# kolenyo2099/revers-o

Hardware: AMD Instinct MI355X
Metric: images/sec embed+top-k (PE-L14-336, 1M x 1024 gallery) (higher is better)
Workload: dtype bf16

## Files before the change

### include/revo.h

```cpp
#ifndef REVO_H
#define REVO_H
#include <stdint.h>

#ifdef __cplusplus
extern "C" {
#endif

typedef struct revo_vit revo_vit;
typedef struct revo_gallery revo_gallery;

typedef struct revo_vit_cfg {
    int32_t image_size, patch_size, width, layers, heads, mlp_dim, out_dim, pool_heads;
    int32_t use_cls;
    int32_t use_ls;
    float ln_eps, rope_theta;
    int32_t pool_mlp_dim;
} revo_vit_cfg;

typedef struct revo_tensor {
    const char* name;
    const float* data;
    int64_t numel;
} revo_tensor;

const char* revo_last_error(void);
int32_t revo_version(void);
int32_t revo_sync(void* stream);

int32_t revo_vit_create(const revo_vit_cfg* cfg, const revo_tensor* weights, int32_t n_weights, int32_t device,
                        int32_t max_batch, revo_vit** out);
int32_t revo_vit_destroy(revo_vit* vit);
int32_t revo_vit_forward(revo_vit* vit, const void* images, int32_t image_dtype, int32_t batch, float* out,
                         int32_t normalize, void* stream);
int32_t revo_vit_seq_len(const revo_vit* vit);
int32_t revo_vit_stats(revo_vit* vit, double* out4, int32_t reset, void* stream);

int32_t revo_gallery_create(int32_t dim, int64_t capacity, int32_t device, int32_t keep_f32, revo_gallery** out);
int32_t revo_gallery_destroy(revo_gallery* g);
int32_t revo_gallery_append(revo_gallery* g, const float* vecs, int64_t n, int32_t normalize, int32_t src_on_device,
                            void* stream);
int64_t revo_gallery_size(const revo_gallery* g);
int32_t revo_gallery_clear(revo_gallery* g);
int32_t revo_gallery_read(revo_gallery* g, int64_t start, int64_t n, float* dst, int32_t dst_on_device);

int32_t revo_gallery_remove(revo_gallery* g, const uint32_t* remove_bits, int64_t rows, int32_t src_on_device,
                            int64_t* n_removed, void* stream);
int32_t revo_gallery_update(revo_gallery* g, const int64_t* row_idx, const float* vecs, int64_t n, int32_t normalize,
                            int32_t src_on_device, void* stream);

int32_t revo_search_topk(revo_gallery* g, const float* queries, int32_t n_queries, int32_t k, int32_t has_threshold,
                         float threshold, int64_t index_offset, float* scores, int64_t* indices, int32_t* counts,
                         void* stream);
int32_t revo_search_topk_large(revo_gallery* g, const float* queries, int32_t n_queries, int32_t k, int32_t has_threshold,
                               float threshold, int64_t index_offset, float* scores, int64_t* indices, int32_t* counts,
                               void* stream);
int32_t revo_gallery_pairs(revo_gallery* g, float threshold, int64_t* n_pairs, void* stream);
int32_t revo_gallery_pairs_read(revo_gallery* g, int64_t start, int64_t n, int64_t* pairs, float* scores,
                                int32_t dst_on_device);
int32_t revo_gallery_clusters(revo_gallery* g, float threshold, int64_t* n_clusters, int64_t* n_members, void* stream);
int32_t revo_gallery_clusters_read(revo_gallery* g, int64_t* labels, int64_t* offsets, int64_t* members,
                                   int32_t dst_on_device);
int32_t revo_search_range(revo_gallery* g, const float* queries, int32_t n_queries, float threshold, int64_t index_offset,
                          int64_t* n_results, void* stream);
int32_t revo_search_range_read(revo_gallery* g, int64_t* offsets, int64_t start, int64_t n, int64_t* indices, float* scores,
                               int32_t dst_on_device);
int32_t revo_search_recommend(revo_gallery* g, const float* examples, int32_t n_positive, int32_t n_negative, int32_t k,
                              int32_t has_threshold, float threshold, int64_t index_offset, float* scores, int64_t* indices,
                              int32_t* counts, void* stream);
int32_t revo_search_discover(revo_gallery* g, const float* target, const float* positives, const float* negatives,
                             int32_t n_pairs, int32_t k, int32_t has_threshold, float threshold, int64_t index_offset,
                             float* scores, int64_t* indices, int32_t* counts, void* stream);
int32_t revo_search_maxsim(revo_gallery* g, const float* queries, int32_t n_vectors, int32_t k, int32_t has_threshold,
                           float threshold, int64_t index_offset, float* scores, int32_t* group_ids, int32_t* counts,
                           float* part_scores, int64_t* part_rows, void* stream);
int32_t revo_search_mmr(revo_gallery* g, const float* queries, int32_t n_queries, int32_t k, int32_t candidates,
                        float diversity, int32_t has_threshold, float threshold, int64_t index_offset, float* scores,
                        float* mmr_values, int64_t* indices, int32_t* counts, void* stream);
int32_t revo_search_ksel(int32_t k);
int32_t revo_search_set_total_rows(revo_gallery* g, int64_t total_rows);
int32_t revo_search_set_filter(revo_gallery* g, const uint32_t* allow_bits, int64_t rows, int32_t src_on_device,
                               void* stream);
int32_t revo_search_set_groups(revo_gallery* g, const int32_t* group_of_row, int64_t rows, int32_t src_on_device,
                               void* stream);
int32_t revo_search_groups(revo_gallery* g, const float* queries, int32_t n_queries, int32_t limit, int32_t group_size,
                           int32_t has_threshold, float threshold, int64_t index_offset, float* scores, int64_t* indices,
                           int32_t* hit_counts, int32_t* group_ids, int32_t* group_counts, void* stream);
int32_t revo_search_estimates(int32_t k);
int32_t revo_search_plan(const revo_gallery* g, int32_t n_queries, int32_t k, int64_t* out4);
int32_t revo_search_candidates(revo_gallery* g, const float* queries, int32_t n_queries, int32_t k, int32_t top_m,
                               uint32_t* bounds, void* stream);
int32_t revo_search_finish(revo_gallery* g, int32_t n_queries, int32_t k, int32_t has_threshold, float threshold,
                           int64_t index_offset, const uint32_t* all_bounds, int32_t parts, int32_t top_m, float* scores,
                           int64_t* indices, int32_t* counts, float* cert, void* stream);
int32_t revo_search_exact(revo_gallery* g, int32_t n, const int32_t* q_idx, const float* need, int32_t k,
                          int32_t has_threshold, float threshold, int64_t index_offset, float* scores, int64_t* indices,
                          int32_t* counts, void* stream);
int32_t revo_search_stats(revo_gallery* g, int32_t* out8, void* stream);
int32_t revo_topk_merge(const float* scores, const int64_t* indices, int32_t parts, int32_t n_queries, int32_t k,
                        int32_t has_threshold, float threshold, float* out_scores, int64_t* out_indices,
                        int32_t* out_counts, void* stream);

int64_t revo_topk_packed_bytes(int32_t n_queries, int32_t k);
int32_t revo_topk_merge_packed(const void* packed, int32_t parts, int32_t n_queries, int32_t k, int32_t has_threshold,
                               float threshold, float* out_scores, int64_t* out_indices, int32_t* out_counts,
                               int32_t* unc_count, int32_t* unc_q, float* unc_need, void* stream);

int32_t revo_op_gemm(int32_t epilogue, const void* a_bf16, int64_t lda, const void* b_bf16, int64_t ldb, int32_t m,
                     int32_t n, int32_t k, void* c, int64_t ldc, const float* bias, const float* gamma, void* stream);
int32_t revo_op_gemm_rope(const void* a_bf16, int64_t lda, const void* b_bf16, int64_t ldb, int32_t m, int32_t n, int32_t k,
                          void* c_bf16, int64_t ldc, const float* bias, const float* cos_sin, int32_t seq,
                          int32_t head_dim, int32_t rope_cols, void* stream);
int32_t revo_op_gemm_resid_ln(const void* a_bf16, int64_t lda, const void* b_bf16, int64_t ldb, int32_t m, int32_t n, int32_t k,
                              float* c, int64_t ldc, const float* bias, const float* gamma, void* xb_bf16, int64_t ldxb,
                              void* stats, int32_t* done, void* xlo_bf16, int32_t x_in_planes, int32_t planes_out, void* stream);
int32_t revo_op_gemm_ln_in(int32_t epilogue, const void* a_bf16, int64_t lda, const void* b_bf16, int64_t ldb, int32_t m, int32_t n,
                           int32_t k, void* c_bf16, int64_t ldc, const float* bias, const float* csum, const void* stats,
                           int32_t parts, float eps, void* tele, void* stream);
int32_t revo_op_gemm_ln_in_rope(const void* a_bf16, int64_t lda, const void* b_bf16, int64_t ldb, int32_t m, int32_t n, int32_t k,
                                void* c_bf16, int64_t ldc, const float* bias, const float* csum, const void* stats, int32_t parts,
                                float eps, const float* cos_sin, int32_t seq, int32_t head_dim, int32_t rope_cols, void* stream);
int32_t revo_op_gemm_resid_norm(const void* a_bf16, int64_t lda, const void* b_bf16, int64_t ldb, int32_t m, int32_t n, int32_t k,
                                float* c, int64_t ldc, const float* bias, const float* gamma, void* ln_out_bf16, int64_t ln_ldo,
                                float eps, int32_t* fused, void* stream);
int32_t revo_probe_mfma(const void* src_bf16, int64_t n_elems, float* sink, int32_t blocks, int32_t iters, void* stream);
int64_t revo_probe_mfma_flops(int32_t blocks, int32_t iters);
int32_t revo_probe_copy(void* dst, const void* src, int64_t bytes, void* stream);
#ifdef REVO_EXPERIMENTS
int32_t revo_vit_set_debug_layers(revo_vit* vit, int32_t n_layers);
int32_t revo_vit_read_residual(revo_vit* vit, int32_t batch, float* dst, void* stream);
int32_t revo_vit_read_tap(revo_vit* vit, int32_t which, int32_t batch, void* dst, void* stream);
int32_t revo_search_set_mode(revo_gallery* g, int32_t mode);
int32_t revo_debug_set_remove_chunk(int64_t rows);
int32_t revo_op_set_phase_groups(int32_t groups);
int32_t revo_op_set_qstores(int32_t on);
int32_t revo_debug_gemm_stamps(void* buf, int32_t items);
int32_t revo_debug_attention_clock(void* buf);
int32_t revo_debug_gemm_forms(int32_t reset);
int32_t revo_op_set_gemm_tile(int32_t tile);
int32_t revo_op_set_variant(int32_t flags);
int32_t revo_op_set_ln_fold(int32_t on);
int32_t revo_op_set_gemm_debug(int32_t flags);
int64_t revo_debug_scan_plan(int32_t Q, int64_t rows, int64_t* out, int32_t cap);
int32_t revo_debug_stream_in_planes(const revo_vit* vit, int32_t batch);
int64_t revo_debug_read_workspace(revo_gallery* g, int64_t offset, int64_t bytes, void* host_dst);
int32_t revo_debug_seed_bounds(revo_gallery* g, const uint32_t* bounds);
int32_t revo_probe_gridbar(int32_t mode, void* ctr_err, void* buf, int32_t n16, int32_t blocks, int32_t threads,
                           int32_t iters, float* sink, void* stamps, void* stream);
int32_t revo_debug_scan_stats(int64_t* out8);
#endif
int32_t revo_op_layernorm(const float* x, int64_t ldx, const float* w, const float* b, float eps, int32_t rows,
                          int32_t width, void* out, int64_t ldo, int32_t out_is_bf16, void* stream);
int32_t revo_op_layernorm_logits(const float* x, int64_t ldx, const float* w, const float* b, float eps, int32_t rows,
                                 int32_t width, float* out, int64_t ldo, const float* qk, const float* ck, int32_t heads,
                                 int32_t seq, float* logits, void* stream);
int32_t revo_op_linear_f32(int32_t epi, const float* A, int64_t lda, const float* Wt, int64_t ldw, const float* bias, int32_t M,
                           int32_t N, int32_t K, float* C, int64_t ldc, void* stream);
int32_t revo_op_pool_rows(const float* x, int64_t ldx, const float* logits, int32_t batch, int32_t seq, int32_t width,
                          int32_t heads, float* u, void* stream);
int32_t revo_op_rope(void* qkv_bf16, int64_t ld, const float* cos_sin, int32_t rows, int32_t seq, int32_t width,
                     int32_t heads, void* stream);
int32_t revo_op_attention(const void* qkv_bf16, int64_t ld, void* out_bf16, int64_t ldo, int32_t batch, int32_t seq,
                          int32_t heads, int32_t head_dim, void* stream);
int32_t revo_op_f32_to_bf16(const float* src, int64_t ld_src, void* dst_bf16, int64_t ld_dst, int64_t rows,
                            int32_t cols, void* stream);

int32_t revo_prof_enable(int32_t on);
int32_t revo_prof_reset(void);
int32_t revo_prof_report(char* buf, int32_t capacity);

typedef struct revo_crop_job {
    const uint8_t* src;
    int32_t height, width;
    int64_t row_stride;
    int32_t x0, y0, x1, y1;
} revo_crop_job;
int32_t revo_preprocess_crop_resize(const revo_crop_job* jobs, int32_t n, int32_t out_size, uint8_t* out, void* stream);

#ifdef __cplusplus
}
#endif
#endif
```

### revers-o_amd/_lib.py

```python
import ctypes as C
import os

_HERE = os.path.dirname(os.path.abspath(__file__))
LIB_PATH = os.path.join(_HERE, "librevo.so")


class RevoError(RuntimeError):
    pass


class VitCfg(C.Structure):
    _fields_ = [(n, C.c_int32) for n in (
        "image_size", "patch_size", "width", "layers", "heads", "mlp_dim", "out_dim", "pool_heads",
        "use_cls", "use_ls")] + [("ln_eps", C.c_float), ("rope_theta", C.c_float), ("pool_mlp_dim", C.c_int32)]


class Tensor(C.Structure):
    _fields_ = [("name", C.c_char_p), ("data", C.c_void_p), ("numel", C.c_int64)]


class CropJob(C.Structure):
    _fields_ = [("src", C.c_void_p), ("height", C.c_int32), ("width", C.c_int32), ("row_stride", C.c_int64),
                ("x0", C.c_int32), ("y0", C.c_int32), ("x1", C.c_int32), ("y1", C.c_int32)]


_p, _i32, _i64, _f32 = C.c_void_p, C.c_int32, C.c_int64, C.c_float

SIGNATURES = {
    "revo_last_error": (C.c_char_p, []),
    "revo_version": (_i32, []),
    "revo_sync": (_i32, [_p]),
    "revo_vit_create": (_i32, [C.POINTER(VitCfg), C.POINTER(Tensor), _i32, _i32, _i32, C.POINTER(_p)]),
    "revo_vit_destroy": (_i32, [_p]),
    "revo_vit_forward": (_i32, [_p, _p, _i32, _i32, _p, _i32, _p]),
    "revo_vit_seq_len": (_i32, [_p]),
    "revo_vit_stats": (_i32, [_p, C.POINTER(C.c_double), _i32, _p]),
    "revo_gallery_create": (_i32, [_i32, _i64, _i32, _i32, C.POINTER(_p)]),
    "revo_gallery_destroy": (_i32, [_p]),
    "revo_gallery_append": (_i32, [_p, _p, _i64, _i32, _i32, _p]),
    "revo_gallery_size": (_i64, [_p]),
    "revo_gallery_clear": (_i32, [_p]),
    "revo_gallery_read": (_i32, [_p, _i64, _i64, _p, _i32]),
    "revo_gallery_remove": (_i32, [_p, _p, _i64, _i32, C.POINTER(C.c_int64), _p]),
    "revo_gallery_update": (_i32, [_p, _p, _p, _i64, _i32, _i32, _p]),
    "revo_gallery_pairs": (_i32, [_p, _f32, C.POINTER(C.c_int64), _p]),
    "revo_gallery_pairs_read": (_i32, [_p, _i64, _i64, _p, _p, _i32]),
    "revo_gallery_clusters": (_i32, [_p, _f32, C.POINTER(C.c_int64), C.POINTER(C.c_int64), _p]),
    "revo_gallery_clusters_read": (_i32, [_p, _p, _p, _p, _i32]),
    "revo_search_range": (_i32, [_p, _p, _i32, _f32, _i64, C.POINTER(C.c_int64), _p]),
    "revo_search_range_read": (_i32, [_p, _p, _i64, _i64, _p, _p, _i32]),
    "revo_search_recommend": (_i32, [_p, _p, _i32, _i32, _i32, _i32, _f32, _i64, _p, _p, _p, _p]),
    "revo_search_discover": (_i32, [_p, _p, _p, _p, _i32, _i32, _i32, _f32, _i64, _p, _p, _p, _p]),
    "revo_search_maxsim": (_i32, [_p, _p, _i32, _i32, _i32, _f32, _i64, _p, _p, _p, _p, _p, _p]),
    "revo_search_mmr": (_i32, [_p, _p, _i32, _i32, _i32, _f32, _i32, _f32, _i64, _p, _p, _p, _p, _p]),
    "revo_search_topk": (_i32, [_p, _p, _i32, _i32, _i32, _f32, _i64, _p, _p, _p, _p]),
    "revo_search_topk_large": (_i32, [_p, _p, _i32, _i32, _i32, _f32, _i64, _p, _p, _p, _p]),
    "revo_search_ksel": (_i32, [_i32]),
    "revo_search_set_total_rows": (_i32, [_p, _i64]),
    "revo_search_set_filter": (_i32, [_p, _p, _i64, _i32, _p]),
    "revo_search_set_groups": (_i32, [_p, _p, _i64, _i32, _p]),
    "revo_search_groups": (_i32, [_p, _p, _i32, _i32, _i32, _i32, _f32, _i64, _p, _p, _p, _p, _p, _p]),
    "revo_search_estimates": (_i32, [_i32]),
    "revo_search_plan": (_i32, [_p, _i32, _i32, C.POINTER(C.c_int64)]),
    "revo_search_candidates": (_i32, [_p, _p, _i32, _i32, _i32, _p, _p]),
    "revo_search_finish": (_i32, [_p, _i32, _i32, _i32, _f32, _i64, _p, _i32, _i32, _p, _p, _p, _p, _p]),
    "revo_search_exact": (_i32, [_p, _i32, _p, _p, _i32, _i32, _f32, _i64, _p, _p, _p, _p]),
    "revo_search_stats": (_i32, [_p, C.POINTER(C.c_int32), _p]),
    "revo_topk_merge": (_i32, [_p, _p, _i32, _i32, _i32, _i32, _f32, _p, _p, _p, _p]),
    "revo_topk_packed_bytes": (_i64, [_i32, _i32]),
    "revo_topk_merge_packed": (_i32, [_p, _i32, _i32, _i32, _i32, _f32, _p, _p, _p, _p, _p, _p, _p]),
    "revo_op_gemm": (_i32, [_i32, _p, _i64, _p, _i64, _i32, _i32, _i32, _p, _i64, _p, _p, _p]),
    "revo_op_gemm_resid_ln": (_i32, [_p, _i64, _p, _i64, _i32, _i32, _i32, _p, _i64, _p, _p, _p, _i64, _p, C.POINTER(C.c_int32), _p, _i32,
                                     _i32, _p]),
    "revo_op_gemm_ln_in": (_i32, [_i32, _p, _i64, _p, _i64, _i32, _i32, _i32, _p, _i64, _p, _p, _p, _i32, _f32, _p, _p]),
    "revo_op_gemm_rope": (_i32, [_p, _i64, _p, _i64, _i32, _i32, _i32, _p, _i64, _p, _p, _i32, _i32, _i32, _p]),
    "revo_op_gemm_ln_in_rope": (_i32, [_p, _i64, _p, _i64, _i32, _i32, _i32, _p, _i64, _p, _p, _p, _i32, _f32, _p, _i32, _i32, _i32,
                                       _p]),
    "revo_op_gemm_resid_norm": (_i32, [_p, _i64, _p, _i64, _i32, _i32, _i32, _p, _i64, _p, _p, _p, _i64, _f32, C.POINTER(C.c_int32),
                                       _p]),
    "revo_op_layernorm": (_i32, [_p, _i64, _p, _p, _f32, _i32, _i32, _p, _i64, _i32, _p]),
    "revo_op_layernorm_logits": (_i32, [_p, _i64, _p, _p, _f32, _i32, _i32, _p, _i64, _p, _p, _i32, _i32, _p, _p]),
    "revo_op_linear_f32": (_i32, [_i32, _p, _i64, _p, _i64, _p, _i32, _i32, _i32, _p, _i64, _p]),
    "revo_op_pool_rows": (_i32, [_p, _i64, _p, _i32, _i32, _i32, _i32, _p, _p]),
    "revo_op_rope": (_i32, [_p, _i64, _p, _i32, _i32, _i32, _i32, _p]),
    "revo_op_attention": (_i32, [_p, _i64, _p, _i64, _i32, _i32, _i32, _i32, _p]),
    "revo_op_f32_to_bf16": (_i32, [_p, _i64, _p, _i64, _i64, _i32, _p]),
    "revo_prof_enable": (_i32, [_i32]),
    "revo_prof_reset": (_i32, []),
    "revo_prof_report": (_i32, [C.c_char_p, _i32]),
    "revo_preprocess_crop_resize": (_i32, [C.POINTER(CropJob), _i32, _i32, _p, _p]),
    "revo_probe_mfma": (_i32, [_p, _i64, _p, _i32, _i32, _p]),
    "revo_probe_mfma_flops": (_i64, [_i32, _i32]),
    "revo_probe_copy": (_i32, [_p, _p, _i64, _p]),
}

EXPERIMENT_SIGNATURES = {
    "revo_vit_set_debug_layers": (_i32, [_p, _i32]),
    "revo_vit_read_residual": (_i32, [_p, _i32, _p, _p]),
    "revo_vit_read_tap": (_i32, [_p, _i32, _i32, _p, _p]),
    "revo_search_set_mode": (_i32, [_p, _i32]),
    "revo_op_set_gemm_tile": (_i32, [_i32]),
    "revo_op_set_phase_groups": (_i32, [_i32]),
    "revo_op_set_qstores": (_i32, [_i32]),
    "revo_debug_gemm_forms": (_i32, [_i32]),
    "revo_debug_gemm_stamps": (_i32, [_p, _i32]),
    "revo_debug_attention_clock": (_i32, [_p]),
    "revo_op_set_variant": (_i32, [_i32]),
    "revo_op_set_ln_fold": (_i32, [_i32]),
    "revo_op_set_gemm_debug": (_i32, [_i32]),
    "revo_debug_scan_stats": (_i32, [C.POINTER(C.c_int64)]),
    "revo_debug_set_remove_chunk": (_i32, [_i64]),
    "revo_debug_seed_bounds": (_i32, [_p, _p]),
    "revo_debug_read_workspace": (_i64, [_p, _i64, _i64, _p]),
    "revo_debug_stream_in_planes": (_i32, [_p, _i32]),
    "revo_probe_gridbar": (_i32, [_i32, _p, _p, _i32, _i32, _i32, _i32, _p, _p, _p]),
    "revo_debug_scan_plan": (_i64, [_i32, _i64, C.POINTER(C.c_int64), _i32]),
}
BASE_SIGNATURES = dict(SIGNATURES)
if os.environ.get("REVO_LIBRARY_PATH"):
    LIB_PATH = os.environ["REVO_LIBRARY_PATH"]
elif os.environ.get("REVO_EXPERIMENTS") == "1":
    LIB_PATH = os.path.join(_HERE, "librevo_exp.so")
if os.environ.get("REVO_EXPERIMENTS") == "1":
    SIGNATURES = dict(SIGNATURES, **EXPERIMENT_SIGNATURES)

_lib = None
_lib_exp = None


def product_is_experiment_build():
    return os.environ.get("REVO_EXPERIMENTS") == "1"


def load_exp():
    global _lib_exp
    if _lib_exp is not None:
        return _lib_exp
    import torch
    path = os.path.join(_HERE, "librevo_exp.so")
    if not os.path.exists(path):
        raise RevoError(f"{path} not found: build it with `make -C revers-o_amd/csrc exp`")
    lib = C.CDLL(path)
    for name, (res, args) in dict(BASE_SIGNATURES, **EXPERIMENT_SIGNATURES).items():
        fn = getattr(lib, name)
        fn.restype = res
        fn.argtypes = args
    _lib_exp = lib
    return lib


def load():
    global _lib
    if _lib is not None:
        return _lib
    import torch
    if not os.path.exists(LIB_PATH):
        raise RevoError(
            f"{LIB_PATH} not found: build it with `python -c 'import __graft_entry__ as g; g.build()'` "
            "(or `make -C revers-o_amd/csrc`).  There is no CPU fallback for the hot path.")
    lib = C.CDLL(LIB_PATH)
    for name, (res, args) in SIGNATURES.items():
        try:
            fn = getattr(lib, name)
        except AttributeError:
            if os.environ.get("REVO_LIBRARY_PATH"):
                continue
            raise
        fn.restype = res
        fn.argtypes = args
    _lib = lib
    return lib


def check(rc, what=""):
    if rc != 0:
        msg = load().revo_last_error().decode("utf-8", "replace")
        if _lib_exp is not None:
            msg = (msg + " | " if msg else "") + _lib_exp.revo_last_error().decode("utf-8", "replace")
        raise RevoError(f"{what} failed (status {rc}): {msg}")


def ptr(t):
    return None if t is None else C.c_void_p(t.data_ptr())


def current_stream():
    import torch
    return C.c_void_p(torch.cuda.current_stream().cuda_stream)
```

### revers-o_amd/csrc/api.hip

```cpp
#include <algorithm>
#include <cmath>
#include <cstdlib>
#include <cstring>
#include <map>
#include <memory>
#include <mutex>
#include <string>
#include <vector>

#include "../../include/revo.h"
#include "api_internal.h"
#include "kernels.h"

static thread_local std::string g_err;
void revo_set_error(const std::string& msg) { g_err = msg; }
extern "C" const char* revo_last_error(void) { return g_err.c_str(); }
extern "C" int32_t revo_version(void) { return 100; }

extern "C" int32_t revo_sync(void* stream) {
    REVO_HIP_CHECK(hipStreamSynchronize((hipStream_t)stream));
    return 0;
}

namespace {
struct Profiler {
    int on = 0;
    unsigned sample[4] = {0, 0, 0, 0};
    std::mutex mu;
    std::vector<ProfRec> recs;
    std::vector<hipEvent_t> pool;
    std::map<std::string, std::pair<long, double>> acc;
    hipEvent_t get() {
        if (!pool.empty()) { hipEvent_t e = pool.back(); pool.pop_back(); return e; }
        hipEvent_t e; (void)hipEventCreate(&e); return e;
    }
    void drain() {
        for (auto& r : recs) {
            float ms = 0.f;
            if (hipEventSynchronize(r.b) == hipSuccess && hipEventElapsedTime(&ms, r.a, r.b) == hipSuccess) {
                auto& s = acc[r.cls];
                s.first += 1; s.second += ms;
            }
            pool.push_back(r.a); pool.push_back(r.b);
        }
        recs.clear();
    }
} g_prof;
}

ProfScope::ProfScope(const char* cls, hipStream_t s) : active(g_prof.on != 0), st(s) {
    if (active && g_prof.on >= 2) {
        const int which = !strcmp(cls, "gemm_qkv") ? 0 : !strcmp(cls, "gemm_out") ? 1 : !strcmp(cls, "gemm_fc1") ? 2 :
                          !strcmp(cls, "gemm_fc2") ? 3 : -1;
        active = which >= 0;
        if (active && g_prof.on == 3) active = (g_prof.sample[which]++ & 3) == 0;
    }
    if (!active) return;
    std::lock_guard<std::mutex> lk(g_prof.mu);
    rec.cls = cls; rec.a = g_prof.get(); rec.b = g_prof.get();
    (void)hipEventRecord(rec.a, st);
}
ProfScope::~ProfScope() {
    if (!active) return;
    (void)hipEventRecord(rec.b, st);
    std::lock_guard<std::mutex> lk(g_prof.mu);
    g_prof.recs.push_back(rec);
}

extern "C" int32_t revo_prof_enable(int32_t on) {
    g_prof.on = on < 0 ? 0 : (on > 3 ? 1 : on);
    for (auto& x : g_prof.sample) x = 0;
    return 0;
}
extern "C" int32_t revo_prof_reset(void) {
    std::lock_guard<std::mutex> lk(g_prof.mu);
    g_prof.drain();
    g_prof.acc.clear();
    return 0;
}
extern "C" int32_t revo_prof_report(char* buf, int32_t capacity) {
    std::lock_guard<std::mutex> lk(g_prof.mu);
    g_prof.drain();
    std::string s = "{";
    bool first = true;
    for (auto& kv : g_prof.acc) {
        if (!first) s += ", ";
        first = false;
        s += "\"" + kv.first + "\": {\"launches\": " + std::to_string(kv.second.first) +
             ", \"ms\": " + std::to_string(kv.second.second) + "}";
    }
    s += "}";
    if ((int)s.size() + 1 > capacity) { revo_set_error("prof_report: buffer too small"); return -2; }
    memcpy(buf, s.c_str(), s.size() + 1);
    return 0;
}

namespace revo {
__global__ __launch_bounds__(256) void probe_q_kernel(const float* __restrict__ w, const float* __restrict__ bias,
                                                      const float* __restrict__ probe, int W, float scale,
                                                      float* __restrict__ q) {
    const int lane = threadIdx.x & 63;
    const int o = blockIdx.x * 4 + (threadIdx.x >> 6);
    if (o >= W) return;
    float acc = 0.f;
    for (int i = lane; i < W; i += 64) acc = fmaf(w[(long)o * W + i], probe[i], acc);
    acc = wave_sum(acc);
    if (lane == 0) q[o] = (acc + bias[o]) * scale;
}
}

struct LayerW {
    bf16_t *w_qkv, *w_o, *w_fc1, *w_fc2;
    float *b_qkv, *b_o, *b_fc1, *b_fc2, *c_qkv, *c_fc1, *ls1, *ls2;
};

constexpr size_t SPLITK_WS_ELEMS = 16u << 20;
struct revo_vit {
    revo_vit_cfg cfg;
    int device = 0, max_batch = 0, S = 0, G2 = 0, Kp = 0, hd = 0, phd = 0, PM = 0, debug_layers = -1;
    std::vector<void*> owned;
    bf16_t* w_patch = nullptr; float *cls = nullptr, *pos = nullptr, *lnpre_w = nullptr, *lnpre_b = nullptr,
            *lnpost_w = nullptr, *lnpost_b = nullptr;
    std::vector<LayerW> layers;
    float *q_probe = nullptr, *qk = nullptr, *ck = nullptr, *w_v = nullptr, *b_v = nullptr, *w_po = nullptr, *b_po = nullptr;
    float *pln_w = nullptr, *pln_b = nullptr, *w_pfc1 = nullptr, *b_pfc1 = nullptr, *w_pfc2 = nullptr, *b_pfc2 = nullptr,
          *w_projT = nullptr;
    float2* rope_cs = nullptr;
    bf16_t *patches = nullptr, *h = nullptr, *qkv = nullptr, *att = nullptr, *mlp = nullptr;
    bf16_t* xlo = nullptr;
    float *x = nullptr, *pool_logits = nullptr, *pool_u = nullptr, *pool_att = nullptr, *pool_o = nullptr, *pool_h = nullptr,
          *pool_m = nullptr, *feat = nullptr;
    float* splitk_ws = nullptr;
    float2* ln_stats = nullptr;
    int ln_parts = 0;
    unsigned long long* ln_tele = nullptr;

    template <class T> int dalloc(T** out, size_t count) {
        void* p = nullptr;
        REVO_HIP_CHECK(hipMalloc(&p, count * sizeof(T) + 256));
        owned.push_back(p);
        *out = (T*)p;
        return 0;
    }
    ~revo_vit() {
        for (void* p : owned) (void)hipFree(p);
    }
};

namespace {
struct WeightMap {
    std::map<std::string, const revo_tensor*> m;
    const revo_tensor* get(const std::string& name, int64_t numel) {
        auto it = m.find(name);
        if (it == m.end()) { revo_set_error("missing weight tensor: " + name); return nullptr; }
        if (it->second->numel != numel) {
            revo_set_error("weight " + name + ": expected " + std::to_string(numel) + " elements, got " +
                           std::to_string(it->second->numel));
            return nullptr;
        }
        return it->second;
    }
};

int up_f32(revo_vit* v, WeightMap& wm, const std::string& name, int64_t numel, float** out) {
    const revo_tensor* t = wm.get(name, numel);
    if (!t) return -2;
    CHECK_RC(v->dalloc(out, (size_t)numel));
    REVO_HIP_CHECK(hipMemcpy(*out, t->data, (size_t)numel * 4, hipMemcpyDefault));
    return 0;
}
int up_folded(revo_vit* v, WeightMap& wm, float* stage, float* gb, const std::string& wname, const std::string& bname,
              const std::string& ln, int64_t rows, int64_t cols, bf16_t** w_out, float** c_out, float** b_out) {
    const revo_tensor *tw = wm.get(wname, rows * cols), *tb = wm.get(bname, rows), *tg = wm.get(ln + ".weight", cols),
                      *te = wm.get(ln + ".bias", cols);
    if (!tw || !tb || !tg || !te) return -2;
    CHECK_RC(v->dalloc(w_out, (size_t)(rows * cols)));
    CHECK_RC(v->dalloc(c_out, (size_t)rows));
    CHECK_RC(v->dalloc(b_out, (size_t)rows));
    REVO_HIP_CHECK(hipMemcpy(stage, tw->data, (size_t)(rows * cols) * 4, hipMemcpyDefault));
    REVO_HIP_CHECK(hipMemcpy(gb, tg->data, (size_t)cols * 4, hipMemcpyDefault));
    REVO_HIP_CHECK(hipMemcpy(gb + cols, te->data, (size_t)cols * 4, hipMemcpyDefault));
    REVO_HIP_CHECK(hipMemcpy(gb + 2 * cols, tb->data, (size_t)rows * 4, hipMemcpyDefault));
    CHECK_RC(revo::launch_fold_ln_linear(stage, gb, gb + cols, gb + 2 * cols, (int)rows, (int)cols, *w_out, cols, *c_out, *b_out, 0));
    REVO_HIP_CHECK(hipStreamSynchronize(0));
    return 0;
}
int up_bf16(revo_vit* v, float* stage, const float* src, int64_t rows, int64_t cols, int64_t ld, bf16_t** out) {
    CHECK_RC(v->dalloc(out, (size_t)(rows * ld)));
    REVO_HIP_CHECK(hipMemcpy(stage, src, (size_t)(rows * cols) * 4, hipMemcpyDefault));
    CHECK_RC(revo::launch_f32_to_bf16(stage, cols, *out, ld, rows, (int)cols, 0));
    REVO_HIP_CHECK(hipStreamSynchronize(0));
    return 0;
}
}

extern "C" int32_t revo_vit_create(const revo_vit_cfg* cfg, const revo_tensor* weights, int32_t n_weights,
                                   int32_t device, int32_t max_batch, revo_vit** out) {
    API_BEGIN
    REVO_REQUIRE(cfg && weights && out, "vit_create: null argument");
    REVO_REQUIRE(max_batch >= 1, "vit_create: max_batch must be >= 1");
    const revo_vit_cfg& c = *cfg;
    REVO_REQUIRE(c.image_size % c.patch_size == 0, "vit_create: image_size must be a multiple of patch_size");
    REVO_REQUIRE(c.width % c.heads == 0 && c.width % c.pool_heads == 0, "vit_create: width must divide into heads");
    REVO_REQUIRE(c.width % 64 == 0 && c.mlp_dim % 64 == 0, "vit_create: width and mlp_dim must be multiples of 64");
    REVO_REQUIRE(c.out_dim % 4 == 0, "vit_create: out_dim must be a multiple of 4");
    REVO_REQUIRE(c.width / c.heads == 64 || c.width / c.heads == 96,
                 "vit_create: body head_dim must be 64 (PE-Core B16 / L14) or 96 (G14)");
    REVO_REQUIRE(c.image_size > 0 && c.patch_size > 0 && c.layers >= 1 && c.heads >= 1 && c.pool_heads >= 1 && n_weights >= 0,
                 "vit_create: sizes must be positive");
    std::unique_ptr<revo_vit> v(new revo_vit());
    v->cfg = c; v->device = device; v->max_batch = max_batch;
#ifdef REVO_EXPERIMENTS
    if (const char* e = getenv("REVO_LN_FOLD")) revo::gemm_set_ln_fold(atoi(e));
#endif
    const int W = c.width, M = c.mlp_dim, D = c.out_dim, P = c.patch_size, G = c.image_size / P;
    v->G2 = G * G; v->S = v->G2 + (c.use_cls ? 1 : 0);
    v->hd = W / c.heads; v->phd = W / c.pool_heads;
    const int PM = c.pool_mlp_dim > 0 ? c.pool_mlp_dim : 4 * W;
    REVO_REQUIRE(PM % 64 == 0, "vit_create: pool_mlp_dim must be a multiple of 64");
    v->PM = PM;
    const int Kreal = 3 * P * P;
    v->Kp = (Kreal + 63) / 64 * 64;
    const int S = v->S;

    WeightMap wm;
    for (int i = 0; i < n_weights; ++i) {
        REVO_REQUIRE(weights[i].name && weights[i].data, "vit_create: weight entry with a null name or data pointer");
        wm.m[weights[i].name] = &weights[i];
    }
    {
        std::vector<std::pair<std::string, int64_t>> need = {
            {"visual.conv1.weight", (int64_t)W * Kreal}, {"visual.positional_embedding", (int64_t)S * W},
            {"visual.ln_pre.weight", W}, {"visual.ln_pre.bias", W}, {"visual.ln_post.weight", W}, {"visual.ln_post.bias", W},
            {"visual.attn_pool.probe", W}, {"visual.attn_pool.attn.in_proj_weight", (int64_t)3 * W * W},
            {"visual.attn_pool.attn.in_proj_bias", 3 * W}, {"visual.attn_pool.attn.out_proj.weight", (int64_t)W * W},
            {"visual.attn_pool.attn.out_proj.bias", W}, {"visual.attn_pool.layernorm.weight", W},
            {"visual.attn_pool.layernorm.bias", W}, {"visual.attn_pool.mlp.c_fc.weight", (int64_t)PM * W},
            {"visual.attn_pool.mlp.c_fc.bias", PM}, {"visual.attn_pool.mlp.c_proj.weight", (int64_t)W * PM},
            {"visual.attn_pool.mlp.c_proj.bias", W}, {"visual.proj", (int64_t)W * D}};
        if (c.use_cls) need.push_back({"visual.class_embedding", W});
        for (int i = 0; i < c.layers; ++i) {
            const std::string p = "visual.transformer.resblocks." + std::to_string(i) + ".";
            for (const char* n : {"ln_1.weight", "ln_1.bias", "ln_2.weight", "ln_2.bias", "attn.out_proj.bias", "mlp.c_proj.bias"})
                need.push_back({p + n, W});
            need.push_back({p + "attn.in_proj_weight", (int64_t)3 * W * W});
            need.push_back({p + "attn.in_proj_bias", 3 * W});
            need.push_back({p + "attn.out_proj.weight", (int64_t)W * W});
            need.push_back({p + "mlp.c_fc.weight", (int64_t)M * W});
            need.push_back({p + "mlp.c_fc.bias", M});
            need.push_back({p + "mlp.c_proj.weight", (int64_t)W * M});
            if (c.use_ls) { need.push_back({p + "ls_1.gamma", W}); need.push_back({p + "ls_2.gamma", W}); }
        }
        for (auto& kv : need)
            if (!wm.get(kv.first, kv.second)) return -2;
        if (wm.m.size() != need.size()) {
            std::map<std::string, int64_t> want(need.begin(), need.end());
            for (auto& kv : wm.m)
                if (!want.count(kv.first)) {
                    revo_set_error("unexpected weight tensor: " + kv.first + " (not read by this architecture" +
                                   (c.use_ls ? ")" : "; LayerScale needs cfg.use_ls = 1)"));
                    return -2;
                }
        }
    }
    REVO_ON_DEVICE(device);

    size_t stage_elems = (size_t)std::max({(long)3 * W * W, (long)M * W, (long)PM * W, (long)W * Kreal, (long)W * D});
    float* stage = nullptr;
    REVO_HIP_CHECK(hipMalloc((void**)&stage, stage_elems * 4));
    struct StageGuard { float* p; ~StageGuard() { (void)hipFree(p); } } sg{stage};
    float* gb = nullptr;
    REVO_HIP_CHECK(hipMalloc((void**)&gb, (size_t)(2 * W + std::max(3 * W, M)) * 4));
    StageGuard sg2{gb};

    const revo_tensor* t;
    if (!(t = wm.get("visual.conv1.weight", (int64_t)W * Kreal))) return -2;
    CHECK_RC(v->dalloc(&v->w_patch, (size_t)W * 3 * v->Kp));
    REVO_HIP_CHECK(hipMemcpy(stage, t->data, (size_t)W * Kreal * 4, hipMemcpyDefault));
    CHECK_RC(revo::launch_split_hi_lo_hi(stage, W, Kreal, 1.0f / 255.0f, v->w_patch, v->Kp, 0));
    REVO_HIP_CHECK(hipStreamSynchronize(0));
    if (c.use_cls) CHECK_RC(up_f32(v.get(), wm, "visual.class_embedding", W, &v->cls));
    CHECK_RC(up_f32(v.get(), wm, "visual.positional_embedding", (int64_t)S * W, &v->pos));
    CHECK_RC(up_f32(v.get(), wm, "visual.ln_pre.weight", W, &v->lnpre_w));
    CHECK_RC(up_f32(v.get(), wm, "visual.ln_pre.bias", W, &v->lnpre_b));
    CHECK_RC(up_f32(v.get(), wm, "visual.ln_post.weight", W, &v->lnpost_w));
    CHECK_RC(up_f32(v.get(), wm, "visual.ln_post.bias", W, &v->lnpost_b));
    v->layers.resize(c.layers);
    for (int i = 0; i < c.layers; ++i) {
        const std::string p = "visual.transformer.resblocks." + std::to_string(i) + ".";
        LayerW& L = v->layers[i];
        memset(&L, 0, sizeof(L));
        CHECK_RC(up_folded(v.get(), wm, stage, gb, p + "attn.in_proj_weight", p + "attn.in_proj_bias", p + "ln_1", 3 * W, W,
                           &L.w_qkv, &L.c_qkv, &L.b_qkv));
        if (!(t = wm.get(p + "attn.out_proj.weight", (int64_t)W * W))) return -2;
        CHECK_RC(up_bf16(v.get(), stage, t->data, W, W, W, &L.w_o));
        CHECK_RC(up_f32(v.get(), wm, p + "attn.out_proj.bias", W, &L.b_o));
        CHECK_RC(up_folded(v.get(), wm, stage, gb, p + "mlp.c_fc.weight", p + "mlp.c_fc.bias", p + "ln_2", M, W,
                           &L.w_fc1, &L.c_fc1, &L.b_fc1));
        if (!(t = wm.get(p + "mlp.c_proj.weight", (int64_t)W * M))) return -2;
        CHECK_RC(up_bf16(v.get(), stage, t->data, W, M, M, &L.w_fc2));
        CHECK_RC(up_f32(v.get(), wm, p + "mlp.c_proj.bias", W, &L.b_fc2));
        if (c.use_ls) {
            CHECK_RC(up_f32(v.get(), wm, p + "ls_1.gamma", W, &L.ls1));
            CHECK_RC(up_f32(v.get(), wm, p + "ls_2.gamma", W, &L.ls2));
        }
    }
    {
        const std::string p = "visual.attn_pool.";
        float *probe = nullptr, *wi = nullptr, *bi = nullptr;
        CHECK_RC(up_f32(v.get(), wm, p + "probe", W, &probe));
        CHECK_RC(up_f32(v.get(), wm, p + "attn.in_proj_weight", (int64_t)3 * W * W, &wi));
        CHECK_RC(up_f32(v.get(), wm, p + "attn.in_proj_bias", 3 * W, &bi));
        CHECK_RC(v->dalloc(&v->q_probe, (size_t)W));
        hipLaunchKernelGGL(revo::probe_q_kernel, dim3((W + 3) / 4), dim3(256), 0, 0, wi, bi, probe, W,
                           1.0f / sqrtf((float)v->phd), v->q_probe);
        REVO_HIP_CHECK(hipGetLastError());
        CHECK_RC(v->dalloc(&v->qk, (size_t)c.pool_heads * W));
        CHECK_RC(v->dalloc(&v->ck, (size_t)c.pool_heads));
        CHECK_RC(revo::launch_probe_qk(v->q_probe, wi + (size_t)W * W, bi + W, W, c.pool_heads, v->qk, v->ck, 0));
        v->w_v = wi + (size_t)2 * W * W;
        v->b_v = bi + 2 * W;
        REVO_HIP_CHECK(hipStreamSynchronize(0));
        CHECK_RC(up_f32(v.get(), wm, p + "attn.out_proj.weight", (int64_t)W * W, &v->w_po));
        CHECK_RC(up_f32(v.get(), wm, p + "attn.out_proj.bias", W, &v->b_po));
        CHECK_RC(up_f32(v.get(), wm, p + "layernorm.weight", W, &v->pln_w));
        CHECK_RC(up_f32(v.get(), wm, p + "layernorm.bias", W, &v->pln_b));
        CHECK_RC(up_f32(v.get(), wm, p + "mlp.c_fc.weight", (int64_t)PM * W, &v->w_pfc1));
        CHECK_RC(up_f32(v.get(), wm, p + "mlp.c_fc.bias", PM, &v->b_pfc1));
        CHECK_RC(up_f32(v.get(), wm, p + "mlp.c_proj.weight", (int64_t)W * PM, &v->w_pfc2));
        CHECK_RC(up_f32(v.get(), wm, p + "mlp.c_proj.bias", W, &v->b_pfc2));
    }
    if (!(t = wm.get("visual.proj", (int64_t)W * D))) return -2;
    CHECK_RC(v->dalloc(&v->w_projT, (size_t)D * W));
    REVO_HIP_CHECK(hipMemcpy(stage, t->data, (size_t)W * D * 4, hipMemcpyDefault));
    CHECK_RC(revo::launch_transpose_f32(stage, W, D, v->w_projT, 0));
    REVO_HIP_CHECK(hipStreamSynchronize(0));

    {
        const int hd = v->hd, d = hd / 2, nf = d / 2;
        std::vector<float2> cs((size_t)S * (hd / 2));
        const int start = c.use_cls ? 1 : 0;
        for (int s = 0; s < S; ++s) {
            for (int pi = 0; pi < hd / 2; ++pi) {
                double ang = 0.0;
                if (!(c.use_cls && s == 0)) {
                    const int g = s - (c.use_cls ? 1 : 0);
                    const int gy = g / G, gx = g % G;
                    const bool xaxis = pi < nf;
                    const int f = xaxis ? pi : pi - nf;
                    const double freq = 1.0 / pow((double)c.rope_theta, (double)(2 * f) / (double)d);
                    ang = (double)((xaxis ? gx : gy) + start) * freq;
                }
                cs[(size_t)s * (hd / 2) + pi] = make_float2((float)cos(ang), (float)sin(ang));
            }
        }
        CHECK_RC(v->dalloc(&v->rope_cs, cs.size()));
        REVO_HIP_CHECK(hipMemcpy(v->rope_cs, cs.data(), cs.size() * sizeof(float2), hipMemcpyHostToDevice));
    }

    const size_t rows = (size_t)max_batch * S, B = (size_t)max_batch;
    CHECK_RC(v->dalloc(&v->patches, (size_t)max_batch * v->G2 * 3 * v->Kp));
    CHECK_RC(v->dalloc(&v->x, rows * W));
    CHECK_RC(v->dalloc(&v->h, rows * W));
    CHECK_RC(v->dalloc(&v->qkv, rows * 3 * W));
    CHECK_RC(v->dalloc(&v->att, rows * W));
    CHECK_RC(v->dalloc(&v->mlp, rows * M));
    CHECK_RC(v->dalloc(&v->pool_logits, B * c.pool_heads * S));
    CHECK_RC(v->dalloc(&v->pool_u, B * c.pool_heads * W));
    CHECK_RC(v->dalloc(&v->pool_att, B * W));
    CHECK_RC(v->dalloc(&v->pool_o, B * W));
    CHECK_RC(v->dalloc(&v->pool_h, B * W));
    CHECK_RC(v->dalloc(&v->pool_m, B * PM));
    CHECK_RC(v->dalloc(&v->feat, B * D));
    CHECK_RC(v->dalloc(&v->splitk_ws, SPLITK_WS_ELEMS));
    v->ln_parts = (W % 256 == 0 && W / 256 <= 6) ? W / 256 : 0;
    if (v->ln_parts) CHECK_RC(v->dalloc(&v->ln_stats, rows * (size_t)v->ln_parts));
    if (v->ln_parts) CHECK_RC(v->dalloc(&v->xlo, rows * W));
    CHECK_RC(v->dalloc(&v->ln_tele, 4));
    REVO_HIP_CHECK(hipMemset(v->ln_tele, 0, 4 * sizeof(unsigned long long)));
    REVO_HIP_CHECK(hipDeviceSynchronize());
    *out = v.release();
    return 0;
    API_END
}

extern "C" int32_t revo_vit_destroy(revo_vit* vit) {
    API_BEGIN
    if (vit) { DeviceGuard dg(vit->device); delete vit; }
    return 0;
    API_END
}
extern "C" int32_t revo_vit_seq_len(const revo_vit* vit) { return vit ? vit->S : -1; }
extern "C" int32_t revo_vit_stats(revo_vit* vit, double* out4, int32_t reset, void* stream) {
    API_BEGIN
    REVO_REQUIRE(vit && out4, "vit_stats: null argument");
    REVO_ON_DEVICE(vit->device);
    unsigned long long c[4] = {0, 0, 0, 0};
    REVO_HIP_CHECK(hipStreamSynchronize((hipStream_t)stream));
    REVO_HIP_CHECK(hipMemcpy(c, vit->ln_tele, sizeof(c), hipMemcpyDeviceToHost));
    if (reset) REVO_HIP_CHECK(hipMemset(vit->ln_tele, 0, sizeof(c)));
    out4[0] = (double)c[0]; out4[1] = (double)c[1]; out4[2] = (double)c[2]; out4[3] = (double)revo::LNC_TELE_RATIO;
    return 0;
    API_END
}
#ifdef REVO_EXPERIMENTS
extern "C" int32_t revo_vit_set_debug_layers(revo_vit* vit, int32_t n) {
    REVO_REQUIRE(vit, "null handle");
    vit->debug_layers = n;
    return 0;
}
extern "C" int32_t revo_vit_read_residual(revo_vit* vit, int32_t batch, float* dst, void* stream) {
    REVO_REQUIRE(vit && dst && batch >= 1 && batch <= vit->max_batch, "read_residual: bad arguments");
    REVO_ON_DEVICE(vit->device);
    REVO_HIP_CHECK(hipMemcpyAsync(dst, vit->x, (size_t)batch * vit->S * vit->cfg.width * 4, hipMemcpyDeviceToDevice,
                                  (hipStream_t)stream));
    return 0;
}

extern "C" int32_t revo_vit_read_tap(revo_vit* vit, int32_t which, int32_t batch, void* dst, void* stream) {
    REVO_REQUIRE(vit && dst && batch >= 1 && batch <= vit->max_batch, "read_tap: bad arguments");
    REVO_ON_DEVICE(vit->device);
    const size_t rows = (size_t)batch * vit->S, W = vit->cfg.width;
    const void* src = nullptr;
    size_t bytes = 0;
    switch (which) {
        case 0: src = vit->x; bytes = rows * W * 4; break;
        case 1: src = vit->x; bytes = rows * W * 4; break;
        case 2: src = vit->pool_o; bytes = (size_t)batch * W * 4; break;
        default: REVO_REQUIRE(false, "read_tap: which must be 0 (residual), 1 (ln_post output) or 2 (pooled)");
    }
    REVO_HIP_CHECK(hipMemcpyAsync(dst, src, bytes, hipMemcpyDeviceToDevice, (hipStream_t)stream));
    return 0;
}
#endif

namespace {
struct LnAfter { float eps; bf16_t* out; long ldo; int* fused; float2* stats; int* folded; bf16_t* lo; int x_in_planes, planes_out; };
struct LnBefore { const float2* stats; int parts; const float* c; float eps; };
int gemm(const char* cls, int epi, const bf16_t* A, long lda, const bf16_t* B, long ldb, int M, int N, int K, void* C,
         long ldc, const float* bias, const float* gamma, hipStream_t st, float* ws = nullptr, long ws_elems = 0,
         const LnAfter* ln = nullptr) {
    revo::GemmArgs a{};
    a.A = A; a.lda = lda; a.B = B; a.ldb = ldb; a.M = M; a.N = N; a.K = K; a.C = C; a.ldc = ldc;
    a.bias = bias; a.gamma = gamma; a.ws = ws; a.ws_elems = ws_elems;
    if (ln) {
        a.ln_eps = ln->eps; a.ln_ldo = ln->ldo; a.ln_fused = ln->fused;
        if (ln->fused) a.ln_out = ln->out;
        if (ln->stats) { a.lnf_xb = ln->out; a.lnf_ldxb = ln->ldo; a.lnf_stats = ln->stats; a.lnf_done = ln->folded; }
        if (ln->lo) { a.xp_hi = ln->out; a.xp_lo = ln->lo; a.xp_ld = ln->ldo; a.xp_in = ln->x_in_planes; a.xp_out = ln->planes_out; }
    }
    ProfScope ps(cls, st);
    return revo::launch_gemm(epi, a, st);
}
}

static int vit_forward_range(revo_vit* vv, const void* images_all, int32_t image_dtype, int b0, int B, float* out_all,
                             int32_t normalize, hipStream_t st) {
    const revo_vit_cfg& c = vv->cfg;
    const int W = c.width, Md = c.mlp_dim, D = c.out_dim, S = vv->S, PM = vv->PM;
    const int rows = B * S;
    using namespace revo;
    struct View {
        bf16_t *patches, *h, *qkv, *att, *mlp;
        float *x, *pool_logits, *pool_u, *pool_att, *pool_o, *pool_h, *pool_m, *feat;
    } w;
    const size_t r0 = (size_t)b0 * S;
    const int PH = c.pool_heads;
    w.patches = vv->patches + (size_t)b0 * vv->G2 * 3 * vv->Kp;
    w.x = vv->x + r0 * W; w.h = vv->h + r0 * W; w.qkv = vv->qkv + r0 * 3 * W; w.att = vv->att + r0 * W;
    w.mlp = vv->mlp + r0 * Md;
    w.pool_logits = vv->pool_logits + (size_t)b0 * PH * S; w.pool_u = vv->pool_u + (size_t)b0 * PH * W;
    w.pool_att = vv->pool_att + (size_t)b0 * W; w.pool_o = vv->pool_o + (size_t)b0 * W;
    w.pool_h = vv->pool_h + (size_t)b0 * W; w.pool_m = vv->pool_m + (size_t)b0 * PM;
    w.feat = vv->feat + (size_t)b0 * D;
    const size_t img_elems = (size_t)3 * c.image_size * c.image_size;
    const void* images = (const char*)images_all + (size_t)b0 * img_elems * (image_dtype == 1 ? 1 : 4);
    float* out = out_all + (size_t)b0 * D;
    struct FW {
        bf16_t *patches, *h, *qkv, *att, *mlp;
        float *x, *pool_logits, *pool_u, *pool_att, *pool_o, *pool_h, *pool_m, *feat;
        int Kp, G2, hd, phd, debug_layers;
        bf16_t* w_patch; float *pos, *cls, *lnpre_w, *lnpre_b, *lnpost_w, *lnpost_b;
        const std::vector<LayerW>& layers;
        float *qk, *ck, *w_v, *b_v, *w_po, *b_po, *pln_w, *pln_b, *w_pfc1, *b_pfc1, *w_pfc2, *b_pfc2, *w_projT;
        float2* rope_cs;
    } fw{w.patches, w.h, w.qkv, w.att, w.mlp, w.x, w.pool_logits, w.pool_u, w.pool_att, w.pool_o, w.pool_h, w.pool_m, w.feat,
         vv->Kp, vv->G2, vv->hd, vv->phd, vv->debug_layers, vv->w_patch, vv->pos, vv->cls, vv->lnpre_w, vv->lnpre_b,
         vv->lnpost_w, vv->lnpost_b, vv->layers, vv->qk, vv->ck, vv->w_v, vv->b_v, vv->w_po, vv->b_po, vv->pln_w,
         vv->pln_b, vv->w_pfc1, vv->b_pfc1, vv->w_pfc2, vv->b_pfc2, vv->w_projT, vv->rope_cs};
    const FW* v = &fw;

    {
        const int parts = image_dtype == 1 ? 2 : 3;
        { ProfScope ps("patchify", st);
          CHECK_RC(launch_patchify(images, image_dtype == 1, B, c.image_size, c.patch_size, v->patches, v->Kp, st)); }
        GemmArgs a{};
        a.A = v->patches; a.lda = (long)parts * v->Kp; a.B = v->w_patch; a.ldb = 3l * v->Kp; a.M = B * v->G2; a.N = W;
        a.K = parts * v->Kp;
        a.C = v->x; a.ldc = W; a.pos = v->pos; a.S = S; a.G2 = v->G2; a.cls = c.use_cls ? 1 : 0;
        { ProfScope ps("gemm_patch", st); CHECK_RC(launch_gemm(EPI_PATCH, a, st)); }
        if (c.use_cls) { ProfScope ps("elementwise", st); CHECK_RC(launch_cls_rows(v->x, W, v->cls, v->pos, B, S, W, st)); }
    }
    if (v->debug_layers == -2) return 0;
    { ProfScope ps("layernorm", st);
      CHECK_RC(launch_layernorm(v->x, W, v->lnpre_w, v->lnpre_b, c.ln_eps, rows, W, v->x, W, 0, st)); }

    const int nl = v->debug_layers < 0 ? c.layers : std::min(v->debug_layers, c.layers);
    enum { H_NONE = 0, H_NORM = 1, H_XB = 2 };
    int h_state = H_NONE;
    float2* stats = vv->ln_parts ? vv->ln_stats + r0 * vv->ln_parts : nullptr;
    bf16_t* xlo = (vv->xlo && gemm_ln_planes_enabled() && gemm_resid_folds(rows, W, W, W, W, W) && gemm_resid_folds(rows, W, Md, Md, Md, W))
                      ? vv->xlo + r0 * W : nullptr;
    bool x_planes = false;
    auto ln_before = [&](const float* csum, GemmArgs& a) {
        if (h_state == H_XB) { a.lnc_stats = stats; a.lnc_parts = vv->ln_parts; a.lnc_c = csum; a.lnc_eps = c.ln_eps; a.lnc_tele = vv->ln_tele; }
    };
    auto normalise_if_needed = [&]() -> int {
        if (h_state != H_NONE) return 0;
        if (x_planes) { revo_set_error("vit_forward: internal: a LayerNorm kernel was asked for while the stream is in planes"); return -3; }
        ProfScope ps("layernorm", st);
        CHECK_RC(launch_layernorm(v->x, W, nullptr, nullptr, c.ln_eps, rows, W, v->h, W, 1, st));
        h_state = H_NORM;
        return 0;
    };
    for (int i = 0; i < nl; ++i) {
        const LayerW& L = v->layers[i];
        CHECK_RC(normalise_if_needed());
        {
            GemmArgs a{};
            a.A = v->h; a.lda = W; a.B = L.w_qkv; a.ldb = W; a.M = rows; a.N = 3 * W; a.K = W; a.C = v->qkv;
            a.ldc = 3 * W; a.bias = L.b_qkv; a.rope_cs = v->rope_cs; a.rope_S = S; a.rope_hd = v->hd;
            a.rope_cols = 2 * W;
            ln_before(L.c_qkv, a);
            ProfScope ps("gemm_qkv", st);
            CHECK_RC(launch_gemm(EPI_BF16_ROPE, a, st));
        }
        { ProfScope ps("attention", st);
          CHECK_RC(launch_attention_ex(v->qkv, 3 * W, v->att, W, B, S, c.heads, v->hd, c.use_cls, st)); }
        int fused = 0, folded = 0;
        const LnAfter ln2{c.ln_eps, v->h, W, &fused, stats, &folded, xlo, x_planes ? 1 : 0, xlo ? 1 : 0};
        CHECK_RC(gemm("gemm_out", EPI_RESID_F32, v->att, W, L.w_o, W, rows, W, W, v->x, W, L.b_o, L.ls1, st, vv->splitk_ws,
                      (long)SPLITK_WS_ELEMS, &ln2));
        h_state = folded ? H_XB : (fused ? H_NORM : H_NONE);
        x_planes = xlo && folded;
#ifdef REVO_EXPERIMENTS
        if (folded && getenv("REVO_LNFOLD_TOUCH")) {
            ProfScope ps("touch", st);
            REVO_HIP_CHECK(hipMemcpyAsync(v->qkv, v->h, (size_t)rows * W * 2, hipMemcpyDeviceToDevice, st));
        }
#endif
        CHECK_RC(normalise_if_needed());
        {
            GemmArgs a{};
            a.A = v->h; a.lda = W; a.B = L.w_fc1; a.ldb = W; a.M = rows; a.N = Md; a.K = W; a.C = v->mlp; a.ldc = Md;
            a.bias = L.b_fc1;
            ln_before(L.c_fc1, a);
            ProfScope ps("gemm_fc1", st);
            CHECK_RC(launch_gemm(EPI_BF16_GELU, a, st));
        }
        fused = 0; folded = 0;
        const bool last = i + 1 >= nl;
        const LnAfter ln1n{c.ln_eps, v->h, W, last ? nullptr : &fused, last ? nullptr : stats, last ? nullptr : &folded, xlo,
                           x_planes ? 1 : 0, (xlo && !last) ? 1 : 0};
        CHECK_RC(gemm("gemm_fc2", EPI_RESID_F32, v->mlp, Md, L.w_fc2, Md, rows, W, Md, v->x, W, L.b_fc2, L.ls2, st,
                      vv->splitk_ws, (long)SPLITK_WS_ELEMS, (!last || x_planes) ? &ln1n : nullptr));
        h_state = last ? H_NONE : (folded ? H_XB : (fused ? H_NORM : H_NONE));
        x_planes = !last && xlo && folded;
#ifdef REVO_EXPERIMENTS
        if (folded && !last && getenv("REVO_LNFOLD_TOUCH")) {
            ProfScope ps("touch", st);
            REVO_HIP_CHECK(hipMemcpyAsync(v->qkv, v->h, (size_t)rows * W * 2, hipMemcpyDeviceToDevice, st));
        }
#endif
    }
    if (v->debug_layers >= 0) return 0;

    { ProfScope ps("layernorm", st);
      const LnLogits lg{v->qk, v->ck, v->pool_logits, PH, S};
      CHECK_RC(launch_layernorm(v->x, W, v->lnpost_w, v->lnpost_b, c.ln_eps, rows, W, v->x, W, 0, st, &lg)); }
    { ProfScope ps("pool_attention", st);
      CHECK_RC(launch_pool_head_rows(v->x, W, B, S, W, PH, v->pool_logits, v->pool_u, st)); }
    { ProfScope ps("gemm_pool", st);
      CHECK_RC(launch_gemm_f32_skinny(0, v->pool_u, (long)PH * W, W, v->phd, v->w_v, W, v->b_v, B, W, W, v->pool_att, W, st));
      CHECK_RC(launch_gemm_f32_skinny(0, v->pool_att, W, 0, 0, v->w_po, W, v->b_po, B, W, W, v->pool_o, W, st)); }
    { ProfScope ps("layernorm", st);
      CHECK_RC(launch_layernorm(v->pool_o, W, v->pln_w, v->pln_b, c.ln_eps, B, W, v->pool_h, W, 0, st)); }
    float* feat = normalize ? v->feat : out;
    { ProfScope ps("gemm_pool", st);
      CHECK_RC(launch_gemm_f32_skinny(1, v->pool_h, W, 0, 0, v->w_pfc1, W, v->b_pfc1, B, PM, W, v->pool_m, PM, st));
      CHECK_RC(launch_gemm_f32_skinny(2, v->pool_m, PM, 0, 0, v->w_pfc2, PM, v->b_pfc2, B, W, PM, v->pool_o, W, st));
      CHECK_RC(launch_gemm_f32_skinny(0, v->pool_o, W, 0, 0, v->w_projT, W, nullptr, B, D, W, feat, D, st)); }
    if (normalize) {
        ProfScope ps("l2norm", st);
        CHECK_RC(launch_l2norm_rows(v->feat, D, out, D, nullptr, 0, B, D, st));
    }
    return 0;
}

extern "C" int32_t revo_vit_forward(revo_vit* v, const void* images, int32_t image_dtype, int32_t batch, float* out,
                                    int32_t normalize, void* stream) {
    API_BEGIN
    REVO_REQUIRE(v && images && out, "vit_forward: null argument");
    REVO_REQUIRE(batch >= 1 && batch <= v->max_batch, "vit_forward: batch exceeds max_batch of the handle");
    REVO_REQUIRE(image_dtype == 0 || image_dtype == 1, "vit_forward: image_dtype must be 0 (f32) or 1 (u8)");
    REVO_ON_DEVICE(v->device);
    hipStream_t st = (hipStream_t)stream;
    return vit_forward_range(v, images, image_dtype, 0, batch, out, normalize, st);
    API_END
}

extern "C" int32_t revo_op_gemm(int32_t epi, const void* a, int64_t lda, const void* b, int64_t ldb, int32_t m,
                                int32_t n, int32_t k, void* c, int64_t ldc, const float* bias, const float* gamma,
                                void* stream) {
    API_BEGIN
    REVO_REQUIRE(epi >= 0 && epi <= 3, "op_gemm: epilogue must be 0..3");
    constexpr long OP_WS_ELEMS = 16l << 20;
    hipStream_t st = (hipStream_t)stream;
    float* ws = nullptr;
    if (epi == revo::EPI_RESID_F32) REVO_HIP_CHECK(hipMallocAsync((void**)&ws, OP_WS_ELEMS * 4, st));
    const int rc = gemm("gemm_op", epi, (const bf16_t*)a, lda, (const bf16_t*)b, ldb, m, n, k, c, ldc, bias, gamma, st, ws,
                        ws ? OP_WS_ELEMS : 0);
    if (ws) REVO_HIP_CHECK(hipFreeAsync(ws, st));
    return rc;
    API_END
}
extern "C" int32_t revo_op_gemm_resid_ln(const void* a, int64_t lda, const void* b, int64_t ldb, int32_t m, int32_t n, int32_t k,
                                         float* c, int64_t ldc, const float* bias, const float* gamma, void* xb, int64_t ldxb,
                                         void* stats, int32_t* done, void* xlo, int32_t x_in_planes, int32_t planes_out,
                                         void* stream) {
    API_BEGIN
    REVO_REQUIRE(a && b && c && xb && done, "op_gemm_resid_ln: null argument");
    REVO_REQUIRE(stats || (xlo && x_in_planes && !planes_out), "op_gemm_resid_ln: stats may be NULL only for planes in, fp32 out");
    REVO_REQUIRE(xlo || (!x_in_planes && !planes_out), "op_gemm_resid_ln: planes need the low plane");
    constexpr long OP_WS_ELEMS = 16l << 20;
    hipStream_t st = (hipStream_t)stream;
    float* ws = nullptr;
    REVO_HIP_CHECK(hipMallocAsync((void**)&ws, OP_WS_ELEMS * 4, st));
    revo::GemmArgs g{};
    g.A = (const bf16_t*)a; g.lda = lda; g.B = (const bf16_t*)b; g.ldb = ldb; g.M = m; g.N = n; g.K = k; g.C = c; g.ldc = ldc;
    g.bias = bias; g.gamma = gamma; g.ws = ws; g.ws_elems = OP_WS_ELEMS;
    int flag = 0;
    if (stats) { g.lnf_xb = (bf16_t*)xb; g.lnf_ldxb = ldxb; g.lnf_stats = (float2*)stats; g.lnf_done = &flag; }
    if (xlo) { g.xp_hi = (bf16_t*)xb; g.xp_lo = (bf16_t*)xlo; g.xp_ld = ldxb; g.xp_in = x_in_planes != 0; g.xp_out = planes_out != 0; }
    const int rc = revo::launch_gemm(revo::EPI_RESID_F32, g, st);
    REVO_HIP_CHECK(hipFreeAsync(ws, st));
    *done = flag;
    return rc;
    API_END
}
extern "C" int32_t revo_op_gemm_ln_in(int32_t epi, const void* a, int64_t lda, const void* b, int64_t ldb, int32_t m, int32_t n,
                                      int32_t k, void* c, int64_t ldc, const float* bias, const float* csum, const void* stats,
                                      int32_t parts, float eps, void* tele, void* stream) {
    API_BEGIN
    REVO_REQUIRE(epi == revo::EPI_BF16 || epi == revo::EPI_BF16_GELU, "op_gemm_ln_in: epilogue must be 0 (bf16) or 1 (bf16 + GELU)");
    REVO_REQUIRE(a && b && c && csum && stats, "op_gemm_ln_in: null argument");
    revo::GemmArgs g{};
    g.A = (const bf16_t*)a; g.lda = lda; g.B = (const bf16_t*)b; g.ldb = ldb; g.M = m; g.N = n; g.K = k; g.C = c; g.ldc = ldc;
    g.bias = bias; g.lnc_stats = (const float2*)stats; g.lnc_parts = parts; g.lnc_c = csum; g.lnc_eps = eps;
    g.lnc_tele = (unsigned long long*)tele;
    return revo::launch_gemm(epi, g, (hipStream_t)stream);
    API_END
}
extern "C" int32_t revo_op_gemm_rope(const void* a, int64_t lda, const void* b, int64_t ldb, int32_t m, int32_t n,
                                     int32_t k, void* c, int64_t ldc, const float* bias, const float* cos_sin,
                                     int32_t seq, int32_t head_dim, int32_t rope_cols, void* stream) {
    API_BEGIN
    revo::GemmArgs g{};
    g.A = (const bf16_t*)a; g.lda = lda; g.B = (const bf16_t*)b; g.ldb = ldb; g.M = m; g.N = n; g.K = k; g.C = c; g.ldc = ldc;
    g.bias = bias; g.rope_cs = (const float2*)cos_sin; g.rope_S = seq; g.rope_hd = head_dim; g.rope_cols = rope_cols;
    return revo::launch_gemm(revo::EPI_BF16_ROPE, g, (hipStream_t)stream);
    API_END
}
extern "C" int32_t revo_op_gemm_ln_in_rope(const void* a, int64_t lda, const void* b, int64_t ldb, int32_t m, int32_t n, int32_t k,
                                           void* c, int64_t ldc, const float* bias, const float* csum, const void* stats,
                                           int32_t parts, float eps, const float* cos_sin, int32_t seq, int32_t head_dim,
                                           int32_t rope_cols, void* stream) {
    API_BEGIN
    REVO_REQUIRE(a && b && c && csum && stats && cos_sin, "op_gemm_ln_in_rope: null argument");
    revo::GemmArgs g{};
    g.A = (const bf16_t*)a; g.lda = lda; g.B = (const bf16_t*)b; g.ldb = ldb; g.M = m; g.N = n; g.K = k; g.C = c; g.ldc = ldc;
    g.bias = bias; g.rope_cs = (const float2*)cos_sin; g.rope_S = seq; g.rope_hd = head_dim; g.rope_cols = rope_cols;
    g.lnc_stats = (const float2*)stats; g.lnc_parts = parts; g.lnc_c = csum; g.lnc_eps = eps;
    return revo::launch_gemm(revo::EPI_BF16_ROPE, g, (hipStream_t)stream);
    API_END
}
extern "C" int32_t revo_op_gemm_resid_norm(const void* a, int64_t lda, const void* b, int64_t ldb, int32_t m, int32_t n, int32_t k,
                                           float* c, int64_t ldc, const float* bias, const float* gamma, void* ln_out,
                                           int64_t ln_ldo, float eps, int32_t* fused, void* stream) {
    API_BEGIN
    REVO_REQUIRE(a && b && c && ln_out && fused, "op_gemm_resid_norm: null argument");
    constexpr long OP_WS_ELEMS = 16l << 20;
    hipStream_t st = (hipStream_t)stream;
    float* ws = nullptr;
    REVO_HIP_CHECK(hipMallocAsync((void**)&ws, OP_WS_ELEMS * 4, st));
    int flag = 0;
    const LnAfter ln{eps, (bf16_t*)ln_out, ln_ldo, &flag, nullptr, nullptr, nullptr, 0, 0};
    const int rc = gemm("gemm_op", revo::EPI_RESID_F32, (const bf16_t*)a, lda, (const bf16_t*)b, ldb, m, n, k, c, ldc, bias, gamma,
                        st, ws, OP_WS_ELEMS, &ln);
    REVO_HIP_CHECK(hipFreeAsync(ws, st));
    *fused = flag;
    return rc;
    API_END
}
#ifdef REVO_EXPERIMENTS
extern "C" int32_t revo_op_set_variant(int32_t flags) {
    revo::gemm_force_gy((flags >> 4) & 15);
    revo::attention_force_nw((flags >> 8) & 15);
    revo::gemm_set_tail_split(((flags >> 12) & 1) ? 0 : 1);
    revo::gemm_set_persistent(((flags >> 16) & 1) ? 0 : 1);
    revo::gemm_set_splitk(((flags >> 17) & 1) ? 0 : 1);
    revo::gemm_set_min_tiles256(((flags >> 18) & 1) ? 0 : 100);
    revo::gemm_set_ring(((flags >> 19) & 1) ? 0 : 1, 0);
    revo::gemm_set_rows192(((flags >> 3) & 1) ? 0 : 1);
    revo::attention_set_shape16((flags >> 20) & 1);
    return 0;
}
extern "C" int32_t revo_op_set_ln_fold(int32_t on) {
    REVO_REQUIRE(on >= 0 && on <= 2, "set_ln_fold: 0 (LayerNorm kernels), 1 (folded, stream in planes: default) or 2 (folded, fp32 stream + bf16 copy)");
    revo::gemm_set_ln_fold(on);
    return 0;
}
extern "C" int32_t revo_op_set_qstores(int32_t on) {
    revo::gemm_set_qstores(on);
    return 0;
}
extern "C" int32_t revo_op_set_phase_groups(int32_t groups) {
    REVO_REQUIRE(groups >= 0 && groups <= 4, "set_phase_groups: 0 (heuristic), 1 (off) or 2..4");
    revo::gemm_set_phase_groups(groups);
    return 0;
}
extern "C" int32_t revo_debug_attention_clock(void* buf) {
    revo::attention_set_clock_buffer((unsigned long long*)buf);
    return 0;
}
extern "C" int32_t revo_debug_gemm_stamps(void* buf, int32_t items) {
    revo::gemm_set_stamps((unsigned long long*)buf, buf ? items : 0);
    return 0;
}
extern "C" int32_t revo_debug_gemm_forms(int32_t reset) { return (int32_t)revo::gemm_debug_forms(reset); }
extern "C" int32_t revo_op_set_gemm_tile(int32_t tile) {
    REVO_REQUIRE(tile == 0 || tile == 128 || tile == 256, "set_gemm_tile: 0, 128 or 256");
    revo::gemm_force_tile(tile);
    return 0;
}
extern "C" int32_t revo_op_set_gemm_debug(int32_t flags) {
    revo::gemm_set_debug(flags & 3);
    revo::gemm_set_stagger(((flags >> 28) & 15) * 200, 2 + ((flags >> 2) & 3));
    revo::topk_scan256_set_debug(((flags >> 13) & 7) | (((flags >> 20) & 255) << 3));
    return revo_op_set_variant(flags);
}
extern "C" int64_t revo_debug_scan_plan(int32_t Q, int64_t rows, int64_t* out, int32_t cap) {
    if (Q < 1 || rows < 1 || !out || cap < 2) return -1;
    return (int64_t)revo::topk_scan256_plan_dump(Q, (long)rows, (long*)out, cap);
}
extern "C" int32_t revo_debug_stream_in_planes(const revo_vit* v, int32_t batch) {
    if (!v || !v->xlo) return 0;
    const int W = v->cfg.width, Md = v->cfg.mlp_dim, rows = batch * v->S;
    return revo::gemm_ln_planes_enabled() && revo::gemm_resid_folds(rows, W, W, W, W, W) && revo::gemm_resid_folds(rows, W, Md, Md, Md, W);
}
#endif
extern "C" int32_t revo_op_layernorm(const float* x, int64_t ldx, const float* w, const float* b, float eps,
                                     int32_t rows, int32_t width, void* out, int64_t ldo, int32_t out_is_bf16,
                                     void* stream) {
    API_BEGIN
    return revo::launch_layernorm(x, ldx, w, b, eps, rows, width, out, ldo, out_is_bf16, (hipStream_t)stream);
    API_END
}
extern "C" int32_t revo_op_layernorm_logits(const float* x, int64_t ldx, const float* w, const float* b, float eps, int32_t rows,
                                            int32_t width, float* out, int64_t ldo, const float* qk, const float* ck,
                                            int32_t heads, int32_t seq, float* logits, void* stream) {
    API_BEGIN
    REVO_REQUIRE(x && out && qk && ck && logits && rows >= 1 && seq >= 1 && rows % seq == 0, "op_layernorm_logits: bad arguments");
    const revo::LnLogits lg{qk, ck, logits, heads, seq};
    return revo::launch_layernorm(x, ldx, w, b, eps, rows, width, out, ldo, 0, (hipStream_t)stream, &lg);
    API_END
}
extern "C" int32_t revo_op_linear_f32(int32_t epi, const float* A, int64_t lda, const float* Wt, int64_t ldw, const float* bias,
                                      int32_t M, int32_t N, int32_t K, float* C, int64_t ldc, void* stream) {
    API_BEGIN
    REVO_REQUIRE(A && Wt && C && M >= 1 && N >= 1 && K >= 16 && lda >= K && ldw >= K && ldc >= N, "op_linear_f32: bad arguments");
    return revo::launch_gemm_f32_skinny(epi, A, lda, 0, 0, Wt, ldw, bias, M, N, K, C, ldc, (hipStream_t)stream);
    API_END
}
extern "C" int32_t revo_op_pool_rows(const float* x, int64_t ldx, const float* logits, int32_t batch, int32_t seq, int32_t width,
                                     int32_t heads, float* u, void* stream) {
    API_BEGIN
    REVO_REQUIRE(x && logits && u && batch >= 1 && seq >= 1 && width >= 4 && ldx >= width, "op_pool_rows: bad arguments");
    return revo::launch_pool_head_rows(x, ldx, batch, seq, width, heads, logits, u, (hipStream_t)stream);
    API_END
}
extern "C" int32_t revo_op_rope(void* qkv, int64_t ld, const float* cs, int32_t rows, int32_t seq, int32_t width,
                                int32_t heads, void* stream) {
    API_BEGIN
    return revo::launch_rope((bf16_t*)qkv, ld, (const float2*)cs, rows, seq, width, heads, (hipStream_t)stream);
    API_END
}
extern "C" int32_t revo_op_attention(const void* qkv, int64_t ld, void* out, int64_t ldo, int32_t batch, int32_t seq,
                                     int32_t heads, int32_t head_dim, void* stream) {
    API_BEGIN
    ProfScope ps("attention", (hipStream_t)stream);
    return revo::launch_attention((const bf16_t*)qkv, ld, (bf16_t*)out, ldo, batch, seq, heads, head_dim,
                                  (hipStream_t)stream);
    API_END
}
extern "C" int32_t revo_op_f32_to_bf16(const float* src, int64_t ld_src, void* dst, int64_t ld_dst, int64_t rows,
                                       int32_t cols, void* stream) {
    API_BEGIN
    return revo::launch_f32_to_bf16(src, ld_src, (bf16_t*)dst, ld_dst, rows, cols, (hipStream_t)stream);
    API_END
}
```

### revers-o_amd/csrc/gemm.hip

```cpp
#include <type_traits>
#include "gemm_core.h"
#include "gemm256_core.h"
#include "kernels.h"

namespace revo {

__device__ __forceinline__ f32x2 gelu_erf2(f32x2 x) {
    const f32x2 ax = {__builtin_fabsf(x.x), __builtin_fabsf(x.y)};
    const f32x2 z = ax * 0.70710678118654752f;
    f32x2 p = z * 0.0000430638f + 0.0002765672f;
    p = p * z + 0.0001520143f;
    p = p * z + 0.0092705272f;
    p = p * z + 0.0422820123f;
    p = p * z + 0.0705230784f;
    p = p * z + 1.0f;
    p = p * p;
    p = p * p;
    p = p * p;
    p = p * p;
    const f32x2 r = {__builtin_amdgcn_rcpf(p.x), __builtin_amdgcn_rcpf(p.y)};
    return (x + ax * (1.0f - r)) * 0.5f;
}
__device__ __forceinline__ f32x4 gelu_erf4(f32x4 v) {
    const f32x2 lo = gelu_erf2((f32x2){v[0], v[1]}), hi = gelu_erf2((f32x2){v[2], v[3]});
    return (f32x4){lo.x, lo.y, hi.x, hi.y};
}
#ifndef REVO_LNC_ABLATE
#define REVO_LNC_ABLATE 0
#endif
#ifndef REVO_GELU_WIDTH
#define REVO_GELU_WIDTH 2
#endif
template <int NV>
__device__ __forceinline__ void gelu_erf4xn(f32x4 (&v)[NV]) {
    constexpr int NP = 2 * NV;
    f32x2 x[NP], ax[NP], z[NP], q[NP];
#pragma unroll
    for (int i = 0; i < NP; ++i) {
        x[i] = (f32x2){v[i >> 1][(i & 1) * 2], v[i >> 1][(i & 1) * 2 + 1]};
        ax[i] = (f32x2){__builtin_fabsf(x[i].x), __builtin_fabsf(x[i].y)};
    }
#pragma unroll
    for (int i = 0; i < NP; ++i) z[i] = ax[i] * 0.70710678118654752f;
#pragma unroll
    for (int i = 0; i < NP; ++i) q[i] = z[i] * 0.0000430638f + 0.0002765672f;
#pragma unroll
    for (int i = 0; i < NP; ++i) q[i] = q[i] * z[i] + 0.0001520143f;
#pragma unroll
    for (int i = 0; i < NP; ++i) q[i] = q[i] * z[i] + 0.0092705272f;
#pragma unroll
    for (int i = 0; i < NP; ++i) q[i] = q[i] * z[i] + 0.0422820123f;
#pragma unroll
    for (int i = 0; i < NP; ++i) q[i] = q[i] * z[i] + 0.0705230784f;
#pragma unroll
    for (int i = 0; i < NP; ++i) q[i] = q[i] * z[i] + 1.0f;
#pragma unroll
    for (int r = 0; r < 4; ++r)
#pragma unroll
        for (int i = 0; i < NP; ++i) q[i] = q[i] * q[i];
#pragma unroll
    for (int i = 0; i < NP; ++i) q[i] = (f32x2){__builtin_amdgcn_rcpf(q[i].x), __builtin_amdgcn_rcpf(q[i].y)};
#pragma unroll
    for (int i = 0; i < NP; ++i) q[i] = 1.0f - q[i];
#pragma unroll
    for (int i = 0; i < NP; ++i) x[i] = x[i] + ax[i] * q[i];
#pragma unroll
    for (int i = 0; i < NP; ++i) x[i] = x[i] * 0.5f;
#pragma unroll
    for (int i = 0; i < NV; ++i) v[i] = (f32x4){x[2 * i].x, x[2 * i].y, x[2 * i + 1].x, x[2 * i + 1].y};
}

__device__ __forceinline__ float row16_sum(float v) {
    v += __builtin_bit_cast(float, __builtin_amdgcn_update_dpp(0, __builtin_bit_cast(int, v), 0xB1, 0xf, 0xf, true));
    v += __builtin_bit_cast(float, __builtin_amdgcn_update_dpp(0, __builtin_bit_cast(int, v), 0x4E, 0xf, 0xf, true));
    v += __builtin_bit_cast(float, __builtin_amdgcn_update_dpp(0, __builtin_bit_cast(int, v), 0x141, 0xf, 0xf, true));
    v += __builtin_bit_cast(float, __builtin_amdgcn_update_dpp(0, __builtin_bit_cast(int, v), 0x140, 0xf, 0xf, true));
    return v;
}
constexpr int LNF_SLICE = 256;
__device__ __forceinline__ void lnf_merge(const float2* part, int P, float eps, float& rstd, float& mr) {
    float sm = 0.f, sq = 0.f;
    for (int i = 0; i < P; ++i) { const float2 t = part[i]; sm += t.x; sq += t.y; }
    const float mean = sm / (float)P;
    float dd = 0.f;
    for (int i = 0; i < P; ++i) { const float d = part[i].x - mean; dd = fmaf(d, d, dd); }
    const float var = fmaf((float)LNF_SLICE, dd, sq) / (float)(LNF_SLICE * P);
    rstd = rsqrtf(var + eps);
    mr = -mean * rstd;
}

template <int EPI, int MF, int NF>
__device__ __forceinline__ void gemm_epilogue(const GemmArgs& p, int m_base, int n_base, int lane,
                                              f32x4 (&acc)[MF][NF]) {
    const int lr = lane & 15, lq = lane >> 4;
    const bool lnc = (EPI == EPI_BF16 || EPI == EPI_BF16_GELU || EPI == EPI_BF16_ROPE) && p.lnc_stats != nullptr;
#pragma unroll
    for (int m = 0; m < MF; ++m) {
        const int row = m_base + m * 16 + lr;
        if (row >= p.M) continue;
        float ln_rstd = 1.f, ln_mr = 0.f;
        if (lnc)
            lnf_merge(p.lnc_stats + (long)row * p.lnc_parts, p.lnc_parts, p.lnc_eps, ln_rstd, ln_mr);
        long orow = row;
        int prow = 0;
        if (EPI == EPI_PATCH) {
            const int b = row / p.G2, g = row - b * p.G2;
            orow = (long)b * p.S + p.cls + g;
            prow = p.cls + g;
        }
#pragma unroll
        for (int n = 0; n < NF; ++n) {
            const int col = n_base + n * 16 + lq * 4;
            if (col >= p.N) continue;
            f32x4 v = acc[m][n];
            if (lnc) {
                const f32x4 c = *(const f32x4*)(p.lnc_c + col);
                const f32x4 b = p.bias ? *(const f32x4*)(p.bias + col) : (f32x4){0.f, 0.f, 0.f, 0.f};
                v = v * ln_rstd + (c * ln_mr + b);
            } else
            if (p.bias) {
                const f32x4 b = *(const f32x4*)(p.bias + col);
                v += b;
            }
            if (EPI == EPI_BF16_ROPE) {
                {
                    const bool rot = col < p.rope_cols;
                    const float2* t = p.rope_cs + (long)(row % p.rope_S) * (p.rope_hd >> 1) + ((col % p.rope_hd) >> 1);
                    const f32x4 tc = *(const f32x4*)t;
#pragma unroll
                    for (int h2 = 0; h2 < 2; ++h2) {
                        const float x0 = bf16_to_f32(f32_to_bf16(v[2 * h2])), x1 = bf16_to_f32(f32_to_bf16(v[2 * h2 + 1]));
                        const float cx = rot ? tc[2 * h2] : 1.0f, cy = rot ? tc[2 * h2 + 1] : 0.0f;
                        v[2 * h2] = x0 * cx - x1 * cy;
                        v[2 * h2 + 1] = x1 * cx + x0 * cy;
                    }
                }
            }
            if (EPI == EPI_BF16 || EPI == EPI_BF16_GELU || EPI == EPI_BF16_ROPE) {
                if (EPI == EPI_BF16_GELU) v = gelu_erf4(v);
                uint2 o;
                o.x = pack_bf16x2(v[0], v[1]);
                o.y = pack_bf16x2(v[2], v[3]);
                *(uint2*)((bf16_t*)p.C + orow * p.ldc + col) = o;
            } else if (EPI == EPI_RESID_F32) {
                float* dst = (float*)p.C + orow * p.ldc + col;
                f32x4 x = *(const f32x4*)dst;
                if (p.gamma) {
                    const f32x4 g = *(const f32x4*)(p.gamma + col);
                    v *= g;
                }
                x += v;
                *(f32x4*)dst = x;
            } else if (EPI == EPI_F32) {
                *(f32x4*)((float*)p.C + orow * p.ldc + col) = v;
            } else if (EPI == EPI_PATCH) {
                const f32x4 pe = *(const f32x4*)(p.pos + (long)prow * p.N + col);
                v += pe;
                *(f32x4*)((float*)p.C + orow * p.ldc + col) = v;
            }
        }
    }
}

template <int QT>
__device__ __forceinline__ void gemm256_load_resid(const GemmArgs& p, int m_base, int n_base, int lane, f32x4 (&res)[8],
                                                   bool nt = false) {
    int gcol = n_base + (lane & 15) * 4;
    gcol = gcol < p.N ? gcol : p.N - 4;
#pragma unroll
    for (int it = 0; it < 8; ++it) {
        int grow = m_base + QT * 32 + it * 4 + (lane >> 4);
        grow = grow < p.M ? grow : p.M - 1;
        const f32x4* src = (const f32x4*)((const float*)p.C + (long)grow * p.ldc + gcol);
        res[it] = nt ? __builtin_nontemporal_load(src) : *src;
    }
}
template <int EPI, int QT>
__device__ __forceinline__ void gemm256_epilogue_f32_quarter(const GemmArgs& p, char* slab, int m_base, int n_base,
                                                             int lane, f32x4 (&acc)[8][4], const f32x4 (&bias4)[4],
                                                             const f32x4 (&gamma4)[4], const f32x4 (&res)[8],
                                                             float2* lnst = nullptr) {
    constexpr int RS = 272;
    asm volatile("" : "+v"(lane) :: "memory");
    const int lr = lane & 15, lq = lane >> 4;
#pragma unroll
    for (int m = 0; m < 2; ++m)
#pragma unroll
        for (int n = 0; n < 4; ++n) {
            f32x4 v = acc[QT * 2 + m][n] + bias4[n];
            if (EPI == EPI_RESID_F32) v *= gamma4[n];
            *(f32x4*)(slab + (m * 16 + lr) * RS + (n * 16 + lq * 4) * 4) = v;
        }
    const int gcol = n_base + (lane & 15) * 4;
    float keep_m = 0.f, keep_q = 0.f;
#pragma unroll
    for (int it = 0; it < 8; ++it) {
        const int rl = it * 4 + (lane >> 4);
        f32x4 v = *(const f32x4*)(slab + rl * RS + (lane & 15) * 16);
        const int grow = m_base + QT * 32 + rl;
        if (EPI == EPI_RESID_F32) v += res[it];
        if (grow < p.M && gcol < p.N) {
            float* dst = (float*)p.C + (long)grow * p.ldc + gcol;
            if (EPI == EPI_RESID_F32 && lnst) __builtin_nontemporal_store(v, (f32x4*)dst);
            else *(f32x4*)dst = v;
            if (EPI == EPI_RESID_F32 && lnst) {
                uint2 o;
                o.x = pack_bf16x2(v[0], v[1]);
                o.y = pack_bf16x2(v[2], v[3]);
                *(uint2*)(p.lnf_xb + (long)grow * p.lnf_ldxb + gcol) = o;
            }
        }
        if (EPI == EPI_RESID_F32 && lnst) {
            const float mean = row16_sum((v[0] + v[1]) + (v[2] + v[3])) * (1.0f / 64.0f);
            const float d0 = v[0] - mean, d1 = v[1] - mean, d2 = v[2] - mean, d3 = v[3] - mean;
            const float q = row16_sum(fmaf(d0, d0, d1 * d1) + fmaf(d2, d2, d3 * d3));
            if ((lane & 15) == it) { keep_m = mean; keep_q = q; }
        }
    }
    if (EPI == EPI_RESID_F32 && lnst && (lane & 15) < 8)
        lnst[(QT * 32 + (lane & 15) * 4 + (lane >> 4)) * 4] = make_float2(keep_m, keep_q);
    asm volatile("" ::: "memory");
}

template <int QT, bool PIN>
__device__ __forceinline__ void gemm256_resid8_load(const GemmArgs& p, int m_base, int n_base, int lane, uint4 (&res)[4][2]) {
    typedef uint32_t nt_u32x4 __attribute__((ext_vector_type(4)));
    asm volatile("" : "+v"(lane));
    int gcol = n_base + (lane & 7) * 8;
    gcol = gcol < p.N ? gcol : p.N - 8;
#pragma unroll
    for (int it = 0; it < 4; ++it) {
        int grow = m_base + QT * 32 + it * 8 + (lane >> 3);
        grow = grow < p.M ? grow : p.M - 1;
        const nt_u32x4 *s0, *s1;
        if (PIN) {
            s0 = (const nt_u32x4*)(p.xp_hi + (long)grow * p.xp_ld + gcol);
            s1 = (const nt_u32x4*)(p.xp_lo + (long)grow * p.xp_ld + gcol);
        } else {
            s0 = (const nt_u32x4*)((const float*)p.C + (long)grow * p.ldc + gcol);
            s1 = s0 + 1;
        }
        res[it][0] = __builtin_bit_cast(uint4, __builtin_nontemporal_load(s0));
        res[it][1] = __builtin_bit_cast(uint4, __builtin_nontemporal_load(s1));
    }
}
__device__ __forceinline__ float row8_sum(float v) {
    v += __builtin_bit_cast(float, __builtin_amdgcn_update_dpp(0, __builtin_bit_cast(int, v), 0xB1, 0xf, 0xf, true));
    v += __builtin_bit_cast(float, __builtin_amdgcn_update_dpp(0, __builtin_bit_cast(int, v), 0x4E, 0xf, 0xf, true));
    v += __builtin_bit_cast(float, __builtin_amdgcn_update_dpp(0, __builtin_bit_cast(int, v), 0x141, 0xf, 0xf, true));
    return v;
}
template <int QT, bool PIN, bool POUT, bool ST>
__device__ __forceinline__ void gemm256_resid8_quarter(const GemmArgs& p, char* slab, int m_base, int n_base, int lane,
                                                       f32x4 (&acc)[8][4], const uint4 (&res)[4][2], float2* lnst) {
    constexpr int RS = 272;
    typedef uint32_t nt_u32x4 __attribute__((ext_vector_type(4)));
    asm volatile("" : "+v"(lane) :: "memory");
    const int lr = lane & 15, lq = lane >> 4;
#pragma unroll
    for (int m = 0; m < 2; ++m)
#pragma unroll
        for (int n = 0; n < 4; ++n) *(f32x4*)(slab + (m * 16 + lr) * RS + (n * 16 + lq * 4) * 4) = acc[QT * 2 + m][n];
    const int gcol = n_base + (lane & 7) * 8;
    float keep_m = 0.f, keep_q = 0.f;
#pragma unroll
    for (int it = 0; it < 4; ++it) {
        const int rl = it * 8 + (lane >> 3);
        const f32x4 v0 = *(const f32x4*)(slab + rl * RS + (lane & 7) * 32), v1 = *(const f32x4*)(slab + rl * RS + (lane & 7) * 32 + 16);
        float x[8] = {v0[0], v0[1], v0[2], v0[3], v1[0], v1[1], v1[2], v1[3]};
        const uint32_t a[4] = {res[it][0].x, res[it][0].y, res[it][0].z, res[it][0].w};
        const uint32_t b[4] = {res[it][1].x, res[it][1].y, res[it][1].z, res[it][1].w};
        if (PIN) {
#pragma unroll
            for (int j = 0; j < 4; ++j) {
                x[2 * j] += __uint_as_float(a[j] << 16) + __uint_as_float(b[j] << 16);
                x[2 * j + 1] += __uint_as_float(a[j] & 0xffff0000u) + __uint_as_float(b[j] & 0xffff0000u);
            }
        } else {
#pragma unroll
            for (int j = 0; j < 4; ++j) { x[j] += __uint_as_float(a[j]); x[4 + j] += __uint_as_float(b[j]); }
        }
        const int grow = m_base + QT * 32 + rl;
        if (grow < p.M && gcol < p.N) {
            uint32_t hi[4];
#pragma unroll
            for (int j = 0; j < 4; ++j) hi[j] = pack_bf16x2(x[2 * j], x[2 * j + 1]);
            if (POUT) {
                uint32_t lo[4];
#pragma unroll
                for (int j = 0; j < 4; ++j)
                    lo[j] = pack_bf16x2(x[2 * j] - __uint_as_float(hi[j] << 16), x[2 * j + 1] - __uint_as_float(hi[j] & 0xffff0000u));
                *(uint4*)(p.xp_hi + (long)grow * p.xp_ld + gcol) = make_uint4(hi[0], hi[1], hi[2], hi[3]);
                __builtin_nontemporal_store((nt_u32x4){lo[0], lo[1], lo[2], lo[3]}, (nt_u32x4*)(p.xp_lo + (long)grow * p.xp_ld + gcol));
            } else {
                float* dst = (float*)p.C + (long)grow * p.ldc + gcol;
                __builtin_nontemporal_store((f32x4){x[0], x[1], x[2], x[3]}, (f32x4*)dst);
                __builtin_nontemporal_store((f32x4){x[4], x[5], x[6], x[7]}, (f32x4*)(dst + 4));
                if (ST) *(uint4*)(p.lnf_xb + (long)grow * p.lnf_ldxb + gcol) = make_uint4(hi[0], hi[1], hi[2], hi[3]);
            }
        }
        if (ST) {
            const float mean = row8_sum(((x[0] + x[1]) + (x[2] + x[3])) + ((x[4] + x[5]) + (x[6] + x[7]))) * (1.0f / 64.0f);
            float q = 0.f;
#pragma unroll
            for (int j = 0; j < 8; ++j) { const float d = x[j] - mean; q = fmaf(d, d, q); }
            q = row8_sum(q);
            if ((lane & 7) == it) { keep_m = mean; keep_q = q; }
        }
    }
    if (ST && (lane & 7) < 4) lnst[(QT * 32 + (lane & 7) * 8 + (lane >> 3)) * 4] = make_float2(keep_m, keep_q);
    asm volatile("" ::: "memory");
}

template <int EPI, bool SKIP_DEAD = false, int XP = 0>
__device__ __forceinline__ void gemm256_epilogue(const GemmArgs& p, char* slab, int m_base, int n_base, int lane,
                                                 f32x4 (&acc)[8][4], float2* lnst = nullptr, const float2* lnmr = nullptr) {
    static_assert(EPI == EPI_BF16 || EPI == EPI_BF16_GELU || EPI == EPI_F32 || EPI == EPI_RESID_F32 ||
                  EPI == EPI_BF16_ROPE, "");
    asm volatile("" : "+v"(lane) :: "memory");
    const int lq = lane >> 4;
    f32x4 bias4[4], gamma4[4];
#pragma unroll
    for (int n = 0; n < 4; ++n) {
        const int col = n_base + n * 16 + lq * 4;
        bias4[n] = (p.bias && col < p.N) ? *(const f32x4*)(p.bias + col) : (f32x4){0.f, 0.f, 0.f, 0.f};
        if (EPI == EPI_RESID_F32)
            gamma4[n] = (p.gamma && col < p.N) ? *(const f32x4*)(p.gamma + col) : (f32x4){1.f, 1.f, 1.f, 1.f};
    }
    if (EPI == EPI_BF16 || EPI == EPI_BF16_GELU || EPI == EPI_BF16_ROPE) {
        constexpr int RS = 144;
        f32x4 c4[4];
        if (lnmr) {
#pragma unroll
            for (int n = 0; n < 4; ++n) {
                const int col = n_base + n * 16 + lq * 4;
                c4[n] = col < p.N ? *(const f32x4*)(p.lnc_c + col) : (f32x4){0.f, 0.f, 0.f, 0.f};
            }
        }
        f32x4 rtab_next[8][2];
#pragma unroll
        for (int half = 0; half < 2; ++half) {
            if (SKIP_DEAD && m_base + half * 64 >= p.M) break;
            asm volatile("" : "+v"(lane) :: "memory");
            const int lr = lane & 15, lq = lane >> 4;
            auto rope_load = [&](int hf, f32x4 (&rt)[8][2]) {
                const int gcol_ = n_base + (lane & 7) * 8;
                int tok_ = (m_base + hf * 64 + (lane >> 3)) % p.rope_S;
                const float2* cs_ = p.rope_cs + ((gcol_ % p.rope_hd) >> 1);
#pragma unroll
                for (int it = 0; it < 8; ++it) {
                    const float2* t = cs_ + (long)tok_ * (p.rope_hd >> 1);
                    rt[it][0] = *(const f32x4*)t;
                    rt[it][1] = *(const f32x4*)(t + 2);
                    tok_ += 8;
                    if (tok_ >= p.rope_S) tok_ -= p.rope_S;
                }
            };
            f32x4 rtab[8][2];
            if (EPI == EPI_BF16_ROPE) {
                if (half == 0) rope_load(0, rtab);
                else {
#pragma unroll
                    for (int it = 0; it < 8; ++it) { rtab[it][0] = rtab_next[it][0]; rtab[it][1] = rtab_next[it][1]; }
                }
            }
            auto frag_phase = [&](auto lnc_tag) {
                constexpr bool LNC = decltype(lnc_tag)::value;
#pragma unroll
                for (int m = 0; m < 4; ++m) {
                    float2 st = make_float2(1.f, 0.f);
                    if (LNC) st = lnmr[half * 64 + m * 16 + lr];
                    if (EPI == EPI_BF16_GELU) {
                        constexpr int GV = REVO_GELU_WIDTH;
#pragma unroll
                        for (int n0 = 0; n0 < 4; n0 += GV) {
                            f32x4 v[GV];
#pragma unroll
                            for (int n = 0; n < GV; ++n) {
                                if (LNC && !(REVO_LNC_ABLATE & 2)) v[n] = acc[half * 4 + m][n0 + n] * st.x + (c4[n0 + n] * st.y + bias4[n0 + n]);
                                else v[n] = acc[half * 4 + m][n0 + n] + bias4[n0 + n];
                            }
                            gelu_erf4xn<GV>(v);
#pragma unroll
                            for (int n = 0; n < GV; ++n) {
                                uint2 o;
                                o.x = pack_bf16x2(v[n][0], v[n][1]);
                                o.y = pack_bf16x2(v[n][2], v[n][3]);
                                *(uint2*)(slab + (m * 16 + lr) * RS + ((n0 + n) * 16 + lq * 4) * 2) = o;
                            }
                        }
                    } else {
#pragma unroll
                        for (int n = 0; n < 4; ++n) {
                            f32x4 v;
                            if (LNC && !(REVO_LNC_ABLATE & 2)) v = acc[half * 4 + m][n] * st.x + (c4[n] * st.y + bias4[n]);
                            else v = acc[half * 4 + m][n] + bias4[n];
                            uint2 o;
                            o.x = pack_bf16x2(v[0], v[1]);
                            o.y = pack_bf16x2(v[2], v[3]);
                            *(uint2*)(slab + (m * 16 + lr) * RS + (n * 16 + lq * 4) * 2) = o;
                        }
                    }
                }
            };
            if (lnmr) frag_phase(std::true_type{});
            else frag_phase(std::false_type{});
            if (EPI == EPI_BF16_ROPE && half == 0 && !(SKIP_DEAD && m_base + 64 >= p.M)) rope_load(1, rtab_next);
            const int gcol = n_base + (lane & 7) * 8;
#pragma unroll
            for (int it = 0; it < 8; ++it) {
                const int rl = it * 8 + (lane >> 3);
                uint4 v = *(const uint4*)(slab + rl * RS + (lane & 7) * 16);
                const int grow = m_base + half * 64 + rl;
                if (EPI == EPI_BF16_ROPE) {
                    if (gcol < p.rope_cols) {
                        uint32_t w[4] = {v.x, v.y, v.z, v.w};
#pragma unroll
                        for (int j = 0; j < 4; ++j) {
                            const float x0 = bf16_to_f32((bf16_t)(w[j] & 0xffff)), x1 = bf16_to_f32((bf16_t)(w[j] >> 16));
                            const float cx = rtab[it][j >> 1][(j & 1) * 2], cy = rtab[it][j >> 1][(j & 1) * 2 + 1];
                            w[j] = pack_bf16x2(x0 * cx - x1 * cy, x1 * cx + x0 * cy);
                        }
                        v = make_uint4(w[0], w[1], w[2], w[3]);
                    }
                }
                typedef uint32_t nt_u32x4 __attribute__((ext_vector_type(4)));
                if (EPI == EPI_BF16_ROPE || EPI == EPI_BF16_GELU) {
                    if (grow < p.M && gcol < p.N)
                        __builtin_nontemporal_store(__builtin_bit_cast(nt_u32x4, v), (nt_u32x4*)((bf16_t*)p.C + (long)grow * p.ldc + gcol));
                } else
                if (grow < p.M && gcol < p.N) *(uint4*)((bf16_t*)p.C + (long)grow * p.ldc + gcol) = v;
            }
            asm volatile("" ::: "memory");
        }
    } else {
        if (SKIP_DEAD && m_base >= p.M) return;
        if constexpr (EPI == EPI_RESID_F32 && XP != 0) {
            constexpr bool PIN = XP >= 2, POUT = XP <= 2, ST = XP <= 2;
#pragma unroll
            for (int m = 0; m < 8; ++m)
#pragma unroll
                for (int n = 0; n < 4; ++n) acc[m][n] = (acc[m][n] + bias4[n]) * gamma4[n];
            asm volatile("" ::: "memory");
            uint4 pa[4][2], pb[4][2];
            gemm256_resid8_load<0, PIN>(p, m_base, n_base, lane, pa);
            gemm256_resid8_quarter<0, PIN, POUT, ST>(p, slab, m_base, n_base, lane, acc, pa, lnst);
            gemm256_resid8_load<1, PIN>(p, m_base, n_base, lane, pa);
            gemm256_resid8_load<2, PIN>(p, m_base, n_base, lane, pb);
            gemm256_resid8_quarter<1, PIN, POUT, ST>(p, slab, m_base, n_base, lane, acc, pa, lnst);
            if (SKIP_DEAD && m_base + 64 >= p.M) return;
            gemm256_resid8_quarter<2, PIN, POUT, ST>(p, slab, m_base, n_base, lane, acc, pb, lnst);
            gemm256_resid8_load<3, PIN>(p, m_base, n_base, lane, pa);
            gemm256_resid8_quarter<3, PIN, POUT, ST>(p, slab, m_base, n_base, lane, acc, pa, lnst);
            return;
        }
        f32x4 ra[8], rb[8];
        const bool nt = lnst != nullptr;
        if (EPI == EPI_RESID_F32) gemm256_load_resid<0>(p, m_base, n_base, lane, ra, nt);
        if (EPI == EPI_RESID_F32) gemm256_load_resid<1>(p, m_base, n_base, lane, rb, nt);
        gemm256_epilogue_f32_quarter<EPI, 0>(p, slab, m_base, n_base, lane, acc, bias4, gamma4, ra, lnst);
        gemm256_epilogue_f32_quarter<EPI, 1>(p, slab, m_base, n_base, lane, acc, bias4, gamma4, rb, lnst);
        if (SKIP_DEAD && m_base + 64 >= p.M) return;
        if (EPI == EPI_RESID_F32) gemm256_load_resid<2>(p, m_base, n_base, lane, ra, nt);
        if (EPI == EPI_RESID_F32) gemm256_load_resid<3>(p, m_base, n_base, lane, rb, nt);
        gemm256_epilogue_f32_quarter<EPI, 2>(p, slab, m_base, n_base, lane, acc, bias4, gamma4, ra, lnst);
        gemm256_epilogue_f32_quarter<EPI, 3>(p, slab, m_base, n_base, lane, acc, bias4, gamma4, rb, lnst);
    }
}

constexpr int LNC_RAW_BYTES = 256 * 6 * 8 + 1024, LNC_MR_BYTES = 256 * 8;
constexpr int G256P_LN_OFF = 98304 + 5 * 9216;
static_assert(G256P_LN_OFF + LNC_RAW_BYTES + LNC_MR_BYTES <= 163840, "");
constexpr int G256_LDS_LN = G256_LDS + LNC_RAW_BYTES + LNC_MR_BYTES;
constexpr int G256Q_BC_OFF = G256_LDS_LN + LNC_MR_BYTES;
constexpr int G256Q_LDS = G256Q_BC_OFF + 2 * 2048;
static_assert(G256Q_LDS <= 163840, "");
template <class ARGS>
__device__ __forceinline__ void lnc_issue_stats(const ARGS& p, int m0, char* lds_raw, int wave, int ) {
    if (wave >= 4) return;
    int lane;
    asm volatile("v_mbcnt_lo_u32_b32 %0, -1, 0\n\tv_mbcnt_hi_u32_b32 %0, -1, %0" : "=v"(lane) :: "memory");
    const int P = p.lnc_parts;
    long left = ((long)p.M - m0) * P * 8;
    const long full = 256l * P * 8;
    left = left < 0 ? 0 : (left > full ? full : left);
    const __amdgpu_buffer_rsrc_t rs = __builtin_amdgcn_make_buffer_rsrc((void*)(p.lnc_stats + (long)m0 * P), 0, (int)left, 0x00020000);
    const int share = 512 * P, pieces = (share + 1023) >> 10;
    for (int j = 0; j < pieces; ++j) {
        const int off = wave * share + j * 1024;
        if (off + 1024 <= LNC_RAW_BYTES)
            __builtin_amdgcn_raw_ptr_buffer_load_lds(rs, (__attribute__((address_space(3))) void*)(lds_raw + off), 16,
                                                     (uint32_t)(off + lane * 16), 0, 0, 0);
    }
}
template <int VM = 4, class ARGS = GemmArgs>
__device__ __forceinline__ void lnc_merge_rows(const ARGS& p, const char* lds_raw, float2* lds_mr, int wave, int , bool one_ktile,
                                               bool tele = false, int rows_left = 0) {
    if (wave >= 4) return;
    int lane;
    asm volatile("v_mbcnt_lo_u32_b32 %0, -1, 0\n\tv_mbcnt_hi_u32_b32 %0, -1, %0" : "=v"(lane) :: "memory");
    if (one_ktile) asm volatile("s_waitcnt vmcnt(0)" ::: "memory");
    else asm volatile("s_waitcnt vmcnt(%0)" :: "n"(VM) : "memory");
    const int t = wave * 64 + lane;
    if (t < 256) {
        float r, m;
        auto merge_n = [&](auto np) {
            constexpr int NP = decltype(np)::value;
            f32x4 v[NP / 2];
#pragma unroll
            for (int i = 0; i < NP / 2; ++i) v[i] = *(const f32x4*)(lds_raw + t * (NP * 8) + i * 16);
            float sm = 0.f, sq = 0.f;
#pragma unroll
            for (int i = 0; i < NP; ++i) { sm += v[i >> 1][(i & 1) * 2]; sq += v[i >> 1][(i & 1) * 2 + 1]; }
            const float mean = sm / (float)NP;
            float dd = 0.f;
#pragma unroll
            for (int i = 0; i < NP; ++i) { const float d = v[i >> 1][(i & 1) * 2] - mean; dd = fmaf(d, d, dd); }
            const float var = fmaf((float)LNF_SLICE, dd, sq) / (float)(LNF_SLICE * NP);
            r = rsqrtf(var + p.lnc_eps);
            m = -mean * r;
        };
        if (p.lnc_parts == 4) merge_n(std::integral_constant<int, 4>{});
        else if (p.lnc_parts == 6) merge_n(std::integral_constant<int, 6>{});
        else lnf_merge((const float2*)lds_raw + t * p.lnc_parts, p.lnc_parts, p.lnc_eps, r, m);
        lds_mr[t] = make_float2(r, m);
        if (tele) {
            const int live = rows_left - wave * 64 < 0 ? 0 : (rows_left - wave * 64 > 64 ? 64 : rows_left - wave * 64);
            const float am = lane < live ? __builtin_fabsf(m) : 0.f;
            const unsigned long long big = __builtin_amdgcn_ballot_w64(am > LNC_TELE_RATIO);
            const unsigned long long huge = __builtin_amdgcn_ballot_w64(am > 4.0f * LNC_TELE_RATIO);
            if (lane == 0 && live > 0) {
                unsigned long long* tp = p.lnc_tele;
                asm volatile("" : "+v"(tp));
                atomicAdd(tp, (unsigned long long)live);
                if (big) atomicAdd(tp + 1, (unsigned long long)__builtin_popcountll(big));
                if (huge) atomicAdd(tp + 2, (unsigned long long)__builtin_popcountll(huge));
            }
        }
    }
    asm volatile("s_waitcnt lgkmcnt(0)" ::: "memory");
}
__device__ __forceinline__ void lnf_store_tile_stats(const GemmArgs& p, const float2* lds_st, int m0, int mend, int tn, int wave,
                                                     int lane) {
    asm volatile("" : "+v"(lane) :: "memory");
    const int t = wave * 64 + lane;
    if (t < 256 && m0 + t < mend) {
        const float2 a = lds_st[t * 4], b = lds_st[t * 4 + 1], c = lds_st[t * 4 + 2], d = lds_st[t * 4 + 3];
        const float mean = ((a.x + b.x) + (c.x + d.x)) * 0.25f;
        const float da = a.x - mean, db = b.x - mean, dc = c.x - mean, dd = d.x - mean;
        const float m2 = ((a.y + b.y) + (c.y + d.y)) + 64.0f * (fmaf(da, da, db * db) + fmaf(dc, dc, dd * dd));
        p.lnf_stats[(long)(m0 + t) * (p.N / LNF_SLICE) + tn] = make_float2(mean, m2);
    }
}

template <int EPI, int BN = 128>
__global__ __launch_bounds__(GEMM_THREADS) void gemm128_kernel(GemmArgs p) {
    extern __shared__ __attribute__((aligned(16))) char smem[];
    constexpr int BM = 128, MF = 4, NF = BN / 32;
    const int tiles_n = (p.N + BN - 1) / BN;
    const int tiles_m = (p.M + BM - 1) / BM;
    const int s = xcd_remap(blockIdx.x, tiles_m * tiles_n);
    const int tm = s / tiles_n, tn = s - tm * tiles_n;
    const int m0 = tm * BM, n0 = tn * BN;
    const int wave = __builtin_amdgcn_readfirstlane(threadIdx.x >> 6);
    const int lane = threadIdx.x & 63;
    const int wr = wave >> 1, wc = wave & 1;

    TileLoader<BM> la;
    TileLoader<BN> lb;
    la.init(p.A, p.lda, m0, p.M, wave, lane);
    lb.init(p.B, p.ldb, n0, p.N, wave, lane);

    f32x4 acc[MF][NF];
#pragma unroll
    for (int m = 0; m < MF; ++m)
#pragma unroll
        for (int n = 0; n < NF; ++n) acc[m][n] = (f32x4){0.f, 0.f, 0.f, 0.f};

    gemm_mainloop<BM, BN, MF, NF>(la, lb, smem, p.K, wave, lane, wr * 64, wc * (BN / 2), acc);
    gemm_epilogue<EPI, MF, NF>(p, m0 + wr * 64, n0 + wc * (BN / 2), lane, acc);
}

constexpr int G128R_NST = 6;
template <int EPI>
__global__ __launch_bounds__(GEMM_THREADS) void gemm128r_kernel(GemmArgs p) {
    extern __shared__ __attribute__((aligned(16))) char smem[];
    constexpr int BM = 128, BN = 64, MF = 4, NF = BN / 32;
    const int tiles_n = (p.N + BN - 1) / BN;
    const int tiles_m = (p.M + BM - 1) / BM;
    const int s = xcd_remap(blockIdx.x, tiles_m * tiles_n);
    const int tm = s / tiles_n, tn = s - tm * tiles_n;
    const int m0 = tm * BM, n0 = tn * BN;
    const int wave = __builtin_amdgcn_readfirstlane(threadIdx.x >> 6);
    const int lane = threadIdx.x & 63;
    const int wr = wave >> 1, wc = wave & 1;
    if (EPI == EPI_F32 && p.ksplit > 1) {
        const int nt = p.K >> 6, t0 = (int)blockIdx.y * nt / p.ksplit, t1 = ((int)blockIdx.y + 1) * nt / p.ksplit;
        p.A += t0 * 64;
        p.B += t0 * 64;
        p.K = (t1 - t0) * 64;
        p.C = (float*)p.C + (long)blockIdx.y * p.c_split_stride;
    }
    TileLoader<BM> la;
    TileLoader<BN> lb;
    la.init(p.A, p.lda, m0, p.M, wave, lane);
    lb.init(p.B, p.ldb, n0, p.N, wave, lane);
    f32x4 acc[MF][NF];
#pragma unroll
    for (int m = 0; m < MF; ++m)
#pragma unroll
        for (int n = 0; n < NF; ++n) acc[m][n] = (f32x4){0.f, 0.f, 0.f, 0.f};
    gemm_mainloop_ring<BM, BN, MF, NF, G128R_NST>(la, lb, smem, p.K, wave, lane, wr * 64, wc * (BN / 2), acc);
    gemm_epilogue<EPI, MF, NF>(p, m0 + wr * 64, n0 + wc * (BN / 2), lane, acc);
}

template <int EPI, int DBG>
__global__ __launch_bounds__(G256_THREADS, 2) void gemm256_kernel(GemmArgs p) {
    extern __shared__ __attribute__((aligned(16))) char smem[];
    const int tiles_n = (p.N + 255) / 256;
    const int tiles_m = (p.M + 255) / 256;
    const int gy = p.gy, gx = 8 / gy;
    const int xcd = blockIdx.x & 7, slot = blockIdx.x >> 3;
    const int xi = xcd / gy, xj = xcd - xi * gy;
    const int pm = (tiles_m + gx - 1) / gx, pn = (tiles_n + gy - 1) / gy;
    const int m_lo = xi * pm, n_lo = xj * pn;
    const int m_cnt = (tiles_m - m_lo) < pm ? (tiles_m - m_lo) : pm;
    const int n_cnt = (tiles_n - n_lo) < pn ? (tiles_n - n_lo) : pn;
    if (m_cnt <= 0 || n_cnt <= 0 || slot >= m_cnt * n_cnt) return;
    const int tm = m_lo + slot / n_cnt, tn = n_lo + slot % n_cnt;
    const int m0 = tm * 256, n0 = tn * 256;
    const int wave = __builtin_amdgcn_readfirstlane(threadIdx.x >> 6);
    const int lane = threadIdx.x & 63;

    if (DBG & 4) {
        const int nt = p.K >> 6, t0 = (int)blockIdx.y * nt / p.ksplit, t1 = ((int)blockIdx.y + 1) * nt / p.ksplit;
        p.A += t0 * 64;
        p.B += t0 * 64;
        p.K = (t1 - t0) * 64;
        p.C = (float*)p.C + (long)blockIdx.y * p.c_split_stride;
    }
    G256Operand A, B;
    g256_operand_init(A, p.A, p.lda, p.M, m0, wave, lane);
    g256_operand_init(B, p.B, p.ldb, p.N, n0, wave, lane);

    f32x4 acc[8][4];
#pragma unroll
    for (int m = 0; m < 8; ++m)
#pragma unroll
        for (int n = 0; n < 4; ++n) acc[m][n] = (f32x4){0.f, 0.f, 0.f, 0.f};

    const bool lnc = (EPI == EPI_BF16 || EPI == EPI_BF16_GELU || EPI == EPI_BF16_ROPE) && p.lnc_stats != nullptr;
    float2* lds_mr = (float2*)(smem + G256_LDS + LNC_RAW_BYTES);
    if (!(DBG & 2)) {
        if (lnc) lnc_issue_stats(p, m0, smem + G256_LDS, wave, lane);
        g256_issue_prologue(A, B, smem, p.K, wave);
        if (lnc) lnc_merge_rows(p, smem + G256_LDS, lds_mr, wave, lane, p.K <= 64, p.lnc_tele != nullptr && n0 == 0, p.M - m0);
        gemm256_mainloop(A, B, smem, p.K, wave, lane, acc);
    }
    if (DBG & 1) {
        if (acc[0][0][0] != 12345.678f) return;
    }
    if constexpr (EPI == EPI_PATCH) {
        gemm_epilogue<EPI, 8, 4>(p, m0 + (wave >> 2) * 128, n0 + (wave & 3) * 64, lane, acc);
    } else {
        const bool wide = (p.N & 7) == 0 && (p.ldc & 7) == 0;
        if (wide) gemm256_epilogue<EPI>(p, smem + wave * 16384, m0 + (wave >> 2) * 128, n0 + (wave & 3) * 64, lane, acc, nullptr,
                                        lnc ? lds_mr + (wave >> 2) * 128 : nullptr);
        else gemm_epilogue<EPI, 8, 4>(p, m0 + (wave >> 2) * 128, n0 + (wave & 3) * 64, lane, acc);
    }
}


constexpr int G256P_LDS = 163840;
template <int EPI, int BMR = 256, int XP = 0>
__global__ __launch_bounds__(G256_THREADS, 2) void gemm256p_kernel(GemmArgs p, int nslot) {
    static_assert(BMR == 256 || BMR == 192, "");
    extern __shared__ __attribute__((aligned(16))) char smem[];
    const int tiles_n = (p.N + 255) / 256;
    const int tiles_m = BMR == 256 ? (p.M + 255) / 256 : p.t192_tiles;
    const int tall0 = tiles_m - p.t192_tall;
    const int gy = p.gy, gx = 8 / gy;
    const int xcd = blockIdx.x & 7;
    const int xi = __builtin_amdgcn_readfirstlane(xcd / gy), xj = xcd - xi * gy;
    const int pm = __builtin_amdgcn_readfirstlane((tiles_m + gx - 1) / gx), pn = __builtin_amdgcn_readfirstlane((tiles_n + gy - 1) / gy);
    const int m_lo = xi * pm, n_lo = xj * pn;
    const int m_cnt = (tiles_m - m_lo) < pm ? (tiles_m - m_lo) : pm;
    const int n_cnt = (tiles_n - n_lo) < pn ? (tiles_n - n_lo) : pn;
    const int total = (m_cnt > 0 && n_cnt > 0) ? m_cnt * n_cnt : 0;
    int slot = blockIdx.x >> 3;
    if (slot >= total) return;
    const int wave = __builtin_amdgcn_readfirstlane(threadIdx.x >> 6);
    const int lane = threadIdx.x & 63;
    char* slab = smem + (wave < 3 ? 32768 + wave * 9216 : 98304 + (wave - 3) * 9216);
#ifdef REVO_EXPERIMENTS
    if (p.stagger_cycles > 0) {
        const int grp = (blockIdx.x >> 3) % p.stagger_groups;
        const long t0 = (long)__builtin_amdgcn_s_memrealtime();
        const long wait = (long)p.stagger_cycles * grp / p.stagger_groups;
        while ((long)__builtin_amdgcn_s_memrealtime() - t0 < wait) __builtin_amdgcn_s_sleep(8);
    }
#endif

    auto tile_row0 = [&](int mi) { return BMR == 256 ? mi * 256 : mi * 192 + (mi > tall0 ? (mi - tall0) * 16 : 0); };
    int sq = __builtin_amdgcn_readfirstlane(slot / n_cnt);
    int mi = m_lo + sq;
    int m0 = tile_row0(mi), n0 = (n_lo + (slot - sq * n_cnt)) * 256;
    bool tall = BMR != 256 && mi >= tall0;
    const bool lnc = (EPI == EPI_BF16 || EPI == EPI_BF16_GELU || EPI == EPI_BF16_ROPE) && p.lnc_stats != nullptr;
    const bool lnf = EPI == EPI_RESID_F32 && p.lnf_stats != nullptr;
    char* lds_raw = smem + G256P_LN_OFF;
    float2* lds_mr = (float2*)(smem + G256P_LN_OFF + LNC_RAW_BYTES);
    float2* lds_st = (float2*)(smem + G256P_LN_OFF);
    if (lnc) lnc_issue_stats(p, m0, lds_raw, wave, lane);
    G256Operand A, B;
    g256_operand_init(A, p.A, p.lda, p.M, m0, wave, lane, BMR == 256 ? 256 : (tall ? 208 : 192));
    g256_operand_init(B, p.B, p.ldb, p.N, n0, wave, lane);
    g256_issue_half(A, 0, 0, G256_A(smem, 0), wave);
    g256_issue_half(A, 1, 0, G256_A(smem, 0), wave);
    g256_issue_half(B, 0, 0, G256_B(smem, 0), wave);
    g256_issue_half(B, 1, 0, G256_B(smem, 0), wave);
    for (;;) {
        if (p.K > 64) {
            g256_issue_half(A, 0, 128, G256_A(smem, 1), wave);
            g256_issue_half(A, 1, 128, G256_A(smem, 1), wave);
        }
        if (lnc && !(REVO_LNC_ABLATE & 1)) lnc_merge_rows(p, lds_raw, lds_mr, wave, lane, p.K <= 64, p.lnc_tele != nullptr && n0 == 0, p.M - m0);
        f32x4 acc[8][4];
#pragma unroll
        for (int m = 0; m < 8; ++m)
#pragma unroll
            for (int n = 0; n < 4; ++n) acc[m][n] = (f32x4){0.f, 0.f, 0.f, 0.f};
        if constexpr (BMR == 256) gemm256_mainloop(A, B, smem, p.K, wave, lane, acc);
        else gemm256_mainloop<192>(A, B, smem, p.K, wave, lane, acc, tall);

        int lane_e = lane;
        if constexpr (EPI != EPI_BF16 && EPI != EPI_BF16_ROPE)
            asm volatile("v_mbcnt_lo_u32_b32 %0, -1, 0\n\tv_mbcnt_hi_u32_b32 %0, -1, %0" : "=v"(lane_e));
        const int mb = m0 + (wave >> 2) * 128, nb = n0 + (wave & 3) * 64;
        GemmArgs pe = p;
        if (BMR != 256) {
            const int mend = m0 + (tall ? 208 : 192);
            pe.M = mend < p.M ? mend : p.M;
        }
        const int m0_done = m0, tn_done = n0 >> 8;
        slot += nslot;
        const bool more = slot < total;
        if (more) {
            sq = __builtin_amdgcn_readfirstlane(slot / n_cnt);
            mi = m_lo + sq;
            m0 = tile_row0(mi);
            n0 = (n_lo + (slot - sq * n_cnt)) * 256;
            tall = BMR != 256 && mi >= tall0;
            if (lnc && !(REVO_LNC_ABLATE & 4)) lnc_issue_stats(p, m0, lds_raw, wave, lane);
            g256_operand_init(A, p.A, p.lda, p.M, m0, wave, lane, BMR == 256 ? 256 : (tall ? 208 : 192));
            g256_operand_init(B, p.B, p.ldb, p.N, n0, wave, lane);
            g256_issue_half(A, 0, 0, G256_A(smem, 0), wave);
            g256_issue_half(A, 1, 0, G256_A(smem, 0), wave);
            g256_issue_half(B, 0, 0, G256_B(smem, 0), wave);
            g256_issue_half(B, 1, 0, G256_B(smem, 0), wave);
        }
        if constexpr (EPI == EPI_PATCH) {
            gemm_epilogue<EPI, 8, 4>(pe, mb, nb, lane_e, acc);
        } else {
            const bool wide = (p.N & 7) == 0 && (p.ldc & 7) == 0;
            if (wide) gemm256_epilogue<EPI, BMR != 256, XP>(pe, slab, mb, nb, lane_e, acc,
                                                            lnf ? lds_st + (wave >> 2) * 128 * 4 + (wave & 3) : nullptr,
                                                            lnc ? lds_mr + (wave >> 2) * 128 : nullptr);
            else gemm_epilogue<EPI, 8, 4>(pe, mb, nb, lane_e, acc);
        }
        if (lnf) {
            asm volatile("s_waitcnt lgkmcnt(0)" ::: "memory");
            __builtin_amdgcn_s_barrier();
            lnf_store_tile_stats(pe, lds_st, m0_done, pe.M, tn_done, wave, lane_e);
            if (!more) break;
            continue;
        }
        if (!more) break;
        __builtin_amdgcn_s_barrier();
    }
}


template <int EPI>
__device__ __forceinline__ void gemm256q_tail(char* smem, int wave) {
    const __attribute__((address_space(4))) GemmArgs* pk0 = (const __attribute__((address_space(4))) GemmArgs*)__builtin_amdgcn_kernarg_segment_ptr();
    if (pk0->qtail_rows <= 0) return;
    const bool lnc = pk0->lnc_stats != nullptr;
    {
        const __attribute__((address_space(4))) GemmArgs& q = *pk0;
        int lane_t;
        asm volatile("v_mbcnt_lo_u32_b32 %0, -1, 0\n\tv_mbcnt_hi_u32_b32 %0, -1, %0" : "=v"(lane_t));
        const int li = lane_t & 15, lq = lane_t >> 4;
        const int tail = q.qtail_rows, Kw = q.K >> 3;
        const __amdgpu_buffer_rsrc_t ars = __builtin_amdgcn_make_buffer_rsrc((void*)(q.A + (long)q.M * q.lda), 0, (int)(tail * q.lda * 2), 0x00020000);
        float* part = (float*)smem;
        for (int strip = blockIdx.x; strip * 16 < q.N; strip += gridDim.x) {
            __builtin_amdgcn_s_barrier();
            f32x4 acc4[4];
#pragma unroll
            for (int m = 0; m < 4; ++m) acc4[m] = (f32x4){0.f, 0.f, 0.f, 0.f};
            const bf16_t* wrow = q.B + (long)(strip * 16 + li) * q.ldb + wave * Kw + lq * 8;
            const int aoff = (li * (int)q.lda + wave * Kw + lq * 8) * 2;
            for (int k0 = 0; k0 < Kw; k0 += 128) {
                bf16x8 wf[4], af[4][4];
#pragma unroll
                for (int s4 = 0; s4 < 4; ++s4) {
                    if (k0 + s4 * 32 < Kw) {
                        wf[s4] = *(const bf16x8*)(wrow + k0 + s4 * 32);
#pragma unroll
                        for (int m = 0; m < 4; ++m)
                            af[s4][m] = __builtin_bit_cast(bf16x8, __builtin_amdgcn_raw_buffer_load_b128(ars, aoff + (m * 16 * (int)q.lda + k0 + s4 * 32) * 2, 0, 0));
                    }
                }
#pragma unroll
                for (int s4 = 0; s4 < 4; ++s4)
                    if (k0 + s4 * 32 < Kw) {
#pragma unroll
                        for (int m = 0; m < 4; ++m) acc4[m] = __builtin_amdgcn_mfma_f32_16x16x32_bf16(wf[s4], af[s4][m], acc4[m], 0, 0, 0);
                    }
            }
#pragma unroll
            for (int m = 0; m < 4; ++m) *(f32x4*)(part + (wave * 64 + m * 16 + li) * 16 + lq * 4) = acc4[m];
            __builtin_amdgcn_s_barrier();
            if (wave < 4) {
                const int tt = wave * 64 + lane_t;
                const int row = tt >> 2, cq = tt & 3;
                f32x4 v = *(const f32x4*)(part + row * 16 + cq * 4);
#pragma unroll
                for (int w = 1; w < 8; ++w) v += *(const f32x4*)(part + (w * 64 + row) * 16 + cq * 4);
                if (row < tail) {
                    const int col = strip * 16 + cq * 4;
                    const long grow = (long)q.M + row;
                    const f32x4 b4 = q.bias ? *(const f32x4*)(q.bias + col) : (f32x4){0.f, 0.f, 0.f, 0.f};
                    if (lnc) {
                        float rstd, mr;
                        lnf_merge(q.lnc_stats + grow * q.lnc_parts, q.lnc_parts, q.lnc_eps, rstd, mr);
                        if (q.lnc_tele && strip == 0 && cq == 0) {
                            unsigned long long* tp = q.lnc_tele;
                            asm volatile("" : "+v"(tp));
                            const float am = __builtin_fabsf(mr);
                            atomicAdd(tp, 1ull);
                            if (am > LNC_TELE_RATIO) atomicAdd(tp + 1, 1ull);
                            if (am > 4.0f * LNC_TELE_RATIO) atomicAdd(tp + 2, 1ull);
                        }
                        const f32x4 c = *(const f32x4*)(q.lnc_c + col);
                        v = v * rstd + (c * mr + b4);
                    } else {
                        v += b4;
                    }
                    if (EPI == EPI_BF16_GELU) v = gelu_erf4(v);
                    uint2 o;
                    o.x = pack_bf16x2(v[0], v[1]);
                    o.y = pack_bf16x2(v[2], v[3]);
                    *(uint2*)((bf16_t*)q.C + grow * q.ldc + col) = o;
                }
            }
        }
    }
}

constexpr int G256Q_STORES = 16;
template <int EPI>
__global__ __launch_bounds__(G256_THREADS, 2) void gemm256q_kernel(GemmArgs p, int nslot) {
    static_assert(EPI == EPI_BF16 || EPI == EPI_BF16_GELU || EPI == EPI_BF16_ROPE, "");
    extern __shared__ __attribute__((aligned(16))) char smem[];
    const int tiles_n = p.N >> 8;
    const int tiles_m = (p.M + 255) >> 8;
    const int gy = p.gy, gx = 8 / gy;
    const int xcd = blockIdx.x & 7;
    const int xi = __builtin_amdgcn_readfirstlane(xcd / gy), xj = xcd - xi * gy;
    const int pm = __builtin_amdgcn_readfirstlane((tiles_m + gx - 1) / gx), pn = __builtin_amdgcn_readfirstlane((tiles_n + gy - 1) / gy);
    const int m_lo = xi * pm, n_lo = xj * pn;
    const int m_cnt = (tiles_m - m_lo) < pm ? (tiles_m - m_lo) : pm;
    const int n_cnt = (tiles_n - n_lo) < pn ? (tiles_n - n_lo) : pn;
    const int total = (m_cnt > 0 && n_cnt > 0) ? m_cnt * n_cnt : 0;
    int slot = blockIdx.x >> 3;
    const int wave = __builtin_amdgcn_readfirstlane(threadIdx.x >> 6);
    if (slot >= total) {
        gemm256q_tail<EPI>(smem, wave);
        return;
    }
    const int lane = threadIdx.x & 63;

    int sq = __builtin_amdgcn_readfirstlane(slot / n_cnt);
    int m0 = (m_lo + sq) * 256, n0 = (n_lo + (slot - sq * n_cnt)) * 256;
    const bool lnc = p.lnc_stats != nullptr;
    char* lds_raw = smem + G256_LDS;
    float2* lds_mr = (float2*)(smem + G256_LDS + LNC_RAW_BYTES);
    float2* lds_mr_next = lds_mr + 256;
    char* lds_bc = smem + G256Q_BC_OFF;
    char* lds_bc_next = lds_bc + 2048;
    auto issue_bias_csum = [&](const float* bias, const float* csum, int N, int n0_, char* dst, int lane_) {
        if (wave == 4 || wave == 5) {
            const float* src = wave == 4 ? bias : csum;
            const __amdgpu_buffer_rsrc_t rs = __builtin_amdgcn_make_buffer_rsrc((void*)(src + n0_), 0, src ? (N - n0_ < 256 ? N - n0_ : 256) * 4 : 0, 0x00020000);
            __builtin_amdgcn_raw_ptr_buffer_load_lds(rs, (__attribute__((address_space(3))) void*)(dst + (wave - 4) * 1024), 16,
                                                     (uint32_t)(lane_ * 16), 0, 0, 0);
        }
    };
    if (lnc) lnc_issue_stats(p, m0, lds_raw, wave, lane);
    issue_bias_csum(p.bias, lnc ? p.lnc_c : nullptr, p.N, n0, lds_bc, lane);
    G256Operand A, B;
    g256_operand_init(A, p.A, p.lda, p.M, m0, wave, lane);
    g256_operand_init(B, p.B, p.ldb, p.N, n0, wave, lane);
    g256_issue_prologue(A, B, smem, p.K, wave);
    G256_FENCE();
    {
        const __amdgpu_buffer_rsrc_t none = __builtin_amdgcn_make_buffer_rsrc(p.C, 0, 0, 0x00020000);
        typedef uint32_t u32x4 __attribute__((ext_vector_type(4)));
#pragma unroll
        for (int i = 0; i < G256Q_STORES; ++i)
            __builtin_amdgcn_raw_buffer_store_b128((u32x4){0u, 0u, 0u, 0u}, none, i * 16, 0, 0);
    }
    G256_FENCE();
#ifdef REVO_EXPERIMENTS
    int tiles_done = 0;
#endif
    if (lnc) lnc_merge_rows<G256Q_STORES>(p, lds_raw, lds_mr, wave, lane, false, p.lnc_tele != nullptr && n0 == 0, p.M - m0);
    else if (threadIdx.x < 512) lds_mr[threadIdx.x] = make_float2(1.f, 0.f);
    for (;;) {
        f32x4 acc[8][4];
#pragma unroll
        for (int m = 0; m < 8; ++m)
#pragma unroll
            for (int n = 0; n < 4; ++n) acc[m][n] = (f32x4){0.f, 0.f, 0.f, 0.f};
#ifdef REVO_EXPERIMENTS
        unsigned long long t_a = 0, t_b = 0, t_c = 0, c_a = 0;
        if (p.stamps) { t_a = __builtin_amdgcn_s_memrealtime(); c_a = __builtin_amdgcn_s_memtime(); }
#endif
        gemm256_mainloop<0, false, false, G256Q_STORES>(A, B, smem, p.K, wave, lane, acc);
#ifdef REVO_EXPERIMENTS
        if (p.stamps) { t_b = __builtin_amdgcn_s_memrealtime(); c_a = __builtin_amdgcn_s_memtime() - c_a; }
#endif

        const __attribute__((address_space(4))) GemmArgs* pk = (const __attribute__((address_space(4))) GemmArgs*)__builtin_amdgcn_kernarg_segment_ptr();
        asm volatile("" : "+s"(pk));
        const __attribute__((address_space(4))) GemmArgs& q = *pk;
        int lane_e;
        asm volatile("v_mbcnt_lo_u32_b32 %0, -1, 0\n\tv_mbcnt_hi_u32_b32 %0, -1, %0" : "=v"(lane_e));
        const int lr = lane_e & 15, lq = lane_e >> 4;
        const int wr = wave >> 2, wc = wave & 3;
        const int m0_done = m0, n0_done = n0;
        const int nb = n0_done + wc * 64;
        slot += nslot;
        const bool more = slot < total;
        float2 st8[8];
#pragma unroll
        for (int m = 0; m < 8; ++m) st8[m] = lds_mr[wr * 128 + m * 16 + lr];
        f32x4 bias4[4], c4[4];
#pragma unroll
        for (int n = 0; n < 4; ++n) {
            bias4[n] = *(const f32x4*)(lds_bc + (wc * 64 + n * 16 + lq * 4) * 4);
            c4[n] = *(const f32x4*)(lds_bc + 1024 + (wc * 64 + n * 16 + lq * 4) * 4);
        }
        asm volatile("s_waitcnt lgkmcnt(0)" ::: "memory");
        G256_FENCE();
        const bool rot = EPI == EPI_BF16_ROPE && nb < q.rope_cols;
        __amdgpu_buffer_rsrc_t rtab = __builtin_amdgcn_make_buffer_rsrc((void*)q.rope_cs, 0, EPI == EPI_BF16_ROPE ? q.rope_S * (q.rope_hd >> 1) * 8 : 0, 0x00020000);
        int tok = 0, cpair[4] = {0, 0, 0, 0};
        if (EPI == EPI_BF16_ROPE) {
            tok = (m0_done + wr * 128 + lr) % q.rope_S;
            int c0 = (nb + lq * 4) % q.rope_hd;
#pragma unroll
            for (int n = 0; n < 4; ++n) {
                cpair[n] = (c0 >> 1) * 8;
                c0 += 16;
                if (c0 >= q.rope_hd) c0 -= q.rope_hd;
            }
        }
        const int tok_row_bytes = (q.rope_hd >> 1) * 8;
        f32x4 rt[2][2][4];
        auto rope_load = [&](auto bufc) {
            constexpr int buf = decltype(bufc)::value;
#pragma unroll
            for (int mm = 0; mm < 2; ++mm) {
#pragma unroll
                for (int n = 0; n < 4; ++n)
                    rt[buf][mm][n] = __builtin_bit_cast(f32x4, __builtin_amdgcn_raw_buffer_load_b128(rtab, tok * tok_row_bytes + cpair[n], 0, 0));
                tok += 16;
                if (tok >= q.rope_S) tok -= q.rope_S;
            }
        };
        using I0 = std::integral_constant<int, 0>; using I1 = std::integral_constant<int, 1>;
        using I2 = std::integral_constant<int, 2>; using I3 = std::integral_constant<int, 3>;
        if (rot) { rope_load(I0{}); rope_load(I1{}); }
        if (rot) {
#pragma unroll
            for (int i = 0; i < 2; ++i)
#pragma unroll
                for (int mm = 0; mm < 2; ++mm)
#pragma unroll
                    for (int n = 0; n < 4; ++n) asm volatile("" : "+v"(rt[i][mm][n]));
        }
        G256_FENCE();
        if (more) {
            sq = __builtin_amdgcn_readfirstlane(slot / n_cnt);
            m0 = (m_lo + sq) * 256;
            n0 = (n_lo + (slot - sq * n_cnt)) * 256;
            if (lnc) lnc_issue_stats(q, m0, lds_raw, wave, lane_e);
            issue_bias_csum(q.bias, lnc ? q.lnc_c : nullptr, q.N, n0, lds_bc_next, lane_e);
            g256_operand_init(A, q.A, q.lda, q.M, m0, wave, lane_e);
            g256_operand_init(B, q.B, q.ldb, q.N, n0, wave, lane_e);
            g256_issue_prologue(A, B, smem, q.K, wave);
        }
        G256_FENCE();
        typedef uint32_t u32x2 __attribute__((ext_vector_type(2)));
        typedef uint32_t u32x4 __attribute__((ext_vector_type(4)));
        const long rows_here = (long)q.M - m0_done < 256 ? (long)q.M - m0_done : 256;
#ifdef REVO_EXPERIMENTS
        const bool drop_stores = (q.stagger_groups & 0x100) != 0;
#else
        constexpr bool drop_stores = false;
#endif
        const __amdgpu_buffer_rsrc_t crs = __builtin_amdgcn_make_buffer_rsrc(
            (void*)((bf16_t*)q.C + (long)m0_done * q.ldc + n0_done), 0, drop_stores ? 0 : (int)((rows_here - 1) * q.ldc * 2 + 512), 0x00020000);
        const int rstep = (int)(q.ldc * 32);
        int voff = (wr * 128 + lr) * (int)(q.ldc * 2) + (wc * 64 + (lq & 1) * 16 + (lq >> 1) * 8) * 2;
        auto quarter = [&](auto qc, auto bufc) {
            u32x4 out[2][2];
            constexpr int q = decltype(qc)::value, buf = decltype(bufc)::value;
#pragma unroll
            for (int mm = 0; mm < 2; ++mm) {
                constexpr int dummy_ = 0; (void)dummy_;
                const int m = q * 2 + mm;
                const float2 st = st8[m];
                uint32_t d[4][2];
#pragma unroll
                for (int n0f = 0; n0f < 4; n0f += 2) {
                    f32x4 v[2];
#pragma unroll
                    for (int n = 0; n < 2; ++n) v[n] = acc[m][n0f + n] * st.x + (c4[n0f + n] * st.y + bias4[n0f + n]);
                    if (EPI == EPI_BF16_GELU) gelu_erf4xn<2>(v);
#pragma unroll
                    for (int n = 0; n < 2; ++n) {
                        uint32_t w0 = pack_bf16x2(v[n][0], v[n][1]), w1 = pack_bf16x2(v[n][2], v[n][3]);
                        if (EPI == EPI_BF16_ROPE) {
                            if (rot) {
                                const f32x4 tc = rt[buf][mm][n0f + n];
                                const float a0 = __uint_as_float(w0 << 16), a1 = __uint_as_float(w0 & 0xffff0000u);
                                const float b0 = __uint_as_float(w1 << 16), b1 = __uint_as_float(w1 & 0xffff0000u);
                                w0 = pack_bf16x2(a0 * tc[0] - a1 * tc[1], a1 * tc[0] + a0 * tc[1]);
                                w1 = pack_bf16x2(b0 * tc[2] - b1 * tc[3], b1 * tc[2] + b0 * tc[3]);
                            }
                        }
                        d[n0f + n][0] = w0;
                        d[n0f + n][1] = w1;
                    }
                }
#pragma unroll
                for (int P = 0; P < 2; ++P) {
                    const u32x2 s0 = __builtin_amdgcn_permlane16_swap(d[2 * P][0], d[2 * P + 1][0], false, false);
                    const u32x2 s1 = __builtin_amdgcn_permlane16_swap(d[2 * P][1], d[2 * P + 1][1], false, false);
                    out[mm][P] = (u32x4){s0[0], s1[0], s0[1], s1[1]};
                }
            }
            G256_FENCE();
#pragma unroll
            for (int mm = 0; mm < 2; ++mm) {
                constexpr int aux = (EPI == EPI_BF16_ROPE || EPI == EPI_BF16_GELU) ? 2 : 0;
                __builtin_amdgcn_raw_buffer_store_b128(out[mm][0], crs, voff, 0, aux);
                __builtin_amdgcn_raw_buffer_store_b128(out[mm][1], crs, voff + 64, 0, aux);
                voff += rstep;
            }
            G256_FENCE();
        };
#ifdef REVO_EXPERIMENTS
        if (q.stamps) t_c = __builtin_amdgcn_s_memrealtime();
#endif
        quarter(I0{}, I0{});
        if (rot) rope_load(I0{});
        quarter(I1{}, I1{});
        if (rot) rope_load(I1{});
        quarter(I2{}, I0{});
        quarter(I3{}, I1{});
        G256_FENCE();
#ifdef REVO_EXPERIMENTS
        if (q.stamps && wave == 0 && lane_e == 0 && tiles_done < q.stamp_items) {
            unsigned long long* dst = q.stamps + ((size_t)blockIdx.x * q.stamp_items + tiles_done) * 4;
            dst[0] = t_a; dst[1] = t_b; dst[2] = (q.stagger_groups & 0x200) ? c_a : t_c; dst[3] = __builtin_amdgcn_s_memrealtime();
        }
        ++tiles_done;
#endif
        if (!more) break;
        if (lnc) {
            lnc_merge_rows<G256Q_STORES>(q, lds_raw, lds_mr_next, wave, lane_e, false, q.lnc_tele != nullptr && n0 == 0, q.M - m0);
        }
        { float2* t = lds_mr; lds_mr = lds_mr_next; lds_mr_next = t; }
        { char* t = lds_bc; lds_bc = lds_bc_next; lds_bc_next = t; }
    }
    gemm256q_tail<EPI>(smem, wave);
}

#ifdef REVO_EXPERIMENTS
template <int EPI, int BMR = 256>
__global__ __launch_bounds__(G256_THREADS, 2) void gemm256pp_kernel(GemmArgs p, int nslot, int groups) {
    static_assert(BMR == 256 || BMR == 192, "");
    extern __shared__ __attribute__((aligned(16))) char smem[];
    const int tiles_n = (p.N + 255) / 256;
    const int tiles_m = BMR == 256 ? (p.M + 255) / 256 : p.t192_tiles;
    const int tall0 = tiles_m - (BMR == 256 ? 0 : p.t192_tall);
    const int gy = p.gy, gx = 8 / gy;
    const int xcd = blockIdx.x & 7;
    const int xi = xcd / gy, xj = xcd - xi * gy;
    const int pm = (tiles_m + gx - 1) / gx, pn = (tiles_n + gy - 1) / gy;
    const int m_lo = xi * pm, n_lo = xj * pn;
    const int m_cnt = (tiles_m - m_lo) < pm ? (tiles_m - m_lo) : pm;
    const int n_cnt = (tiles_n - n_lo) < pn ? (tiles_n - n_lo) : pn;
    const int total = (m_cnt > 0 && n_cnt > 0) ? m_cnt * n_cnt : 0;
    const int slot0 = blockIdx.x >> 3;
    if (slot0 >= total) return;
    const int wave = __builtin_amdgcn_readfirstlane(threadIdx.x >> 6);
    const int lane = threadIdx.x & 63;
    const int wr = wave >> 2;
    char* slab = smem + (wave < 3 ? 32768 + wave * 9216 : 98304 + (wave - 3) * 9216);

    auto tile_row0 = [&](int mi) { return BMR == 256 ? mi * 256 : mi * 192 + (mi > tall0 ? (mi - tall0) * 16 : 0); };
    const int ntiles = (total - slot0 + nslot - 1) / nslot;
    const int grp = (slot0 / n_cnt) % groups;
    const int h = 64 * (((grp + 1) * (BMR / 64) + groups - 1) / groups);
    const bool first_tall = BMR != 256 && (m_lo + slot0 / n_cnt) >= tall0;
    const bool split = h < BMR && ntiles >= 2 && !first_tall;
    const int nitems = ntiles + (split ? 1 : 0);

    int m0, n0, rows;
    auto item = [&](int it) {
        const bool last_piece = split && it == nitems - 1;
        const int s = last_piece ? slot0 : slot0 + it * nslot;
        const int mi = m_lo + s / n_cnt;
        n0 = (n_lo + s % n_cnt) * 256;
        m0 = tile_row0(mi);
        rows = BMR == 256 ? 256 : (mi >= tall0 ? 208 : 192);
        if (split && it == 0) rows = h;
        if (last_piece) { m0 += h; rows = BMR - h; }
    };
    item(0);
    G256Operand A, B;
    g256_operand_init(A, p.A, p.lda, p.M, m0, wave, lane, rows);
    g256_operand_init(B, p.B, p.ldb, p.N, n0, wave, lane);
    g256_issue_half(A, 0, 0, G256_A(smem, 0), wave);
    g256_issue_half(A, 1, 0, G256_A(smem, 0), wave);
    g256_issue_half(B, 0, 0, G256_B(smem, 0), wave);
    g256_issue_half(B, 1, 0, G256_B(smem, 0), wave);
    for (int it = 0;;) {
        if (p.K > 64) {
            g256_issue_half(A, 0, 128, G256_A(smem, 1), wave);
            g256_issue_half(A, 1, 128, G256_A(smem, 1), wave);
        }
        f32x4 acc[8][4];
#pragma unroll
        for (int m = 0; m < 8; ++m)
#pragma unroll
            for (int n = 0; n < 4; ++n) acc[m][n] = (f32x4){0.f, 0.f, 0.f, 0.f};
        const bool do_lo = wr == 0 ? true : rows > 128;
        const bool do_hi = wr == 0 ? rows > 64 : rows >= 256;
        const bool do_ht = wr == 1 && rows == 208;
#ifdef REVO_EXPERIMENTS
        unsigned long long t_a = 0, t_b = 0;
        if (p.stamps) t_a = __builtin_amdgcn_s_memrealtime();
#endif
        gemm256_mainloop<0, true>(A, B, smem, p.K, wave, lane, acc, do_ht, do_lo, do_hi);
#ifdef REVO_EXPERIMENTS
        if (p.stamps) t_b = __builtin_amdgcn_s_memrealtime();
#endif

        const int mb = m0 + wr * 128, nb = n0 + (wave & 3) * 64;
        GemmArgs pe = p;
        {
            const int mend = m0 + rows;
            pe.M = mend < p.M ? mend : p.M;
        }
#ifdef REVO_EXPERIMENTS
        const int it_done = it, rows_done = rows;
#endif
        ++it;
        const bool more = it < nitems;
        if (more) {
            item(it);
            g256_operand_init(A, p.A, p.lda, p.M, m0, wave, lane, rows);
            g256_operand_init(B, p.B, p.ldb, p.N, n0, wave, lane);
            g256_issue_half(A, 0, 0, G256_A(smem, 0), wave);
            g256_issue_half(A, 1, 0, G256_A(smem, 0), wave);
            g256_issue_half(B, 0, 0, G256_B(smem, 0), wave);
            g256_issue_half(B, 1, 0, G256_B(smem, 0), wave);
        }
        if constexpr (EPI == EPI_PATCH) {
            gemm_epilogue<EPI, 8, 4>(pe, mb, nb, lane, acc);
        } else {
            const bool wide = (p.N & 7) == 0 && (p.ldc & 7) == 0;
            if (wide) gemm256_epilogue<EPI, true>(pe, slab, mb, nb, lane, acc);
            else gemm_epilogue<EPI, 8, 4>(pe, mb, nb, lane, acc);
        }
#ifdef REVO_EXPERIMENTS
        if (p.stamps && wave == 0 && lane == 0 && it_done < p.stamp_items) {
            unsigned long long* dst = p.stamps + ((size_t)blockIdx.x * p.stamp_items + it_done) * 4;
            dst[0] = t_a; dst[1] = t_b; dst[2] = __builtin_amdgcn_s_memrealtime(); dst[3] = (unsigned long long)rows_done;
        }
#endif
        if (!more) break;
        __builtin_amdgcn_s_barrier();
    }
}
#endif

template <int EPI, int NW, int DEPTH, int MY>
__global__ __launch_bounds__(NW * 64) void gemm_skinny_kernel(GemmArgs p) {
    constexpr int MFR = MY == 1 ? 4 : 1;
    __shared__ f32x4 red[NW - 1][MFR][64];
    const int wave = threadIdx.x >> 6, lane = threadIdx.x & 63;
    const int lr = lane & 15, lq = lane >> 4;
    const int n0 = blockIdx.x * 16;
    const int m0 = MY == 1 ? 0 : (int)blockIdx.y * 16;
    const int kw = p.K / NW;
    const int nrow = n0 + lr < p.N ? n0 + lr : p.N - 1;
    const bf16_t* bp = p.B + (long)nrow * p.ldb + wave * kw + lq * 8;
    const bf16_t* ap[MFR];
#pragma unroll
    for (int m = 0; m < MFR; ++m) {
        const int row = m0 + m * 16 + lr < p.M ? m0 + m * 16 + lr : p.M - 1;
        ap[m] = p.A + (long)row * p.lda + wave * kw + lq * 8;
    }
    f32x4 acc[MFR][1];
#pragma unroll
    for (int m = 0; m < MFR; ++m) acc[m][0] = (f32x4){0.f, 0.f, 0.f, 0.f};
    for (int k = 0; k < kw; k += 64 * DEPTH) {
        bf16x8 b[2 * DEPTH], a[2 * DEPTH][MFR];
#pragma unroll
        for (int u = 0; u < 2 * DEPTH; ++u) {
            b[u] = *(const bf16x8*)(bp + k + u * 32);
#pragma unroll
            for (int m = 0; m < MFR; ++m) a[u][m] = *(const bf16x8*)(ap[m] + k + u * 32);
        }
#pragma unroll
        for (int u = 0; u < 2 * DEPTH; ++u)
#pragma unroll
            for (int m = 0; m < MFR; ++m)
                acc[m][0] = __builtin_amdgcn_mfma_f32_16x16x32_bf16(b[u], a[u][m], acc[m][0], 0, 0, 0);
    }
    if (wave > 0) {
#pragma unroll
        for (int m = 0; m < MFR; ++m) red[wave - 1][m][lane] = acc[m][0];
    }
    __syncthreads();
    if (wave == 0) {
#pragma unroll
        for (int w = 0; w < NW - 1; ++w)
#pragma unroll
            for (int m = 0; m < MFR; ++m) acc[m][0] += red[w][m][lane];
        gemm_epilogue<EPI, MFR, 1>(p, m0, n0, lane, acc);
    }
}

static const char* check_args(const GemmArgs& a) {
    if (a.K <= 0 || a.K % GEMM_BK) return "gemm: K must be a positive multiple of 64";
    if (a.N % 4) return "gemm: N must be a multiple of 4";
    if (a.M <= 0 || a.N <= 0) return "gemm: empty problem";
    if (a.lda % 8 || a.ldb % 8) return "gemm: lda/ldb must be multiples of 8 (16-byte rows)";
    if (a.ldc % 4) return "gemm: ldc must be a multiple of 4";
    if (((uintptr_t)a.A | (uintptr_t)a.B | (uintptr_t)a.C) & 15) return "gemm: operands must be 16-byte aligned";
    return nullptr;
}

#ifdef REVO_EXPERIMENTS
static unsigned g_forms = 0;
#define REVO_FORM(bit) (g_forms |= (bit))
unsigned gemm_debug_forms(int reset) { const unsigned f = g_forms; if (reset) g_forms = 0; return f; }
#else
#define REVO_FORM(bit) ((void)0)
#endif
static int xcd_stripes(int tiles_n) { return tiles_n >= 24 ? 4 : (tiles_n >= 8 ? 2 : 1); }
static int g_force_gy = 0;
void gemm_force_gy(int gy) { g_force_gy = gy; }
template <int EPI, int DBG>
static int launch_256d(const GemmArgs& a, hipStream_t st) {
    REVO_FUNC_LDS((gemm256_kernel<EPI, DBG>), G256_LDS_LN);
    GemmArgs b = a;
    const int tiles_m = (a.M + 255) / 256, tiles_n = (a.N + 255) / 256;
    int gy = xcd_stripes(tiles_n);
    if (g_force_gy) gy = g_force_gy;
    b.gy = gy;
    const int gx = 8 / gy;
    const int region = ((tiles_m + gx - 1) / gx) * ((tiles_n + gy - 1) / gy);
    hipLaunchKernelGGL((gemm256_kernel<EPI, DBG>), dim3(8 * region), dim3(G256_THREADS), G256_LDS_LN, st, b);
    REVO_FORM(GF_256_TILE);
    REVO_HIP_CHECK(hipGetLastError());
    return 0;
}

#ifdef REVO_EXPERIMENTS
static int g_stagger_cycles = 0, g_stagger_groups = 2;
void gemm_set_stagger(int cycles, int groups) { g_stagger_cycles = cycles; g_stagger_groups = groups < 1 ? 1 : groups; }
#endif
static int g_persistent = 1;
void gemm_set_persistent(int on) { g_persistent = on; }
#ifdef REVO_EXPERIMENTS
static int g_phase_groups = 0;
void gemm_set_phase_groups(int g) { g_phase_groups = g < 0 ? 0 : (g > 4 ? 4 : g); }
static unsigned long long* g_stamps = nullptr; static int g_stamp_items = 0;
void gemm_set_stamps(unsigned long long* buf, int items) { g_stamps = buf; g_stamp_items = items; }
#endif
template <int EPI, int BMR = 256>
static int launch_256p(const GemmArgs& a, hipStream_t st) {
    GemmArgs b = a;
#ifdef REVO_EXPERIMENTS
    b.stagger_cycles = g_stagger_cycles; b.stagger_groups = g_stagger_groups;
    b.stamps = g_stamps; b.stamp_items = g_stamp_items;
#endif
    const int tiles_m = BMR == 256 ? (a.M + 255) / 256 : a.t192_tiles, tiles_n = (a.N + 255) / 256;
    REVO_FORM(BMR == 256 ? GF_256P : GF_256P_192);
    if (EPI == EPI_RESID_F32 && b.xp_in) REVO_FORM(GF_PLANES_IN);
    if (EPI == EPI_RESID_F32 && b.xp_out) REVO_FORM(GF_PLANES_OUT);
    int gy = xcd_stripes(tiles_n);
    if (g_force_gy) gy = g_force_gy;
    b.gy = gy;
    const int gx = 8 / gy;
    const int region = ((tiles_m + gx - 1) / gx) * ((tiles_n + gy - 1) / gy);
    int nslot = region < 32 ? region : 32;
#ifdef REVO_EXPERIMENTS
    if (const char* e = getenv("REVO_GEMM_NSLOT")) { const int v = atoi(e); if (v >= 1 && v < nslot) nslot = v; }
    {
        int groups = g_phase_groups > 1 ? g_phase_groups : 1;
        if (BMR != 256 && groups > 3) groups = 3;
        if (groups > 1 || b.stamps != nullptr) {
            REVO_FUNC_LDS((gemm256pp_kernel<EPI, BMR>), G256P_LDS);
            hipLaunchKernelGGL((gemm256pp_kernel<EPI, BMR>), dim3(8 * nslot), dim3(G256_THREADS), G256P_LDS, st, b, nslot, groups);
            REVO_HIP_CHECK(hipGetLastError());
            return 0;
        }
    }
#endif
    if constexpr (EPI == EPI_RESID_F32) {
        const int xp = (b.xp_in || b.xp_out) ? (b.xp_in ? (b.xp_out ? 2 : 3) : 1) : 0;
        if (xp && ((b.N & 7) || (b.ldc & 7))) { revo_set_error("gemm: planes need the row-coalesced epilogue"); return -2; }
#define REVO_LAUNCH_XP(X)                                                                                              \
    case X:                                                                                                             \
        REVO_FUNC_LDS((gemm256p_kernel<EPI, BMR, X>), G256P_LDS);                                                       \
        hipLaunchKernelGGL((gemm256p_kernel<EPI, BMR, X>), dim3(8 * nslot), dim3(G256_THREADS), G256P_LDS, st, b, nslot); \
        break;
        switch (xp) { REVO_LAUNCH_XP(1) REVO_LAUNCH_XP(2) REVO_LAUNCH_XP(3) default: break; }
#undef REVO_LAUNCH_XP
        if (xp) { REVO_HIP_CHECK(hipGetLastError()); return 0; }
    }
    REVO_FUNC_LDS((gemm256p_kernel<EPI, BMR>), G256P_LDS);
    hipLaunchKernelGGL((gemm256p_kernel<EPI, BMR>), dim3(8 * nslot), dim3(G256_THREADS), G256P_LDS, st, b, nslot);
    REVO_HIP_CHECK(hipGetLastError());
    return 0;
}
#ifdef REVO_EXPERIMENTS
static int g_dbg = 0;
void gemm_set_debug(int d) { g_dbg = d; }
#endif
static int g_qtail = 1;
static int g_qstores = 1;
void gemm_set_qstores(int on) { g_qstores = on & 31; g_qtail = !(on & 32); }
#ifdef REVO_EXPERIMENTS
constexpr bool G256Q_ROPE_BUILT = true;
#else
constexpr bool G256Q_ROPE_BUILT = false;
#endif
template <int EPI>
static bool use_256q(const GemmArgs& a) {
    if (!(EPI == EPI_BF16 || EPI == EPI_BF16_GELU || (EPI == EPI_BF16_ROPE && G256Q_ROPE_BUILT)) || !g_qstores) return false;
    if (a.N % 256 || a.K < 128 || (a.ldc & 7) || 256l * a.ldc * 2 >= (1l << 31)) return false;
    if (EPI == EPI_BF16_ROPE && (a.rope_cols % 64 || (long)a.rope_S * (a.rope_hd >> 1) * 8 >= (1l << 31))) return false;
    if (EPI == EPI_BF16_ROPE && (g_qstores & 7) != 3) return false;
    return true;
}
template <int EPI>
static int launch_256q(const GemmArgs& a, hipStream_t st) {
    if constexpr (EPI == EPI_BF16 || EPI == EPI_BF16_GELU || (EPI == EPI_BF16_ROPE && G256Q_ROPE_BUILT)) {
        GemmArgs b = a;
#ifdef REVO_EXPERIMENTS
        b.stamps = g_stamps; b.stamp_items = g_stamp_items;
        b.stagger_cycles = 0;
        b.stagger_groups = ((g_qstores & 7) == 2 ? 0x100 : 0)
                           | ((g_qstores & 8) ? 0x200 : 0);
#endif
        const int tiles_m = (a.M + 255) / 256, tiles_n = a.N / 256;
        int gy = xcd_stripes(tiles_n);
        if (g_force_gy) gy = g_force_gy;
        b.gy = gy;
        const int gx = 8 / gy;
        const int region = ((tiles_m + gx - 1) / gx) * ((tiles_n + gy - 1) / gy);
        const int nslot = region < 32 ? region : 32;
        REVO_FUNC_LDS((gemm256q_kernel<EPI>), G256Q_LDS);
        hipLaunchKernelGGL((gemm256q_kernel<EPI>), dim3(8 * nslot), dim3(G256_THREADS), G256Q_LDS, st, b, nslot);
        REVO_FORM(b.qtail_rows > 0 ? GF_256Q_QTAIL : GF_256Q);
        REVO_HIP_CHECK(hipGetLastError());
        return 0;
    } else {
        revo_set_error("gemm: internal: queued stores with a non-bf16 epilogue");
        return -3;
    }
}
template <int EPI>
static int launch_256(const GemmArgs& a, hipStream_t st) {
#ifdef REVO_EXPERIMENTS
    if (EPI == EPI_BF16 && g_dbg) {
        switch (g_dbg) {
            case 1: return launch_256d<EPI_BF16, 1>(a, st);
            case 2: return launch_256d<EPI_BF16, 2>(a, st);
            default: return launch_256d<EPI_BF16, 3>(a, st);
        }
    }
#endif
    if (g_persistent && a.K >= 128 && (long)((a.M + 255) / 256) * ((a.N + 255) / 256) > 256) {
#ifdef REVO_EXPERIMENTS
        if (use_256q<EPI>(a) && (a.qtail_rows > 0 || (g_phase_groups <= 1 && g_stagger_cycles == 0))) return launch_256q<EPI>(a, st);
#else
        if (use_256q<EPI>(a)) return launch_256q<EPI>(a, st);
#endif
        return launch_256p<EPI>(a, st);
    }
    return launch_256d<EPI, 0>(a, st);
}

static int g_force_tile = 0;
void gemm_force_tile(int t) { g_force_tile = t; }

static int g_min_tiles256 = 100;
void gemm_set_min_tiles256(int n) { g_min_tiles256 = n; }
static bool use_256(const GemmArgs& a) {
    if (256l * a.lda * 2 >= (1l << 31) || 256l * a.ldb * 2 >= (1l << 31)) return false;
    if (g_force_tile == 256) return true;
    if (g_force_tile == 128) return false;
    return a.M >= 1024 && a.N >= 256 && (long)((a.M + 255) / 256) * ((a.N + 255) / 256) >= g_min_tiles256;
}

bool gemm_uses_wide_epilogue(int M, int N, long lda, long ldb, long ldc) {
    GemmArgs a{};
    a.M = M; a.N = N; a.lda = lda; a.ldb = ldb;
    return use_256(a) && (N & 7) == 0 && (ldc & 7) == 0;
}

template <int EPI>
static int launch_128(const GemmArgs& a, hipStream_t st);

static int g_ring = 1, g_ring_max_tiles = 256;
void gemm_set_ring(int on, int max_tiles) { g_ring = on; if (max_tiles > 0) g_ring_max_tiles = max_tiles; }
static int g_tail_split = 1;
void gemm_set_tail_split(int on) { g_tail_split = on; }

__global__ __launch_bounds__(256) void splitk_reduce_resid_kernel(const float* __restrict__ ws, int S, long plane,
                                                                  int rows, int N, const float* __restrict__ bias,
                                                                  const float* __restrict__ gamma,
                                                                  float* __restrict__ x, long ldc) {
    const long i = ((long)blockIdx.x * 256 + threadIdx.x) * 4;
    if (i >= (long)rows * N) return;
    const int r = (int)(i / N), c = (int)(i - (long)r * N);
    f32x4 v = *(const f32x4*)(ws + i);
    for (int s = 1; s < S; ++s) v += *(const f32x4*)(ws + (long)s * plane + i);
    if (bias) v += *(const f32x4*)(bias + c);
    if (gamma) v *= *(const f32x4*)(gamma + c);
    float* dst = x + (long)r * ldc + c;
    *(f32x4*)dst = *(const f32x4*)dst + v;
}
template <int MAXG>
__global__ __launch_bounds__(256) void splitk_reduce_resid_ln_kernel(const float* __restrict__ ws, int S, long plane, int rows, int N,
                                                                     const float* __restrict__ bias, const float* __restrict__ gamma,
                                                                     float* __restrict__ x, long ldc, const float* __restrict__ lw,
                                                                     const float* __restrict__ lb, float eps,
                                                                     bf16_t* __restrict__ h, long ldo) {
    const int lane = threadIdx.x & 63;
    const int row = blockIdx.x * 4 + (threadIdx.x >> 6);
    if (row >= rows) return;
    const int ngroup = N >> 3;
    f32x4 v[MAXG][2];
    float s = 0.f;
#pragma unroll
    for (int i = 0; i < MAXG; ++i) {
        const int g = lane + 64 * i;
        if (g < ngroup) {
#pragma unroll
            for (int hh = 0; hh < 2; ++hh) {
                const long e = (long)row * N + g * 8 + hh * 4;
                f32x4 t = *(const f32x4*)(ws + e);
                for (int p2 = 1; p2 < S; ++p2) t += *(const f32x4*)(ws + (long)p2 * plane + e);
                if (bias) t += *(const f32x4*)(bias + g * 8 + hh * 4);
                if (gamma) t *= *(const f32x4*)(gamma + g * 8 + hh * 4);
                float* dst = x + (long)row * ldc + g * 8 + hh * 4;
                t = *(const f32x4*)dst + t;
                *(f32x4*)dst = t;
                v[i][hh] = t;
            }
            s += ((v[i][0][0] + v[i][0][1]) + (v[i][0][2] + v[i][0][3])) + ((v[i][1][0] + v[i][1][1]) + (v[i][1][2] + v[i][1][3]));
        } else {
            v[i][0] = v[i][1] = (f32x4){0.f, 0.f, 0.f, 0.f};
        }
    }
    const float mean = wave_sum(s) / (float)N;
    float q = 0.f;
#pragma unroll
    for (int i = 0; i < MAXG; ++i) {
        const int g = lane + 64 * i;
        if (g < ngroup) {
#pragma unroll
            for (int hh = 0; hh < 2; ++hh)
#pragma unroll
                for (int j = 0; j < 4; ++j) {
                    const float d = v[i][hh][j] - mean;
                    q = fmaf(d, d, q);
                }
        }
    }
    const float rstd = rsqrtf(wave_sum(q) / (float)N + eps);
#pragma unroll
    for (int i = 0; i < MAXG; ++i) {
        const int g = lane + 64 * i;
        if (g < ngroup) {
            float y[8];
#pragma unroll
            for (int hh = 0; hh < 2; ++hh) {
                const f32x4 gm = lw ? *(const f32x4*)(lw + g * 8 + hh * 4) : (f32x4){1.f, 1.f, 1.f, 1.f};
                const f32x4 be = lb ? *(const f32x4*)(lb + g * 8 + hh * 4) : (f32x4){0.f, 0.f, 0.f, 0.f};
#pragma unroll
                for (int j = 0; j < 4; ++j) y[hh * 4 + j] = fmaf((v[i][hh][j] - mean) * rstd, gm[j], be[j]);
            }
            uint4 o;
            o.x = pack_bf16x2(y[0], y[1]);
            o.y = pack_bf16x2(y[2], y[3]);
            o.z = pack_bf16x2(y[4], y[5]);
            o.w = pack_bf16x2(y[6], y[7]);
            *(uint4*)(h + (long)row * ldo + g * 8) = o;
        }
    }
}
static int g_splitk = 1;
void gemm_set_splitk(int on) { g_splitk = on; }
static int try_splitk_tail(const GemmArgs& a, hipStream_t st) {
    if (!g_splitk || !a.ws || a.N % 4 || a.K < 1024) return 0;
    const int tiles_m = (a.M + 255) / 256, tiles_n = (a.N + 255) / 256, nt = a.K / 64;
    {
        const int tiles64 = ((a.M + 127) / 128) * ((a.N + 63) / 64);
        const bool with_ln = a.ln_out && a.ln_fused && a.N % 8 == 0 && a.N <= 2048 && a.ln_ldo % 8 == 0;
        int S = g_ring && a.N % 64 == 0 ? 256 / tiles64 : 0;
        S = S > 8 ? 8 : S;
        while (S > 1 && nt / S < (with_ln ? 4 : 8)) --S;
        if (a.K < 2048 && !with_ln) S = 0;
        const long plane = (long)a.M * a.N;
        if (S >= 2 && plane * S <= a.ws_elems) {
            constexpr int LDS = G128R_NST * (128 + 64) * 128;
            REVO_FUNC_LDS((gemm128r_kernel<EPI_F32>), LDS);
            GemmArgs b = a;
            b.C = a.ws; b.ldc = a.N; b.bias = nullptr; b.gamma = nullptr;
            b.ksplit = S; b.c_split_stride = plane;
            hipLaunchKernelGGL((gemm128r_kernel<EPI_F32>), dim3(tiles64, S), dim3(GEMM_THREADS), LDS, st, b);
            REVO_HIP_CHECK(hipGetLastError());
            if (with_ln) {
                const dim3 grid((unsigned)((a.M + 3) / 4));
                const int groups = (a.N / 8 + 63) / 64;
#define RLN_LAUNCH(G) hipLaunchKernelGGL((splitk_reduce_resid_ln_kernel<G>), grid, dim3(256), 0, st, a.ws, S, plane, a.M, a.N, a.bias, \
                                         a.gamma, (float*)a.C, a.ldc, a.ln_w, a.ln_b, a.ln_eps, a.ln_out, a.ln_ldo)
                if (groups <= 1) RLN_LAUNCH(1);
                else if (groups <= 2) RLN_LAUNCH(2);
                else if (groups <= 3) RLN_LAUNCH(3);
                else RLN_LAUNCH(4);
#undef RLN_LAUNCH
                REVO_FORM(GF_SPLITK_RING_LN);
                REVO_HIP_CHECK(hipGetLastError());
                *a.ln_fused = 1;
                return 1;
            }
            const long quads = plane / 4;
            hipLaunchKernelGGL(splitk_reduce_resid_kernel, dim3((unsigned)((quads + 255) / 256)), dim3(256), 0, st, a.ws, S, plane,
                               a.M, a.N, a.bias, a.gamma, (float*)a.C, a.ldc);
            REVO_FORM(GF_SPLITK_RING);
            REVO_HIP_CHECK(hipGetLastError());
            return 1;
        }
    }
    if (a.K < 2048) return 0;
    int gy = 1, per = 1 << 30;
    for (int g : {1, 2, 4, 8}) {
        const int pm = (tiles_m + 8 / g - 1) / (8 / g), pn = (tiles_n + g - 1) / g;
        if (pm * pn < per) { per = pm * pn; gy = g; }
    }
    int S = 32 / per;
    S = S > 8 ? 8 : S;
    while (S > 1 && nt / S < 8) --S;
    if (S < 2) return 0;
    const long plane = (long)a.M * a.N;
    if (plane * S > a.ws_elems) return 0;
    REVO_FUNC_LDS((gemm256_kernel<EPI_F32, 4>), G256_LDS);
    GemmArgs b = a;
    b.C = a.ws; b.ldc = a.N; b.bias = nullptr; b.gamma = nullptr;
    b.ksplit = S; b.c_split_stride = plane;
    b.gy = gy;
    hipLaunchKernelGGL((gemm256_kernel<EPI_F32, 4>), dim3(8 * per, S), dim3(G256_THREADS), G256_LDS, st, b);
    REVO_HIP_CHECK(hipGetLastError());
    const long quads = plane / 4;
    hipLaunchKernelGGL(splitk_reduce_resid_kernel, dim3((unsigned)((quads + 255) / 256)), dim3(256), 0, st, a.ws, S, plane,
                       a.M, a.N, a.bias, a.gamma, (float*)a.C, a.ldc);
    REVO_FORM(GF_SPLITK_256);
    REVO_HIP_CHECK(hipGetLastError());
    return 1;
}

static bool use_skinny(const GemmArgs& a) { return g_force_tile == 0 && a.M <= 64 && a.K % 256 == 0 && a.N >= 256; }

static int g_rows192 = 1;
void gemm_set_rows192(int on) { g_rows192 = on; }
static int plan_rows192(const GemmArgs& a, bool can_split_tail, int* tall) {
    if (!g_rows192 || g_force_tile || a.K < 128 || a.M % 16) return 0;
    const long tn = (a.N + 255) / 256, T = a.M / 192, e = (a.M - T * 192) / 16;
    if (e > T || e > 8) return 0;
    const long tiles192 = T * tn, rounds192 = (tiles192 + 255) / 256;
    if (tiles192 <= 256 || rounds192 * 256 - tiles192 > tiles192 / 32) return 0;
    const long tiles = ((a.M + 255) / 256) * tn, full = tiles / 256, rem = tiles % 256;
    double cost256 = (double)full;
    if (rem) cost256 += (can_split_tail && g_tail_split && full > 0 && rem <= 160) ? (rem > 77 ? rem / 128.0 : 0.6) : 1.0;
    const double cost192 = rounds192 * 0.75 * 1.06 + (e ? 0.0625 : 0.0);
    if (cost192 >= cost256) return 0;
    *tall = (int)e;
    return (int)T;
}
template <int EPI>
static int launch_skinny(const GemmArgs& a, hipStream_t st) {
    if (a.K % 1024 == 0 && a.N <= 2048) {
        hipLaunchKernelGGL((gemm_skinny_kernel<EPI, 4, 4, 4>), dim3((a.N + 15) / 16, (a.M + 15) / 16), dim3(256), 0, st, a);
        REVO_FORM(GF_SKINNY_444);
    } else {
        hipLaunchKernelGGL((gemm_skinny_kernel<EPI, 4, 1, 1>), dim3((a.N + 15) / 16), dim3(256), 0, st, a);
        REVO_FORM(GF_SKINNY_411);
    }
    REVO_HIP_CHECK(hipGetLastError());
    return 0;
}

static int g_lnf = 1;
static int g_ln_planes = 1;
void gemm_set_ln_fold(int on) { g_lnf = on != 0; g_ln_planes = on != 2; }
bool gemm_ln_planes_enabled() { return g_lnf && g_ln_planes; }
static int resid_fold_form(const GemmArgs& a, int* t192 = nullptr, int* tall = nullptr) {
    if (!g_lnf || g_force_tile || a.N % LNF_SLICE || a.N / LNF_SLICE > 6 || (a.ldc & 7)) return 0;
    if (a.prefer256 || 256l * a.lda * 2 >= (1l << 31) || 256l * a.ldb * 2 >= (1l << 31)) return 0;
    const long tm = (a.M + 255) / 256, tn = (a.N + 255) / 256, tiles = tm * tn;
    if (a.M > 64 && a.K >= 1024 && tiles <= 96) return 0;
    if (use_skinny(a) || !use_256(a)) return 0;
    int tl = 0;
    if (const int t = plan_rows192(a, true, &tl)) {
        if (t192) *t192 = t;
        if (tall) *tall = tl;
        return 1;
    }
// ... 177 lines not shown
```

### revers-o_amd/csrc/kernels.h

```cpp
#pragma once
#include "common.h"

namespace revo {

enum GemmEpi {
    EPI_BF16 = 0,
    EPI_BF16_GELU = 1,
    EPI_RESID_F32 = 2,
    EPI_F32 = 3,
    EPI_PATCH = 4,
    EPI_BF16_ROPE = 5,
};

struct GemmArgs {
    const bf16_t* A; long lda;
    const bf16_t* B; long ldb;
    int M, N, K;
    void* C; long ldc;
    const float* bias;
    const float* gamma;
    const float* pos;
    int S, G2, cls;
    int gy;
    const float2* rope_cs;
    int rope_S, rope_hd, rope_cols;
    int prefer256;
    float* ws; long ws_elems;
    int t192_tiles, t192_tall;
    int ksplit; long c_split_stride;
    const float* ln_w; const float* ln_b; float ln_eps; bf16_t* ln_out; long ln_ldo; int* ln_fused;
    bf16_t* lnf_xb; long lnf_ldxb; float2* lnf_stats; int* lnf_done;
    bf16_t* xp_hi; bf16_t* xp_lo; long xp_ld; int xp_in, xp_out;
    const float2* lnc_stats; int lnc_parts; const float* lnc_c; float lnc_eps;
    unsigned long long* lnc_tele;
    int qtail_rows;
#ifdef REVO_EXPERIMENTS
    int stagger_cycles, stagger_groups;
    unsigned long long* stamps; int stamp_items;
#endif
};
constexpr float LNC_TELE_RATIO = 8.0f;
bool gemm_uses_wide_epilogue(int M, int N, long lda, long ldb, long ldc);
int launch_gemm(int epi, const GemmArgs& a, hipStream_t st);
enum GemmForm : unsigned {
    GF_SKINNY_444 = 1u << 0,
    GF_SKINNY_411 = 1u << 1,
    GF_128_128 = 1u << 2,
    GF_128_64 = 1u << 3,
    GF_128R = 1u << 4,
    GF_256_TILE = 1u << 5,
    GF_256P = 1u << 6,
    GF_256P_192 = 1u << 7,
    GF_256Q = 1u << 8,
    GF_256Q_QTAIL = 1u << 9,
    GF_SPLITK_RING = 1u << 10,
    GF_SPLITK_RING_LN = 1u << 11,
    GF_SPLITK_256 = 1u << 12,
    GF_LN_FOLDED = 1u << 13,
    GF_LN_CONSUMED = 1u << 14,
    GF_PLANES_IN = 1u << 15,
    GF_PLANES_OUT = 1u << 16,
};
#ifdef REVO_EXPERIMENTS
unsigned gemm_debug_forms(int reset);
#endif
int launch_gemm_f32_ring(const GemmArgs& a, hipStream_t st);
bool gemm_resid_folds(int M, int N, int K, long lda, long ldb, long ldc);
int launch_planes_to_f32(const bf16_t* hi, const bf16_t* lo, long ldp, float* x, long ldx, long rows, int W, hipStream_t st);
#ifdef REVO_EXPERIMENTS
void gemm_set_debug(int d);
void gemm_set_stagger(int cycles, int groups);
void gemm_set_stamps(unsigned long long* buf, int items);
void gemm_set_phase_groups(int g);
#endif
void gemm_force_gy(int gy);
void gemm_set_tail_split(int on);
void gemm_force_tile(int t);

constexpr int LN_MAXH = 16;
struct LnLogits { const float* qk; const float* ck; float* logits; int H, S; };
int launch_layernorm(const float* x, long ldx, const float* w, const float* b, float eps, int rows, int W,
                     void* out, long ldo, int out_is_bf16, hipStream_t st, const LnLogits* logits = nullptr);
int launch_fold_ln_linear(const float* w, const float* gamma, const float* beta, const float* bias, int rows, int cols,
                          bf16_t* out, long ld, float* csum, float* bias_out, hipStream_t st);
int launch_patchify(const void* images, int is_u8, int B, int img, int P, bf16_t* out, long Kp, hipStream_t st);
int launch_probe_qk(const float* q, const float* Wk, const float* bk, int W, int heads, float* qk, float* ck, hipStream_t st);
int launch_pool_head_rows(const float* x, long ldx, int B, int S, int W, int H, const float* logits, float* u, hipStream_t st);
int launch_gemm_f32_skinny(int epi, const float* A, long lda, long a_group_stride, int group_cols, const float* Wt, long ldw,
                           const float* bias, int M, int N, int K, float* C, long ldc, hipStream_t st);
int launch_transpose_f32(const float* src, int rows, int cols, float* dst, hipStream_t st);
int launch_split_hi_lo_hi(const float* src, long rows, int cols, float scale, bf16_t* dst, long ld, hipStream_t st);
int launch_cls_rows(float* x, long ldx, const float* cls, const float* pos, int B, int S, int W, hipStream_t st);
int launch_rope(bf16_t* qkv, long ld, const float2* cs, int rows, int S, int W, int heads, hipStream_t st);
int launch_f32_to_bf16(const float* src, long ld_src, bf16_t* dst, long ld_dst, long rows, int cols, hipStream_t st);
int launch_l2norm_rows(const float* src, long ld_src, float* dst_f32, long ld_f32, bf16_t* dst_bf16, long ld_bf16,
                       long rows, int D, hipStream_t st, int normalize = 1, float* row_stats = nullptr,
                       uint32_t* max_stats = nullptr, uint32_t* zero_a = nullptr, long zero_a_words = 0,
                       uint32_t* zero_b = nullptr, long zero_b_words = 0, const long long* dst_rows = nullptr);

constexpr long REMOVE_MAX_CHUNK = 65536;
int launch_remove_count(const uint32_t* bits, long N, long chunk, uint32_t* cnt, uint32_t* first, hipStream_t st);
int launch_remove_gather(const uint32_t* bits, long N, long row0, long len, long j0, const uint4* src, uint4* dst,
                         int u4_per_row, hipStream_t st);

int launch_attention(const bf16_t* qkv, long ld, bf16_t* out, long ldo, int B, int S, int H, int hd, hipStream_t st);
int launch_attention_ex(const bf16_t* qkv, long ld, bf16_t* out, long ldo, int B, int S, int H, int hd, int has_cls,
                        hipStream_t st);
void gemm_set_min_tiles256(int n);
void gemm_set_ring(int on, int max_tiles);
void gemm_set_splitk(int on);
void gemm_set_persistent(int on);
void gemm_set_qstores(int on);
void gemm_set_rows192(int on);
void gemm_set_ln_fold(int on);
bool gemm_ln_planes_enabled();
void attention_force_nw(int nw);
void attention_set_shape16(int on);
#ifdef REVO_EXPERIMENTS
void attention_set_clock_buffer(unsigned long long* buf);
#endif

struct ScanArgs {
    const bf16_t* Qb; long ldq;
    const bf16_t* Gb; long ldg;
    int Q; long N; int D;
    int ksel;
    int splits;
    uint64_t* part;
    const uint32_t* allow;
};
int topk_scan_workspace_splits(int Q, long N);
int launch_topk_scan(const ScanArgs& a, hipStream_t st);
int launch_topk_reduce(uint64_t* part, int Q, int splits, int ksel, hipStream_t st);
constexpr int EXACT_COL_CAP = 2048;
constexpr int EXACT_L3_SLICES = 32;
static_assert(EXACT_L3_SLICES * 64 == EXACT_COL_CAP, "the brute-force partial lists live in the collect buffer");
enum ExactCtr : int {
    CTR_UNCERTIFIED,
    CTR_BRUTEFORCE,
    CTR_CHECKED,
    CTR_COLLECTED,
    CTR_MODE3_FAILED,
    CTR_FROM_SEGS,
    CTR_GROUPED,
    CTR_LARGE_FALLBACK,
    CTR_PAIR_PASSES,
    CTR_SLOTS
};
struct ExactWs {
    int* ctr;
    int* unc_q;
    float* unc_lb;
    bf16_t* qb_u;
    long ldqb;
    int* col_cnt;
    uint64_t* col;
    int* over_j;
    int* orow;
    int cap;
};
constexpr int GROUP_K1 = 50;
struct GroupWs {
    const int* group_of_row;
    int* gq;
    int* chosen;
    int hits;
    int has_thr; float thr;
};
struct GroupOut {
    float* scores; long long* idx;
    int* hit_counts; int* group_ids;
    int* group_counts;
    int limit, group_size;
    long idx_offset;
};
int launch_topk_group_select(const float* s1, const long long* i1, const int* c1, int Q, const ExactWs& ws, const GroupWs& gw,
                             int force_fallback, const GroupOut& o, hipStream_t st);
int launch_topk_group_fallback(const ExactWs& ws, GroupWs gw, int max_entries, const float* Qf, long ldqf, const float* Gf,
                               long ldgf, long N, int D, const uint32_t* allow, const GroupOut& o, hipStream_t st);
struct SegSrc { const uint64_t* seg; const int* cnt; int splits, q0, nq; };
struct CertArgs {
    const float* qstat;
    const uint32_t* gstat;
    int mode;
    ExactWs ws;
    const bf16_t* Qb; long ldq;
    float* cert_out;
    SegSrc segs[2]; int nsegs;
    int seg_ksel;
    const uint64_t* prelist;
    const uint32_t* tau_base;
    int estimated;
    const float* marg;
    const int* dropflag;
};
int launch_cert_margin(const float* qstat, const uint32_t* gstat, int D, int Q, float* marg, int* dropflag, hipStream_t st);
int launch_topk_finish(const uint64_t* part, long part_stride, int ksel, const float* Qf, long ldqf, const float* Gf,
                       long ldgf, int D, int Q, int k, int has_thr, float thr, long idx_offset, const uint32_t* all_bounds,
                       int parts, int top_m, float* out_scores, long long* out_idx, int* out_counts, const CertArgs* cert,
                       hipStream_t st);
__host__ __device__ inline float cert_eps(float e_q, float n_qb, float G, float Eg, int D) {
    const float gam1 = (float)D * 1.1920929e-7f;
    const float gam2 = (float)D * 5.9604645e-8f;
    const float eps = e_q * G + n_qb * Eg + gam1 * n_qb * (G + Eg) + gam2 * (n_qb + e_q) * G;
    return eps * 1.001f + 1e-30f;
}
struct Collect256Args {
    const bf16_t* Qb; long ldq;
    const bf16_t* Gb; long ldg;
    long N; int D;
    int splits, small_modes;
    const int* n_q;
    const float* lb;
    int* cnt;
    uint64_t* col;
    int cap;
    const uint32_t* allow;
};
int launch_topk_collect256(const Collect256Args& a, int max_queries, hipStream_t st);
int launch_topk_exact_finish(const ExactWs& ws, int max_entries, const float* Qf, long ldqf, const float* Gf, long ldgf,
                             int D, int k, int has_thr, float thr, long idx_offset, int force_bruteforce, int out_compact,
                             float* out_scores, long long* out_idx, int* out_counts, hipStream_t st);
int launch_topk_exact_bruteforce(const ExactWs& ws, int max_entries, const float* Qf, long ldqf, const float* Gf, long ldgf,
                                 long N, int D, int k, int has_thr, float thr, long idx_offset, int out_compact,
                                 float* out_scores, long long* out_idx, int* out_counts, hipStream_t st,
                                 const uint32_t* allow = nullptr);
int launch_topk_exact_prepare(const ExactWs& ws, const int* q_idx, const float* need, int n, const CertArgs& cert, int D,
                              const uint64_t* cand, long cand_stride, int ksel, hipStream_t st);
int launch_topk_publish(const uint64_t* part, long part_stride, int Q, int top_m, uint32_t* bounds, hipStream_t st);
int topk_scan256_splits(int Q, long rows);
int topk_scan256_main_queries(int Q, long rows);
long topk_scan256_plan_dump(int Q, long rows, long* out, int cap);
int topk_scan256_hist_buckets();
int topk_scan256_hist_shift();
#ifdef REVO_EXPERIMENTS
void topk_scan256_set_debug(int d);
unsigned long long* topk_scan256_stats();
#endif
int launch_topk_scan256(const bf16_t* Qb, long ldq, const bf16_t* Gb, long ldg, int Q, long N, int D, long n_begin,
                        int splits, uint64_t* seg, int* seg_cnt, uint32_t* tau_g, const uint32_t* tau_base, uint32_t* hist,
                        int ksel, hipStream_t st, const float* marg = nullptr, int* dropflag = nullptr,
                        const uint32_t* allow = nullptr);
int launch_topk_reduce_segs(const uint64_t* seg, const int* seg_cnt, int splits, const uint64_t* prelist, uint64_t* out,
                            int Q, int ksel, hipStream_t st, uint32_t* bounds = nullptr, int top_m = 0);
int launch_topk_select_rows(const float* scores, long ld, int n, int Q, uint64_t* part, long part_row_stride, int slot,
                            uint32_t* tau0, int ksel, uint32_t* hist, int hist_buckets, int hist_shift, hipStream_t st,
                            uint32_t* tau_copy = nullptr, float est_z = 0.f, const uint32_t* allow = nullptr);
constexpr int LARGE_K_MAX = 1024;
constexpr int LARGE_NB = 4096;
constexpr int LARGE_CAP = 8192;
constexpr int LARGE_LVL = 8;
constexpr int LARGE_FB_SLICES = 256;
struct LargeWs {
    float* lvl;
    uint32_t* hist;
    int* ctr;
    int* band_q; float* band_lb; int* band_cnt;
    bf16_t* band_qb;
    uint64_t* band_col;
    int* fb_q;
    float* fb_scores;
    int F;
    int* stats;
};
struct LargeCountArgs {
    const bf16_t* Qb; long ldq; const bf16_t* Gb; long ldg;
    long N; int D, nq, splits;
    const float* lvl; uint32_t* hist;
    const uint32_t* allow;
};
int launch_topk_large_sample(const float* pre, long ld, int n_s, const uint32_t* allow, const float* qstat, const uint32_t* gstat,
                             int D, int Q, int k, int has_thr, float thr, const LargeWs& ws, hipStream_t st);
int launch_topk_large_count(const bf16_t* Qb, long ldq, const bf16_t* Gb, long ldg, long N, int D, int Q, const LargeWs& ws,
                            const uint32_t* allow, hipStream_t st);
int launch_topk_large_level(const LargeWs& ws, const bf16_t* Qb, long ldq, int D, int Q, int k, int force_fallback, hipStream_t st);
int launch_topk_large_finish(const LargeWs& ws, int max_entries, const float* Qf, long ldqf, const float* Gf, long ldgf, int D,
                             int k, int has_thr, float thr, long idx_offset, float* out_scores, long long* out_idx,
                             int* out_counts, hipStream_t st);
int launch_topk_large_fallback(const LargeWs& ws, int max_entries, const float* Qf, long ldqf, const float* Gf, long ldgf, long N,
                               int D, int k, int has_thr, float thr, long idx_offset, float* out_scores, long long* out_idx,
                               int* out_counts, const uint32_t* allow, hipStream_t st);
constexpr int SORT_MAX_BLOCKS = 2048;
int launch_sort_keys_u64(uint64_t* keys, float* vals, uint64_t* keys_alt, float* vals_alt, long n, int key_bits, uint32_t* cnt,
                         uint64_t** out_keys, float** out_vals, hipStream_t st);
int launch_inclusive_sums_u64(unsigned long long* c, long n, hipStream_t st);
constexpr long PAIRS_WS_KEYS = 1l << 20;
constexpr long PAIRS_MAX_CAND = 1l << 28;
struct PairsJoinArgs {
    const bf16_t* Gb; long ldg;
    long N; int D;
    long T, pairs;
    const uint32_t* gstat;
    float thr;
    const uint32_t* allow;
    unsigned long long* cnt;
    uint64_t* keys; long cap;
};
int launch_pairs_join(const PairsJoinArgs& a, hipStream_t st);
int pairs_join_plan(PairsJoinArgs& a, const char* who, long* wgs);
int launch_pairs_rescore(const uint64_t* cand, long n, const float* Gf, long ldg, int D, float thr, int b,
                         unsigned long long* kept, uint64_t* out_keys, float* out_scores, hipStream_t st);
int launch_pairs_emit(const uint64_t* keys, const float* vals, long n, int b, long long* pairs, float* scores, hipStream_t st);
struct ClustersJoinArgs {
    PairsJoinArgs j;
    uint32_t* parent;
};
int launch_clusters_init(uint32_t* parent, uint32_t* sizes, long N, unsigned long long* ctr4, hipStream_t st);
int launch_clusters_join(const ClustersJoinArgs& a, hipStream_t st);
int launch_clusters_rescore(const uint64_t* cand, long n, const float* Gf, long ldg, int D, float thr, uint32_t* parent,
                            long N, hipStream_t st);
int launch_clusters_labels(uint32_t* parent, const uint32_t* allow, long N, int b, long long* labels, uint32_t* sizes,
                           uint64_t* keys, unsigned long long* ctr4, hipStream_t st);
int launch_clusters_emit(const uint64_t* keys, long n, long n_clusters, int b, unsigned long long* rank, long long* members,
                         long long* offsets, hipStream_t st);
constexpr int RANGE_CHUNK = 1024;
constexpr long RANGE_WS_PER_QUERY = 1024;
constexpr long RANGE_MAX_CAND = 1l << 28;
constexpr int RANGE_PHASES = 8;
struct RangeJoinArgs {
    const bf16_t* Qb; long ldq;
    const bf16_t* Gb; long ldg;
    int Q; long N; int D;
    const float* qstat;
    const uint32_t* gstat;
    float thr;
    const uint32_t* allow;
    unsigned long long* cnt;
    uint64_t* keys; long cap;
    int nph;
    int ph_first[RANGE_PHASES + 1], ph_q0[RANGE_PHASES], ph_qn[RANGE_PHASES], ph_ns[RANGE_PHASES];
};
int launch_range_join(const RangeJoinArgs& a, hipStream_t st);
int launch_range_rescore(const uint64_t* cand, long n, const float* Qf, long ldq, const float* Gf, long ldg, int D, float thr,
                         int b, unsigned long long* kept, unsigned long long* counts, uint64_t* out_keys, float* out_scores,
                         hipStream_t st);
int launch_range_emit(const uint64_t* keys, const float* vals, long n, int b, long idx_offset, long long* idx, float* scores,
                      hipStream_t st);
constexpr int RECOMMEND_MAX_EXAMPLES = 128;
struct RecommendPassArgs {
    const bf16_t* Qb; long ldq;
    const bf16_t* Gb; long ldg;
    int P, Nn;
    long N; int D;
    const float* qstat;
    const uint32_t* gstat;
    const uint32_t* allow;
    const float* tau;
    unsigned long long* cnt;
    uint32_t* rows; long cap;
    float* lb_out;
};
int launch_recommend_pass(const RecommendPassArgs& a, int sample, hipStream_t st);
int launch_recommend_level(const float* lb, int n, int k, int has_thr, float thr, float* tau, hipStream_t st);
int launch_recommend_rescore(const uint32_t* cand, long n, const float* Qf, long ldq, int P, int Nn, const float* Gf, long ldg,
                             int D, int has_thr, float thr, int b, unsigned long long* kept, uint64_t* out_keys, float* out_scores,
                             hipStream_t st);
int launch_recommend_emit(const uint64_t* keys, const float* vals, long n, int k, int b, long idx_offset, float* scores,
                          long long* idx, int* counts, hipStream_t st);
constexpr int DISCOVER_MAX_PAIRS = 64;
struct DiscoverPassArgs {
    const bf16_t* Qb; long ldq;
    const bf16_t* Gb; long ldg;
    int n_pairs, has_target;
    long N; int D;
    const float* qstat;
    const uint32_t* gstat;
    const uint32_t* allow;
// ... 80 lines not shown
```

Before: 2496.

## Stage factored 2D RoPE axis table in LDS for QKV GEMM epilogue

Builds a small per-axis cos/sin table (G x head_dim/4) on the host and, when the grid shape fits, copies it into spare LDS at kernel start so the QKV GEMM epilogue rotates from LDS instead of loading the full per-position rope table from global memory. Row and column grid coordinates are tracked incrementally per lane, with a special identity entry for the unrotated CLS row. Shapes that do not fit fall back to the XP=1 kernel variant. In exchange it adds LDS setup per block, more index arithmetic in the epilogue, and register-pressure hints.

```diff
diff --git a/include/revo.h b/include/revo.h
--- a/include/revo.h
+++ b/include/revo.h
@@ -122,6 +122,10 @@
 int32_t revo_op_gemm_resid_norm(const void* a_bf16, int64_t lda, const void* b_bf16, int64_t ldb, int32_t m, int32_t n, int32_t k,
                                 float* c, int64_t ldc, const float* bias, const float* gamma, void* ln_out_bf16, int64_t ln_ldo,
                                 float eps, int32_t* fused, void* stream);
+int32_t revo_op_gemm_rope_axis(const void* a_bf16, int64_t lda, const void* b_bf16, int64_t ldb, int32_t m, int32_t n, int32_t k,
+                               void* c_bf16, int64_t ldc, const float* bias, const float* csum, const void* stats, int32_t parts,
+                               float eps, const float* cos_sin, int32_t seq, int32_t head_dim, int32_t rope_cols,
+                               const float* axis, int32_t grid, int32_t start, int32_t row0_unrotated, void* stream);
 int32_t revo_probe_mfma(const void* src_bf16, int64_t n_elems, float* sink, int32_t blocks, int32_t iters, void* stream);
 int64_t revo_probe_mfma_flops(int32_t blocks, int32_t iters);
 int32_t revo_probe_copy(void* dst, const void* src, int64_t bytes, void* stream);
@@ -136,6 +140,7 @@
 int32_t revo_debug_gemm_stamps(void* buf, int32_t items);
 int32_t revo_debug_attention_clock(void* buf);
 int32_t revo_debug_gemm_forms(int32_t reset);
+int32_t revo_debug_gemm_rope_lds(int32_t reset);
 int32_t revo_op_set_gemm_tile(int32_t tile);
 int32_t revo_op_set_variant(int32_t flags);
 int32_t revo_op_set_ln_fold(int32_t on);
diff --git a/revers-o_amd/_lib.py b/revers-o_amd/_lib.py
--- a/revers-o_amd/_lib.py
+++ b/revers-o_amd/_lib.py
@@ -76,6 +76,8 @@
     "revo_op_gemm_rope": (_i32, [_p, _i64, _p, _i64, _i32, _i32, _i32, _p, _i64, _p, _p, _i32, _i32, _i32, _p]),
     "revo_op_gemm_ln_in_rope": (_i32, [_p, _i64, _p, _i64, _i32, _i32, _i32, _p, _i64, _p, _p, _p, _i32, _f32, _p, _i32, _i32, _i32,
                                        _p]),
+    "revo_op_gemm_rope_axis": (_i32, [_p, _i64, _p, _i64, _i32, _i32, _i32, _p, _i64, _p, _p, _p, _i32, _f32, _p, _i32, _i32, _i32,
+                                      _p, _i32, _i32, _i32, _p]),
     "revo_op_gemm_resid_norm": (_i32, [_p, _i64, _p, _i64, _i32, _i32, _i32, _p, _i64, _p, _p, _p, _i64, _f32, C.POINTER(C.c_int32),
                                        _p]),
     "revo_op_layernorm": (_i32, [_p, _i64, _p, _p, _f32, _i32, _i32, _p, _i64, _i32, _p]),
@@ -103,6 +105,7 @@
     "revo_op_set_phase_groups": (_i32, [_i32]),
     "revo_op_set_qstores": (_i32, [_i32]),
     "revo_debug_gemm_forms": (_i32, [_i32]),
+    "revo_debug_gemm_rope_lds": (_i32, [_i32]),
     "revo_debug_gemm_stamps": (_i32, [_p, _i32]),
     "revo_debug_attention_clock": (_i32, [_p]),
     "revo_op_set_variant": (_i32, [_i32]),
diff --git a/revers-o_amd/csrc/api.hip b/revers-o_amd/csrc/api.hip
--- a/revers-o_amd/csrc/api.hip
+++ b/revers-o_amd/csrc/api.hip
@@ -126,6 +126,8 @@
     float *pln_w = nullptr, *pln_b = nullptr, *w_pfc1 = nullptr, *b_pfc1 = nullptr, *w_pfc2 = nullptr, *b_pfc2 = nullptr,
           *w_projT = nullptr;
     float2* rope_cs = nullptr;
+    float2* rope_axis = nullptr;
+    int rope_G = 0;
     bf16_t *patches = nullptr, *h = nullptr, *qkv = nullptr, *att = nullptr, *mlp = nullptr;
     bf16_t* xlo = nullptr;
     float *x = nullptr, *pool_logits = nullptr, *pool_u = nullptr, *pool_att = nullptr, *pool_o = nullptr, *pool_h = nullptr,
@@ -356,6 +358,16 @@
         }
         CHECK_RC(v->dalloc(&v->rope_cs, cs.size()));
         REVO_HIP_CHECK(hipMemcpy(v->rope_cs, cs.data(), cs.size() * sizeof(float2), hipMemcpyHostToDevice));
+        std::vector<float2> axis((size_t)G * nf);
+        for (int g = 0; g < G; ++g)
+            for (int f = 0; f < nf; ++f) {
+                const double freq = 1.0 / pow((double)c.rope_theta, (double)(2 * f) / (double)d);
+                const double ang = (double)(g + start) * freq;
+                axis[(size_t)g * nf + f] = make_float2((float)cos(ang), (float)sin(ang));
+            }
+        CHECK_RC(v->dalloc(&v->rope_axis, axis.size()));
+        REVO_HIP_CHECK(hipMemcpy(v->rope_axis, axis.data(), axis.size() * sizeof(float2), hipMemcpyHostToDevice));
+        v->rope_G = G;
     }
 
     const size_t rows = (size_t)max_batch * S, B = (size_t)max_batch;
@@ -531,6 +543,7 @@
             a.A = v->h; a.lda = W; a.B = L.w_qkv; a.ldb = W; a.M = rows; a.N = 3 * W; a.K = W; a.C = v->qkv;
             a.ldc = 3 * W; a.bias = L.b_qkv; a.rope_cs = v->rope_cs; a.rope_S = S; a.rope_hd = v->hd;
             a.rope_cols = 2 * W;
+            a.rope_axis = vv->rope_axis; a.rope_G = vv->rope_G; a.rope_start = c.use_cls ? 1 : 0; a.rope_row0_unrotated = c.use_cls ? 1 : 0;
             ln_before(L.c_qkv, a);
             ProfScope ps("gemm_qkv", st);
             CHECK_RC(launch_gemm(EPI_BF16_ROPE, a, st));
@@ -684,6 +697,22 @@
     return revo::launch_gemm(revo::EPI_BF16_ROPE, g, (hipStream_t)stream);
     API_END
 }
+extern "C" int32_t revo_op_gemm_rope_axis(const void* a, int64_t lda, const void* b, int64_t ldb, int32_t m, int32_t n, int32_t k,
+                                          void* c, int64_t ldc, const float* bias, const float* csum, const void* stats,
+                                          int32_t parts, float eps, const float* cos_sin, int32_t seq, int32_t head_dim,
+                                          int32_t rope_cols, const float* axis, int32_t grid, int32_t start,
+                                          int32_t row0_unrotated, void* stream) {
+    API_BEGIN
+    REVO_REQUIRE(a && b && c && cos_sin && axis, "op_gemm_rope_axis: null argument");
+    REVO_REQUIRE((csum != nullptr) == (stats != nullptr), "op_gemm_rope_axis: csum and stats go together");
+    revo::GemmArgs g{};
+    g.A = (const bf16_t*)a; g.lda = lda; g.B = (const bf16_t*)b; g.ldb = ldb; g.M = m; g.N = n; g.K = k; g.C = c; g.ldc = ldc;
+    g.bias = bias; g.rope_cs = (const float2*)cos_sin; g.rope_S = seq; g.rope_hd = head_dim; g.rope_cols = rope_cols;
+    g.rope_axis = (const float2*)axis; g.rope_G = grid; g.rope_start = start; g.rope_row0_unrotated = row0_unrotated;
+    if (stats) { g.lnc_stats = (const float2*)stats; g.lnc_parts = parts; g.lnc_c = csum; g.lnc_eps = eps; }
+    return revo::launch_gemm(revo::EPI_BF16_ROPE, g, (hipStream_t)stream);
+    API_END
+}
 extern "C" int32_t revo_op_gemm_resid_norm(const void* a, int64_t lda, const void* b, int64_t ldb, int32_t m, int32_t n, int32_t k,
                                            float* c, int64_t ldc, const float* bias, const float* gamma, void* ln_out,
                                            int64_t ln_ldo, float eps, int32_t* fused, void* stream) {
@@ -738,6 +767,7 @@
     return 0;
 }
 extern "C" int32_t revo_debug_gemm_forms(int32_t reset) { return (int32_t)revo::gemm_debug_forms(reset); }
+extern "C" int32_t revo_debug_gemm_rope_lds(int32_t reset) { return revo::gemm_debug_rope_lds(reset); }
 extern "C" int32_t revo_op_set_gemm_tile(int32_t tile) {
     REVO_REQUIRE(tile == 0 || tile == 128 || tile == 256, "set_gemm_tile: 0, 128 or 256");
     revo::gemm_force_tile(tile);
diff --git a/revers-o_amd/csrc/gemm.hip b/revers-o_amd/csrc/gemm.hip
--- a/revers-o_amd/csrc/gemm.hip
+++ b/revers-o_amd/csrc/gemm.hip
@@ -312,9 +312,10 @@
     asm volatile("" ::: "memory");
 }
 
-template <int EPI, bool SKIP_DEAD = false, int XP = 0>
+template <int EPI, bool SKIP_DEAD = false, int XP = 0, bool RLDS = false>
 __device__ __forceinline__ void gemm256_epilogue(const GemmArgs& p, char* slab, int m_base, int n_base, int lane,
-                                                 f32x4 (&acc)[8][4], float2* lnst = nullptr, const float2* lnmr = nullptr) {
+                                                 f32x4 (&acc)[8][4], float2* lnst = nullptr, const float2* lnmr = nullptr,
+                                                 const char* rope_lds = nullptr) {
     static_assert(EPI == EPI_BF16 || EPI == EPI_BF16_GELU || EPI == EPI_F32 || EPI == EPI_RESID_F32 ||
                   EPI == EPI_BF16_ROPE, "");
     asm volatile("" : "+v"(lane) :: "memory");
@@ -338,6 +339,23 @@
             }
         }
         f32x4 rtab_next[8][2];
+        const bool rope_on = RLDS && n_base < p.rope_cols;
+        int rgx = 0, rgy = 0, rlane_off = 0, rq8 = 0, rr8 = 0;
+        bool rxaxis = false;
+        if (RLDS && rope_on) {
+            int hd = p.rope_hd, S = p.rope_S, G = p.rope_G;
+            asm volatile("" : "+s"(hd), "+s"(S), "+s"(G));
+            const int nf = hd >> 2;
+            const int pr = ((n_base + (lane & 7) * 8) % hd) >> 1;
+            rxaxis = pr < nf;
+            rlane_off = (rxaxis ? pr : pr - nf) * 8;
+            const int g = (m_base + (lane >> 3)) % S - p.rope_start;
+            rgy = g / G;
+            rgx = g - rgy * G;
+            if (g < 0) { rgy = -1; rgx = G - 1; }
+            rq8 = __builtin_amdgcn_readfirstlane(8 / G);
+            rr8 = 8 - rq8 * G;
+        }
 #pragma unroll
         for (int half = 0; half < 2; ++half) {
             if (SKIP_DEAD && m_base + half * 64 >= p.M) break;
@@ -357,7 +375,7 @@
                 }
             };
             f32x4 rtab[8][2];
-            if (EPI == EPI_BF16_ROPE) {
+            if (EPI == EPI_BF16_ROPE && !RLDS) {
                 if (half == 0) rope_load(0, rtab);
                 else {
 #pragma unroll
@@ -405,14 +423,37 @@
             };
             if (lnmr) frag_phase(std::true_type{});
             else frag_phase(std::false_type{});
-            if (EPI == EPI_BF16_ROPE && half == 0 && !(SKIP_DEAD && m_base + 64 >= p.M)) rope_load(1, rtab_next);
+            if (EPI == EPI_BF16_ROPE && !RLDS && half == 0 && !(SKIP_DEAD && m_base + 64 >= p.M)) rope_load(1, rtab_next);
             const int gcol = n_base + (lane & 7) * 8;
 #pragma unroll
             for (int it = 0; it < 8; ++it) {
                 const int rl = it * 8 + (lane >> 3);
                 uint4 v = *(const uint4*)(slab + rl * RS + (lane & 7) * 16);
                 const int grow = m_base + half * 64 + rl;
-                if (EPI == EPI_BF16_ROPE) {
+                if (EPI == EPI_BF16_ROPE && RLDS) {
+                    if (rope_on) {
+                        const int G = p.rope_G, nf8 = p.rope_hd * 2;
+                        const int off = rgy < 0 ? G * nf8 : (rxaxis ? rgx : rgy) * nf8 + rlane_off;
+                        const f32x4 r0 = *(const f32x4*)(rope_lds + off), r1 = *(const f32x4*)(rope_lds + off + 16);
+                        uint32_t w[4] = {v.x, v.y, v.z, v.w};
+#pragma unroll
+                        for (int j = 0; j < 4; ++j) {
+                            const float x0 = bf16_to_f32((bf16_t)(w[j] & 0xffff)), x1 = bf16_to_f32((bf16_t)(w[j] >> 16));
+                            const f32x4 r = j < 2 ? r0 : r1;
+                            const float cx = r[(j & 1) * 2], cy = r[(j & 1) * 2 + 1];
+                            w[j] = pack_bf16x2(x0 * cx - x1 * cy, x1 * cx + x0 * cy);
+                        }
+                        v = make_uint4(w[0], w[1], w[2], w[3]);
+                        rgx += rr8;
+                        rgy += rq8;
+                        if (rgx >= G) { rgx -= G; ++rgy; }
+                        if (rgy >= G) {
+                            rgy -= G;
+                            rgx -= p.rope_start;
+                            if (rgx < 0) { rgx += G; --rgy; }
+                        }
+                    }
+                } else if (EPI == EPI_BF16_ROPE) {
                     if (gcol < p.rope_cols) {
                         uint32_t w[4] = {v.x, v.y, v.z, v.w};
 #pragma unroll
@@ -471,6 +512,9 @@
 constexpr int LNC_RAW_BYTES = 256 * 6 * 8 + 1024, LNC_MR_BYTES = 256 * 8;
 constexpr int G256P_LN_OFF = 98304 + 5 * 9216;
 static_assert(G256P_LN_OFF + LNC_RAW_BYTES + LNC_MR_BYTES <= 163840, "");
+constexpr int G256P_ROPE_OFF = G256P_LN_OFF + LNC_RAW_BYTES + LNC_MR_BYTES;
+constexpr int G256P_ROPE_BYTES = 163840 - G256P_ROPE_OFF;
+static_assert(G256P_ROPE_OFF % 16 == 0 && G256P_ROPE_BYTES >= 3072 + 32, "");
 constexpr int G256_LDS_LN = G256_LDS + LNC_RAW_BYTES + LNC_MR_BYTES;
 constexpr int G256Q_BC_OFF = G256_LDS_LN + LNC_MR_BYTES;
 constexpr int G256Q_LDS = G256Q_BC_OFF + 2 * 2048;
@@ -493,7 +537,7 @@
                                                      (uint32_t)(off + lane * 16), 0, 0, 0);
     }
 }
-template <int VM = 4, class ARGS = GemmArgs>
+template <int VM = 4, class ARGS = GemmArgs, bool FRESH = false>
 __device__ __forceinline__ void lnc_merge_rows(const ARGS& p, const char* lds_raw, float2* lds_mr, int wave, int , bool one_ktile,
                                                bool tele = false, int rows_left = 0) {
     if (wave >= 4) return;
@@ -522,7 +566,11 @@
         };
         if (p.lnc_parts == 4) merge_n(std::integral_constant<int, 4>{});
         else if (p.lnc_parts == 6) merge_n(std::integral_constant<int, 6>{});
-        else lnf_merge((const float2*)lds_raw + t * p.lnc_parts, p.lnc_parts, p.lnc_eps, r, m);
+        else {
+            int parts = p.lnc_parts;
+            if (FRESH) asm volatile("" : "+s"(parts));
+            lnf_merge((const float2*)lds_raw + t * parts, parts, p.lnc_eps, r, m);
+        }
         lds_mr[t] = make_float2(r, m);
         if (tele) {
             const int live = rows_left - wave * 64 < 0 ? 0 : (rows_left - wave * 64 > 64 ? 64 : rows_left - wave * 64);
@@ -675,6 +723,7 @@
 template <int EPI, int BMR = 256, int XP = 0>
 __global__ __launch_bounds__(G256_THREADS, 2) void gemm256p_kernel(GemmArgs p, int nslot) {
     static_assert(BMR == 256 || BMR == 192, "");
+    constexpr bool RLDS = EPI == EPI_BF16_ROPE && XP == 0;
     extern __shared__ __attribute__((aligned(16))) char smem[];
     const int tiles_n = (p.N + 255) / 256;
     const int tiles_m = BMR == 256 ? (p.M + 255) / 256 : p.t192_tiles;
@@ -711,6 +760,13 @@
     char* lds_raw = smem + G256P_LN_OFF;
     float2* lds_mr = (float2*)(smem + G256P_LN_OFF + LNC_RAW_BYTES);
     float2* lds_st = (float2*)(smem + G256P_LN_OFF);
+    if constexpr (RLDS) {
+        const int tab16 = p.rope_G * p.rope_hd >> 3;
+        f32x4* dst = (f32x4*)(smem + G256P_ROPE_OFF);
+        for (int i = threadIdx.x; i < tab16 + 2; i += G256_THREADS)
+            dst[i] = i < tab16 ? ((const f32x4*)p.rope_axis)[i] : (f32x4){1.f, 0.f, 1.f, 0.f};
+        asm volatile("s_waitcnt vmcnt(0) lgkmcnt(0)" ::: "memory");
+    }
     if (lnc) lnc_issue_stats(p, m0, lds_raw, wave, lane);
     G256Operand A, B;
     g256_operand_init(A, p.A, p.lda, p.M, m0, wave, lane, BMR == 256 ? 256 : (tall ? 208 : 192));
@@ -724,17 +780,19 @@
             g256_issue_half(A, 0, 128, G256_A(smem, 1), wave);
             g256_issue_half(A, 1, 128, G256_A(smem, 1), wave);
         }
-        if (lnc && !(REVO_LNC_ABLATE & 1)) lnc_merge_rows(p, lds_raw, lds_mr, wave, lane, p.K <= 64, p.lnc_tele != nullptr && n0 == 0, p.M - m0);
+        if (lnc && !(REVO_LNC_ABLATE & 1)) lnc_merge_rows<4, GemmArgs, RLDS>(p, lds_raw, lds_mr, wave, lane, p.K <= 64, p.lnc_tele != nullptr && n0 == 0, p.M - m0);
         f32x4 acc[8][4];
 #pragma unroll
         for (int m = 0; m < 8; ++m)
 #pragma unroll
             for (int n = 0; n < 4; ++n) acc[m][n] = (f32x4){0.f, 0.f, 0.f, 0.f};
-        if constexpr (BMR == 256) gemm256_mainloop(A, B, smem, p.K, wave, lane, acc);
-        else gemm256_mainloop<192>(A, B, smem, p.K, wave, lane, acc, tall);
+        int lane_m = lane;
+        if constexpr (RLDS) asm volatile("v_mbcnt_lo_u32_b32 %0, -1, 0\n\tv_mbcnt_hi_u32_b32 %0, -1, %0" : "=v"(lane_m));
+        if constexpr (BMR == 256) gemm256_mainloop(A, B, smem, p.K, wave, lane_m, acc);
+        else gemm256_mainloop<192>(A, B, smem, p.K, wave, lane_m, acc, tall);
 
         int lane_e = lane;
-        if constexpr (EPI != EPI_BF16 && EPI != EPI_BF16_ROPE)
+        if constexpr (EPI != EPI_BF16 && (EPI != EPI_BF16_ROPE || RLDS))
             asm volatile("v_mbcnt_lo_u32_b32 %0, -1, 0\n\tv_mbcnt_hi_u32_b32 %0, -1, %0" : "=v"(lane_e));
         const int mb = m0 + (wave >> 2) * 128, nb = n0 + (wave & 3) * 64;
         GemmArgs pe = p;
@@ -746,14 +804,17 @@
         slot += nslot;
         const bool more = slot < total;
         if (more) {
-            sq = __builtin_amdgcn_readfirstlane(slot / n_cnt);
+            int n_cnt_d = n_cnt;
+            if constexpr (RLDS) asm volatile("" : "+s"(n_cnt_d));
+            sq = __builtin_amdgcn_readfirstlane(slot / n_cnt_d);
             mi = m_lo + sq;
             m0 = tile_row0(mi);
             n0 = (n_lo + (slot - sq * n_cnt)) * 256;
             tall = BMR != 256 && mi >= tall0;
             if (lnc && !(REVO_LNC_ABLATE & 4)) lnc_issue_stats(p, m0, lds_raw, wave, lane);
-            g256_operand_init(A, p.A, p.lda, p.M, m0, wave, lane, BMR == 256 ? 256 : (tall ? 208 : 192));
-            g256_operand_init(B, p.B, p.ldb, p.N, n0, wave, lane);
+            const int lane_n = RLDS ? lane_e : lane;
+            g256_operand_init(A, p.A, p.lda, p.M, m0, wave, lane_n, BMR == 256 ? 256 : (tall ? 208 : 192));
+            g256_operand_init(B, p.B, p.ldb, p.N, n0, wave, lane_n);
             g256_issue_half(A, 0, 0, G256_A(smem, 0), wave);
             g256_issue_half(A, 1, 0, G256_A(smem, 0), wave);
             g256_issue_half(B, 0, 0, G256_B(smem, 0), wave);
@@ -763,9 +824,10 @@
             gemm_epilogue<EPI, 8, 4>(pe, mb, nb, lane_e, acc);
         } else {
             const bool wide = (p.N & 7) == 0 && (p.ldc & 7) == 0;
-            if (wide) gemm256_epilogue<EPI, BMR != 256, XP>(pe, slab, mb, nb, lane_e, acc,
-                                                            lnf ? lds_st + (wave >> 2) * 128 * 4 + (wave & 3) : nullptr,
-                                                            lnc ? lds_mr + (wave >> 2) * 128 : nullptr);
+            if (wide) gemm256_epilogue<EPI, BMR != 256, XP, RLDS>(pe, slab, mb, nb, lane_e, acc,
+                                                                  lnf ? lds_st + (wave >> 2) * 128 * 4 + (wave & 3) : nullptr,
+                                                                  lnc ? lds_mr + (wave >> 2) * 128 : nullptr,
+                                                                  smem + G256P_ROPE_OFF);
             else gemm_epilogue<EPI, 8, 4>(pe, mb, nb, lane_e, acc);
         }
         if (lnf) {
@@ -1298,6 +1360,20 @@
 static unsigned long long* g_stamps = nullptr; static int g_stamp_items = 0;
 void gemm_set_stamps(unsigned long long* buf, int items) { g_stamps = buf; g_stamp_items = items; }
 #endif
+static bool rope_axis_fits(const GemmArgs& a) {
+    if (!a.rope_axis || a.rope_G <= 0 || (a.rope_start != 0 && a.rope_start != 1)) return false;
+    if ((a.rope_row0_unrotated != 0) != (a.rope_start == 1)) return false;
+    if ((long)a.rope_G * a.rope_G + a.rope_start != a.rope_S || a.rope_S < 8) return false;
+    if (a.rope_hd % 16 || a.rope_cols % 64 || ((uintptr_t)a.rope_axis & 15)) return false;
+    return (long)a.rope_G * (a.rope_hd >> 2) * 8 + 32 <= G256P_ROPE_BYTES;
+}
+#ifdef REVO_EXPERIMENTS
+static int g_rope_lds_launches = 0;
+int gemm_debug_rope_lds(int reset) { const int n = g_rope_lds_launches; if (reset) g_rope_lds_launches = 0; return n; }
+#define REVO_ROPE_LDS_LAUNCH() (++g_rope_lds_launches)
+#else
+#define REVO_ROPE_LDS_LAUNCH() ((void)0)
+#endif
 template <int EPI, int BMR = 256>
 static int launch_256p(const GemmArgs& a, hipStream_t st) {
     GemmArgs b = a;
@@ -1339,6 +1415,15 @@
         switch (xp) { REVO_LAUNCH_XP(1) REVO_LAUNCH_XP(2) REVO_LAUNCH_XP(3) default: break; }
 #undef REVO_LAUNCH_XP
         if (xp) { REVO_HIP_CHECK(hipGetLastError()); return 0; }
+    }
+    if constexpr (EPI == EPI_BF16_ROPE) {
+        if (!rope_axis_fits(b)) {
+            REVO_FUNC_LDS((gemm256p_kernel<EPI, BMR, 1>), G256P_LDS);
+            hipLaunchKernelGGL((gemm256p_kernel<EPI, BMR, 1>), dim3(8 * nslot), dim3(G256_THREADS), G256P_LDS, st, b, nslot);
+            REVO_HIP_CHECK(hipGetLastError());
+            return 0;
+        }
+        REVO_ROPE_LDS_LAUNCH();
     }
     REVO_FUNC_LDS((gemm256p_kernel<EPI, BMR>), G256P_LDS);
     hipLaunchKernelGGL((gemm256p_kernel<EPI, BMR>), dim3(8 * nslot), dim3(G256_THREADS), G256P_LDS, st, b, nslot);
diff --git a/revers-o_amd/csrc/kernels.h b/revers-o_amd/csrc/kernels.h
--- a/revers-o_amd/csrc/kernels.h
+++ b/revers-o_amd/csrc/kernels.h
@@ -24,6 +24,8 @@
     int gy;
     const float2* rope_cs;
     int rope_S, rope_hd, rope_cols;
+    const float2* rope_axis;
+    int rope_G, rope_start, rope_row0_unrotated;
     int prefer256;
     float* ws; long ws_elems;
     int t192_tiles, t192_tall;
@@ -63,6 +65,7 @@
 };
 #ifdef REVO_EXPERIMENTS
 unsigned gemm_debug_forms(int reset);
+int gemm_debug_rope_lds(int reset);
 #endif
 int launch_gemm_f32_ring(const GemmArgs& a, hipStream_t st);
 bool gemm_resid_folds(int M, int N, int K, long lda, long ldb, long ldc);
```

Result: no change. 2494 (-0.1%).
